# Colmar-zlicheng/Color-NeuS

Hardware: AMD Instinct MI355X
Metric: rays/sec (fwd+bwd) at 128 samples/ray (higher is better)
Workload: dtype f32; 1 GPU; Color_NeuS_dtu.yml renderer block (SDF 8x256 + colour 4x256 + relight 4x256), synthetic 800x800 view, 4096 rays/step/GPU x (64+64) samples, trained-like weights; samples_per_ray=128, parallelism=ray-sharded dp1, step=fwd+fused-loss+bwd+fused-clip-adam

## Files before the change

color-neus_amd/csrc/cnr_backend.h:

```cpp
#pragma once
#include "cnr_common.h"
#include "cnr_views.h"

namespace cnr {

constexpr int kMaxRaySamples = 256;
constexpr int kMaxOutside = 128;

struct Segment { int dst, src, len; };

struct PrepWeight {
  const float* g = nullptr;
  const float* v = nullptr;
  const float* b = nullptr;
  int n = 0, k_ref = 0;
  int nseg = 0; Segment seg[4];
  float* W = nullptr; int ldw = 0; int npad = 0;
  float* Wt = nullptr; int ldwt = 0; int kpad = 0;
  float* bias = nullptr;
  int row_rot = 0;
};

struct FinishWeight {
  const float* partial = nullptr; int nchunk = 0; int npad = 0; int ldk = 0;
// ... 24 lines not shown
};

struct UpSample {
  const float* o; const float* d; long R;
  const float* z; int ldz; const float* sdf; int lds; int n;
  int m;
  float inv_s;
  float* new_z;
  const float* w_in = nullptr;
  const float* u_in = nullptr;
};

struct MergeZ {
  long R; float* z; int ldz; const float* sdf_in; int lds_in; float* sdf_out; int lds_out; int n;
  const float* new_z; const float* new_sdf; int m;
};

struct SamplerStep {
  int do_merge; MergeZ g;
  UpSample u;
  int do_embed; float* E; float scale; int multires;
};
void be_sampler_step(const SamplerStep& p, cnr_stream s);

struct FineSetup {
  const float* o; const float* d; const float* z; long R; int M; float sample_dist;
  float scale; int multires; int multires_view;
  float* E;
  float* AUX;
};

struct GradFinish {
  long P; const float* E; const float* ce0; const float* ces; float scale; int multires;
  float* grad_out;
  float* AUX;
  int neg_g_as_view; int multires_view;
  float* featx; int ldfx; int F;
};

struct CompositeFwd {
  const float* o; const float* d; const float* z; long R; int M; float sample_dist;
  const float* sdf; const float* g; const float* color; int ldcolor; const float* gcolor; int ldg;
  const float* variance; float cos_anneal; const float* background_rgb;
  float* color_fine; float* s_val; float* cdf_fine; float* weight_sum; float* weight_max; float* weights;
  float* inside_sphere; float* depth; float* global_color;
  float* eik_partial;
  float* sdf_s; float* color_s; float* gcolor_s;
  const float* delta = nullptr; float* delta_ray_sum = nullptr;
};

struct PruneCount { const float* weights; long R; int M; float eps; int* counts; };
struct PruneScan { const int* counts; long R; int* offsets ; };
struct PruneGather {
  const float* weights; long R; int M; float eps; const int* offsets;
  int* idx;
  const float* featx; int ldfx; float* featx_c;
  const float* aux; float* aux_c;
  float* zero_gcol = nullptr; float* zero_relit = nullptr; float* zero_delta = nullptr;
};
struct PruneScatter {
  long P; const int* count; const int* idx;
  const float* gcol_c; const float* relit_c; const float* delta_c;
  float* gcol; float* relit; float* delta;
};

struct ReduceEik { const float* partial; long R; float* sums ; float* sums_out ; float* gradient_error; };

struct CompositeBwd {
  const float* o; const float* d; const float* z; long R; int M; float sample_dist;
  const float* sdf; const float* g; const float* color; int ldcolor; const float* gcolor; int ldg;
  const float* variance; float cos_anneal; const float* background_rgb; const float* eik_sums; float sdf_scale;
  int inv_sigmoid; int has_relight;
  const float* d_color_fine; const float* d_s_val; const float* d_cdf; const float* d_weight_sum; const float* d_weight_max;
  const float* d_gradients; const float* d_weights; const float* d_gradient_error; const float* d_depth;
  const float* d_global_color; const float* d_delta_relight; const float* d_delta_relight_ray ;
  const float* d_sdf_s; const float* d_color_s; const float* d_gcolor_s;
  float* ztop; int ldztop; int ztop_col;
  float* gbar;
  int ldtop = kTop;
  float* dtop;
  float* gc_a;
  float* dinvs_partial;
  float* d_rays_d;
  float* d_z;
};

struct ColTopBwd {
  long P; const float* gc_a ; const float* gc_b ; const float* gcolor; int squeeze; float* out;
  int ldtop = kTop;
};

struct GbarFinish {
  long P; const float* gbar_alpha; const float* daux_c; const float* daux_r; const float* E; float scale; int multires;
  float* gbar_total ; float* cbar ;
};

struct VarianceFinish { const float* partial; long R; const float* variance; float* d_variance; };

struct RaysGradFinish {
  long R; int M; const float* d; const float* z; float sample_dist;
  const float* pbar;
  const float* daux_dir_c; const float* daux_dir_r; int lddir; int multires_view;
  const float* d_rays_d_alpha;
  float* d_o; float* d_d;
  const float* dz_parts;
  float* d_near; float* d_far;
};

struct PbarFinish {
  long P; const float* daux_c; const float* daux_r; const float* ebar0; const float* ebars; const float* E;
  const float* ce0; const float* ces; const float* gbar_total ;
  float scale; int multires; float* pbar;
};

constexpr int kQueryCtxTag = 0x53515900;
struct QueryIn {
  long n, P; const float* pts; float* out; int* tag; int tag_value;
};
struct QuerySeed {
  long n, P; int F, ldztop; float inv_scale;
  const float* d_sdf; const float* d_feat; const float* d_grad;
  float* ztop; float* gbar;
  const int* tag; int want_grad;
};
struct QueryOut {
  long n; int F, ldf, ldg;
  const float* sdf_in; const float* feat_in; const float* g_in;
  float* sdf; float* feat; float* g;
};
void be_query_in(const QueryIn& p, cnr_stream s);
void be_query_seed(const QuerySeed& p, cnr_stream s);
void be_query_out(const QueryOut& p, cnr_stream s);

struct PackJob {
  const unsigned short* planes; long plane_stride; int rows; int ld; unsigned short* Wf;
};
void be_pack_frags_many(const PackJob* jobs, int count, cnr_stream s);
struct FusedLayer {
  const unsigned short* Wf;
  const float* wsc;
  const float* bias;
  int K;
  int N;
};
struct SdfValueChain {
  const float* E; long P;
  int nl;
  FusedLayer lay[kMaxLayers];
  int skip_mask; int emb;
  const float* wtop; const float* btop; float top_scale;
  float* sdf_out;
};
bool be_sdf_value_chain(const SdfValueChain& c, cnr_stream s);
struct SdfSaveChain {
  SdfValueChain v;
  float* Z[kMaxLayers] = {};
  int ldz = 0;
  float* rs[kMaxLayers + 1] = {};
  FusedLayer top;
  float* feat = nullptr; int ld_feat = 0;
};
bool be_sdf_save_chain(const SdfSaveChain& c, cnr_stream s);

constexpr int kChainSteps = 12;
struct ChainFwdStep {
  const unsigned short* Wf = nullptr;
  const float* wsc = nullptr;
  const float* bias = nullptr;
  int nkb_w = 0;
  int nkb_main = 0;
  int nkb_x = 0;
  const float* in = nullptr; int ld_in = 0;
  int x_src = 0;
  float* save = nullptr; int ld_save = 0;
  float* rs_in = nullptr;
  int head = 0;
};
struct ChainFwdHead { const float* W = nullptr; int ldw = 0; const float* bias = nullptr; int n = 0; };
struct ReluChainFwd {
  long P = 0; int nsteps = 0; ChainFwdStep st[kChainSteps];
  ChainFwdHead col_head; int col_squeeze = 1;
  float* gcol = nullptr;
  float* rgb_tail = nullptr; int ld_tail = 0;
  ChainFwdHead rel_head; int inv_sigmoid = 1;
  float* delta = nullptr;
  float* relit = nullptr;
  int dbg = 0;
  const int* P_dev = nullptr; const int* row_idx = nullptr;
};
bool be_relu_chain_fwd(const ReluChainFwd& c, cnr_stream s);
bool be_relu_chain_fwd_enabled();

void be_layer_gemm(const LayerGemm& g, cnr_stream s);
struct NarrowBwd {
  const float* X = nullptr; int ldx = 0;
  const float* Xb = nullptr; int ldxb = 0;
  const float* Y = nullptr; int ldy = 0; int ky = 0;
  long P = 0;
  const unsigned short* Wp = nullptr; long wp_stride = 0; int ldw = 0; int w_rows = 0; const float* wscale = nullptr;
  float* dx = nullptr; int lddx = 0; int ndx = 0;
  float* partial = nullptr; int ldk = 0; float* colsum = nullptr;
};
bool be_narrow_bwd_ok(const NarrowBwd& p);
int be_narrow_bwd_slots(long P);
void be_narrow_bwd(const NarrowBwd& p, cnr_stream s);
bool be_sweep0_ok(const LayerGemm& g);
int be_sweep0_slots(long P);
void be_sweep0_dw(const LayerGemm& g, float* partial, int ldk, cnr_stream s);
void be_dw_gemm(const DwGemm& g, cnr_stream s);
struct HeadBwd {
  const float* dtop; int ldt;
  const float* aux; int ldaux;
  const float* W; int ldw;
  int n; int K; long P;
  float* dout; int ldo;
  float* partial; float* colsum; int npad, ldk, nslots;
};
void be_head_bwd(const HeadBwd& p, cnr_stream s);
struct HeadFwd {
  const float* h; int ldh; long P; const int* P_dev;
  const float* W; int ldw; int n;
  Epi E;
};
void be_head_fwd(const HeadFwd& p, cnr_stream s);
struct StripBwd {
  const float* dout; int ldo; long P;
  int nt;
  const float* Wt; int ldwt;
  float* tail; int ldt; float tail_scale;
  const float* y; int ldy;
  float* partial; int npad, ldk, nslots;
};
void be_strip_bwd(const StripBwd& p, cnr_stream s);
bool be_fdw_enabled();
bool be_fdw_xrow();
void be_layer_dw_gemm(const LayerGemm& g, const DwGemm& d, const DwFuse& f, cnr_stream s);
void be_prep_weight(const PrepWeight& p, cnr_stream s);
void be_split_planes(const float* src, int rows, int ld, unsigned short* planes, float* inv_scale, cnr_stream s);
struct SplitJob { const float* src; int rows; int ld; unsigned short* planes; float* inv_scale; };
void be_prep_weights(const PrepWeight* p, int count, cnr_stream s);
void be_finish_weights(const FinishWeight* f, int count, cnr_stream s);
void be_split_planes_many(const SplitJob* jobs, int count, cnr_stream s);
void be_finish_weight(const FinishWeight& p, cnr_stream s);
void be_embed_z(const EmbedZ& p, cnr_stream s);
void be_embed_pts(const EmbedPts& p, cnr_stream s);
void be_upsample(const UpSample& p, cnr_stream s);
void be_merge(const MergeZ& p, cnr_stream s);
void be_fine_setup(const FineSetup& p, cnr_stream s);
void be_grad_finish(const GradFinish& p, cnr_stream s);
void be_composite_fwd(const CompositeFwd& p, cnr_stream s);
void be_reduce_eik(const ReduceEik& p, cnr_stream s);
void be_prune_count(const PruneCount& p, cnr_stream s);
void be_prune_scan(const PruneScan& p, cnr_stream s);
void be_prune_gather(const PruneGather& p, cnr_stream s);
void be_prune_scatter(const PruneScatter& p, cnr_stream s);
void be_composite_bwd(const CompositeBwd& p, cnr_stream s);
void be_coltop_bwd(const ColTopBwd& p, cnr_stream s);
void be_gbar_finish(const GbarFinish& p, cnr_stream s);
void be_variance_finish(const VarianceFinish& p, cnr_stream s);
void be_pbar_finish(const PbarFinish& p, cnr_stream s);
void be_rays_grad_finish(const RaysGradFinish& p, cnr_stream s);
void be_memset_zero(void* p, size_t bytes, cnr_stream s);

struct LossArgs {
  const float* color; const float* wsum; const float* drel; const float* gt; const float* mask;
  long R; int M; int rgb_l1; int include_mask;
  int drel_per_ray = 0;
};
constexpr int kLossBlocks = 256;
void be_loss_sums(const LossArgs& a, float* partial , float* sums , cnr_stream s);
void be_loss_grads(const LossArgs& a, const float* coef, float* d_color, float* d_wsum, float* d_drel, cnr_stream s);
struct LossScalars {
  float lf, le, lm, lr;
  float Rg, den_rgb, den_rel;
  float c_rgb, c_bce, c_rel;
  int use_mask, use_relight;
};
void be_loss_combine(const LossScalars& c, const float* sums, const float* gerr, float* out6, cnr_stream s);
void be_loss_coef(const LossScalars& c, const float* g_loss, const float* mean_rel, float* coef4, cnr_stream s);
void be_loss_forward(const LossArgs& a, float* partial, unsigned* ticket, const LossScalars& c, const float* gerr, float* sums, float* out6, cnr_stream s);
void be_loss_backward(const LossArgs& a, const LossScalars& c, const float* g_loss, const float* mean_rel, const float* eik_factor , float* coef4,
                      float* d_color, float* d_wsum, float* d_drel_ray , cnr_stream s);
void be_loss_shard_stats(const LossArgs& a, float* partial, unsigned* ticket, const float* eik_sums , float* stats8, cnr_stream s);
void be_loss_shard_combine(const LossScalars& c, const float* stats8, float* out8, cnr_stream s);
constexpr int kAdamBatch = 64;
constexpr int kAdamChunk = 4096;
struct AdamTensor { float* w; const float* g; long off; long n; int chunk0; };
struct AdamArgs {
  int count; AdamTensor t[kAdamBatch];
  int nchunks; float* partial;
  float* m; float* v;
  float lr, beta1, beta2, eps, max_norm;
  float bc1, bc2_sqrt;
  const float* hyper;
};
CNR_HD float adam_clip_coef(float norm2, float max_norm) {
  if (!(max_norm > 0.0f)) return 1.0f;
  const float c = max_norm / (sqrtf(norm2) + 1e-6f);
  return c < 1.0f ? c : 1.0f;
}
CNR_HD void adam_update1(const AdamArgs& a, float* w, float g, float* m, float* v) {
  const float m1 = *m + (g - *m) * (1.0f - a.beta1);
  const float v1 = *v * a.beta2 + (1.0f - a.beta2) * g * g;
  *m = m1; *v = v1;
  const float lr = a.hyper ? a.hyper[0] : a.lr, bc1 = a.hyper ? a.hyper[1] : a.bc1, bc2_sqrt = a.hyper ? a.hyper[2] : a.bc2_sqrt;
  const float denom = sqrtf(v1) / bc2_sqrt + a.eps;
// ... 270 lines not shown
```

color-neus_amd/csrc/cnr_bodies.h:

```cpp
#pragma once
#include "cnr_backend.h"
#include "cnr_raymath.h"

namespace cnr {

CNR_HD void body_embed_z_rows(const EmbedZ& p, long idx, float* out, float*) {
  long r = idx / p.m;
  int j = (int)(idx - r * p.m);
  float zz;
  if (p.make_z) {
    float nr = p.near_[r], fr = p.far_[r];
    zz = nr + (fr - nr) * linspace_at(0.0f, 1.0f, p.m, j);
    if (p.t_rand) zz = zz + (p.t_rand[r] - 0.5f) * 2.0f / (float)p.m;
    p.z[r * p.ldz + j] = zz;
  } else {
    zz = p.z[r * p.ldz + j];
  }
  float x[3];
  for (int c = 0; c < 3; ++c) x[c] = (p.o[r * 3 + c] + p.d[r * 3 + c] * zz) * p.scale;
  for (int c = 0; c < kEmb; ++c) out[c] = 0.0f;
  pe_row(x, p.multires, out);
}
CNR_HD void body_embed_z(const EmbedZ& p, long idx) { body_embed_z_rows(p, idx, p.E + idx * kEmb, nullptr); }

CNR_HD void body_embed_pts_rows(const EmbedPts& p, long i, float* e, float* a) {
  float pp[3];
  if (p.pts) {
    pp[0] = p.pts[i * 3]; pp[1] = p.pts[i * 3 + 1]; pp[2] = p.pts[i * 3 + 2];
  } else {
    long idx = p.start + i;
    long r2 = (long)p.res * p.res;
    int ix = (int)(idx / r2), iy = (int)((idx / p.res) % p.res), iz = (int)(idx % p.res);
    pp[0] = linspace_at(p.bmin[0], p.bmax[0], p.res, ix);
    pp[1] = linspace_at(p.bmin[1], p.bmax[1], p.res, iy);
    pp[2] = linspace_at(p.bmin[2], p.bmax[2], p.res, iz);
  }
  float x[3] = {pp[0] * p.scale, pp[1] * p.scale, pp[2] * p.scale};
  for (int c = 0; c < kEmb; ++c) e[c] = 0.0f;
  pe_row(x, p.multires, e);
  if (p.AUX) {
    for (int c = 0; c < kAux; ++c) a[c] = 0.0f;
    a[0] = pp[0]; a[1] = pp[1]; a[2] = pp[2];
  }
}
CNR_HD void body_embed_pts(const EmbedPts& p, long i) { body_embed_pts_rows(p, i, p.E + i * kEmb, p.AUX ? p.AUX + i * kAux : nullptr); }

CNR_HD void body_fine_setup_rows(const FineSetup& p, long pt, float* e, float* a) {
  long r = pt / p.M;
  int j = (int)(pt - r * p.M);
  float z0 = p.z[r * p.M + j];
  float dist = (j + 1 < p.M) ? p.z[r * p.M + j + 1] - z0 : p.sample_dist;
  float mid = z0 + dist * 0.5f;
  float pp[3], x[3], dd[3];
  for (int c = 0; c < 3; ++c) {
    dd[c] = p.d[r * 3 + c];
    pp[c] = p.o[r * 3 + c] + dd[c] * mid;
    x[c] = pp[c] * p.scale;
  }
  for (int c = 0; c < kEmb; ++c) e[c] = 0.0f;
  pe_row(x, p.multires, e);
  for (int c = 0; c < kAux; ++c) a[c] = 0.0f;
  a[0] = pp[0]; a[1] = pp[1]; a[2] = pp[2];
  if (p.multires_view > 0) pe_row(dd, p.multires_view, a + 6);
  else { a[6] = dd[0]; a[7] = dd[1]; a[8] = dd[2]; }
}
CNR_HD void body_fine_setup(const FineSetup& p, long pt) { body_fine_setup_rows(p, pt, p.E + pt * kEmb, p.AUX + pt * kAux); }

CNR_HD void body_grad_finish(const GradFinish& p, long pt) {
  const float* e = p.E + pt * kEmb;
  const float* c0 = p.ce0 + pt * kEmb;
  const float* cs = p.ces ? p.ces + pt * kEmb : nullptr;
  for (int c = 0; c < 3; ++c) {
    float acc = c0[c] + (cs ? cs[c] : 0.0f);
    float f = 1.0f;
    for (int k = 0; k < p.multires; ++k) {
      float csin = c0[3 + 6 * k + c] + (cs ? cs[3 + 6 * k + c] : 0.0f);
      float ccos = c0[6 + 6 * k + c] + (cs ? cs[6 + 6 * k + c] : 0.0f);
      acc = acc + f * (e[6 + 6 * k + c] * csin - e[3 + 6 * k + c] * ccos);
      f *= 2.0f;
    }
    float g = acc * p.scale;
    p.grad_out[pt * 3 + c] = g;
    p.AUX[pt * kAux + 3 + c] = g;
  }
  if (p.neg_g_as_view) {
    float v[3] = {-p.AUX[pt * kAux + 3], -p.AUX[pt * kAux + 4], -p.AUX[pt * kAux + 5]};
    float row[kAux];
    for (int c = 0; c < kAux; ++c) row[c] = 0.0f;
    if (p.multires_view > 0) pe_row(v, p.multires_view, row);
    else { row[0] = v[0]; row[1] = v[1]; row[2] = v[2]; }
    int npe = p.multires_view > 0 ? 3 + 6 * p.multires_view : 3;
    for (int c = 0; c < npe; ++c) p.AUX[pt * kAux + 6 + c] = row[c];
  }
  if (p.featx) {
    float* fx = p.featx + pt * p.ldfx + p.F;
    const float* a = p.AUX + pt * kAux;
    const int w = p.ldfx - p.F;
    for (int c = 0; c < w; ++c) fx[c] = c < kAux ? a[c] : 0.0f;
  }
}

CNR_HD void body_coltop_bwd(const ColTopBwd& p, long pt) {
  for (int c = 0; c < 3; ++c) {
    float gc = p.gc_a[pt * p.ldtop + c] + (p.gc_b ? p.gc_b[pt * 4 + c] : 0.0f);
    float y = p.gcolor[pt * 4 + c];
    p.out[pt * p.ldtop + c] = p.squeeze ? gc * y * (1.0f - y) : gc;
  }
  for (int c = 3; c < p.ldtop; ++c) p.out[pt * p.ldtop + c] = 0.0f;
}

CNR_HD void body_gbar_finish(const GbarFinish& p, long pt) {
  const float* e = p.E + pt * kEmb;
  float* cb = p.cbar + pt * kEmb;
  for (int c = 0; c < kEmb; ++c) cb[c] = 0.0f;
  for (int c = 0; c < 3; ++c) {
    float gb = p.gbar_alpha[pt * 4 + c];
    if (p.daux_c) gb += p.daux_c[pt * kAux + 3 + c];
    if (p.daux_r) gb += p.daux_r[pt * kAux + 3 + c];
    p.gbar_total[pt * 4 + c] = gb;
    float t = gb * p.scale;
    cb[c] = t;
    float f = 1.0f;
    for (int k = 0; k < p.multires; ++k) {
      cb[3 + 6 * k + c] = f * e[6 + 6 * k + c] * t;
      cb[6 + 6 * k + c] = -f * e[3 + 6 * k + c] * t;
      f *= 2.0f;
    }
  }
  p.gbar_total[pt * 4 + 3] = 0.0f;
}

CNR_HD void body_pbar_finish(const PbarFinish& p, long pt) {
  const float* e = p.E + pt * kEmb;
  for (int c = 0; c < 3; ++c) {
    float eb = p.ebar0[pt * kEmb + c] + (p.ebars ? p.ebars[pt * kEmb + c] : 0.0f);
    float x0bar = eb;
    float second = 0.0f;
    float f = 1.0f;
    for (int k = 0; k < p.multires; ++k) {
      float s = e[3 + 6 * k + c], co = e[6 + 6 * k + c];
      float ebs = p.ebar0[pt * kEmb + 3 + 6 * k + c] + (p.ebars ? p.ebars[pt * kEmb + 3 + 6 * k + c] : 0.0f);
      float ebc = p.ebar0[pt * kEmb + 6 + 6 * k + c] + (p.ebars ? p.ebars[pt * kEmb + 6 + 6 * k + c] : 0.0f);
      x0bar += f * (co * ebs - s * ebc);
      if (p.gbar_total) {
        float ces = p.ce0[pt * kEmb + 3 + 6 * k + c] + (p.ces ? p.ces[pt * kEmb + 3 + 6 * k + c] : 0.0f);
        float cec = p.ce0[pt * kEmb + 6 + 6 * k + c] + (p.ces ? p.ces[pt * kEmb + 6 + 6 * k + c] : 0.0f);
        second += f * f * (-s * ces - co * cec);
      }
      f *= 2.0f;
    }
    if (p.gbar_total) x0bar += p.gbar_total[pt * 4 + c] * p.scale * second;
    float pb = x0bar * p.scale;
    if (p.daux_c) pb += p.daux_c[pt * kAux + c];
    if (p.daux_r) pb += p.daux_r[pt * kAux + c];
    p.pbar[pt * 4 + c] = pb;
  }
  p.pbar[pt * 4 + 3] = 0.0f;
}

CNR_HD void body_query_in(const QueryIn& p, long i) {
  p.out[i] = i < p.n * 3 ? p.pts[i] : 0.0f;
  if (i == 0) *p.tag = p.tag_value;
}
CNR_HD bool query_ctx_mismatch(const QuerySeed& p) {
  const int t = *p.tag;
  return p.want_grad ? t != kQueryCtxTag + 1 : (t != kQueryCtxTag && t != kQueryCtxTag + 1);
}

CNR_HD void body_query_seed(const QuerySeed& p, long i) {
  const long q4 = p.ldztop / 4, nz = p.P * q4;
  const float poison = query_ctx_mismatch(p) ? __builtin_nanf("") : 0.0f;
  if (i < nz) {
    const long row = i / q4;
    const int c0 = (int)(i - row * q4) * 4;
    float v[4];
    for (int j = 0; j < 4; ++j) {
      const int c = c0 + j;
      float t = 0.0f;
      if (row < p.n) {
        if (c < p.F) t = p.d_feat ? p.d_feat[row * p.F + c] : 0.0f;
        else if (c == p.F) t = p.d_sdf ? p.d_sdf[row] * p.inv_scale : 0.0f;
      }
      v[j] = t + poison;
    }
    f4 o; o.x = v[0]; o.y = v[1]; o.z = v[2]; o.w = v[3];
    *reinterpret_cast<f4*>(p.ztop + row * p.ldztop + c0) = o;
  } else {
    const long row = i - nz;
    const bool live = row < p.n && p.d_grad;
    f4 o;
    o.x = (live ? p.d_grad[row * 3 + 0] : 0.0f) + poison; o.y = (live ? p.d_grad[row * 3 + 1] : 0.0f) + poison;
    o.z = (live ? p.d_grad[row * 3 + 2] : 0.0f) + poison; o.w = 0.0f;
    *reinterpret_cast<f4*>(p.gbar + row * 4) = o;
  }
}

CNR_HD void body_query_out(const QueryOut& p, long i) {
  if (p.sdf) {
    if (i < p.n) { p.sdf[i] = p.sdf_in[i]; return; }
    i -= p.n;
  }
  if (p.feat) {
    const long nf = p.n * p.F;
    if (i < nf) { const long r = i / p.F; p.feat[i] = p.feat_in[r * p.ldf + (i - r * p.F)]; return; }
    i -= nf;
  }
  const long r = i / 3;
  p.g[i] = p.g_in[r * p.ldg + (i - r * 3)];
}
CNR_HD long query_out_count(const QueryOut& p) { return (p.sdf ? p.n : 0) + (p.feat ? p.n * p.F : 0) + (p.g ? p.n * 3 : 0); }

struct PixKey { unsigned k0, k1, step; };
CNR_HD PixKey pix_key(long seed, long step) {
  const unsigned long long s = (unsigned long long)seed;
  return PixKey{(unsigned)(s & 0xffffffffull), (unsigned)(s >> 32), (unsigned)((unsigned long long)step & 0xffffffffull)};
}
CNR_HD void pix_philox(unsigned c0, unsigned c1, unsigned c2, unsigned c3, unsigned k0, unsigned k1, unsigned out[4]) {
// ... 636 lines not shown
```

color-neus_amd/csrc/cnr_chain.hip:

```cpp
#include <hip/hip_runtime.h>

#include <cstdlib>
#include <type_traits>

#include "cnr_backend.h"
#include "cnr_hip_util.h"
#include "cnr_gemm_int.h"
#include "cnr_chain_util.h"

namespace cnr {

constexpr int kPackBatch = 64;
struct PackBatch { int count; int blk_start[kPackBatch + 1]; PackJob j[kPackBatch]; };
static_assert(sizeof(PackBatch) <= 4096, "kernel argument block");

__global__ __launch_bounds__(64) void pack_frags_kernel(const PackBatch b) {
  int i = 0;
  while (i + 1 < b.count && (int)blockIdx.x >= b.blk_start[i + 1]) ++i;
  const PackJob& j = b.j[i];
  const int blk = (int)blockIdx.x - b.blk_start[i];
  const int nkb = j.ld / 16;
  const int plane = blk & 1, kb = (blk >> 1) % nkb, cb = (blk >> 1) / nkb;
  const int lane = threadIdx.x, m = lane & 31;
  const int n = cb * 32 + 16 * ((m >> 2) & 1) + 4 * (m >> 3) + (m & 3);
  typedef unsigned short u16x8 __attribute__((ext_vector_type(8)));
  u16x8 v = {0, 0, 0, 0, 0, 0, 0, 0};
  if (n < j.rows) v = *reinterpret_cast<const u16x8*>(j.planes + (long)plane * j.plane_stride + (long)n * j.ld + kb * 16 + (lane >> 5) * 8);
  *reinterpret_cast<u16x8*>(j.Wf + ((long)blk * 64 + lane) * 8) = v;
}

void be_pack_frags_many(const PackJob* jobs, int count, cnr_stream s) {
  for (int i0 = 0; i0 < count; i0 += kPackBatch) {
    PackBatch b;
    b.count = count - i0 < kPackBatch ? count - i0 : kPackBatch;
    int blks = 0;
    for (int i = 0; i < b.count; ++i) { b.blk_start[i] = blks; b.j[i] = jobs[i0 + i]; blks += 8 * (jobs[i0 + i].ld / 16) * 2; }
    b.blk_start[b.count] = blks;
    TimingScope ts_("pack_frags", 2, 0, blks, 0, 0, 0, s);
    hipLaunchKernelGGL(pack_frags_kernel, dim3(blks), dim3(64), 0, s, b);
  }
  CNR_LAUNCH_CHECK("pack_frags");
}

template <int RT, int CB>
__global__ __launch_bounds__(512 / CB, 2 / (3 - CB) + 0) void sdf_value_chain_kernel(const SdfValueChain c) {
  constexpr int WAVES = 8 / CB, THREADS = 64 * WAVES;
  constexpr int T = 32 * RT;
  constexpr int APLANE = T * CH_ALD;
  extern __shared__ __attribute__((aligned(16))) unsigned char smem[];
  float* rs = reinterpret_cast<float*>(smem + 2 * APLANE);
  float* pm = rs + T;
  float* cwb = pm + T * 8;
  float* wtop = cwb + 1024;
  const int tid0 = threadIdx.x, wave = __builtin_amdgcn_readfirstlane(tid0 >> 6);
  const long ntiles = (c.P + T - 1) / T;
#define VC_LANE_INDICES                                                                      \
  int tid = tid0;                                                                            \
  asm volatile("" : "+v"(tid));                                                              \
  const int lane = tid & 63, half = lane >> 5, pt = lane & 31;                               \
  const int cbase = wave * CB * 32 + 16 * half;

  f16x8 wr1[4][CB], wr2[4][CB];
  auto wlane_of = [&](const FusedLayer& L, int lane_) __attribute__((always_inline)) { return L.Wf + (long)wave * CB * (L.K >> 4) * 1024 + lane_ * 8; };
  auto wprime = [&](const FusedLayer& L, int lane_) __attribute__((always_inline)) { chain_wprime<CB>(wr1, wr2, wlane_of(L, lane_), L.K >> 4, 0, L.K >> 4); };
  auto cw_fetch = [&](const FusedLayer& L, int tid_) __attribute__((always_inline)) {
    f4 v = {0.f, 0.f, 0.f, 0.f};
    if (tid_ < 64) v = *reinterpret_cast<const f4*>(L.wsc + tid_ * 4);
    else if (tid_ < 128) v = *reinterpret_cast<const f4*>(L.bias + (tid_ - 64) * 4);
    return v;
  };

  wprime(c.lay[0], tid0 & 63);
  for (int i = tid0; i < 256; i += THREADS) wtop[i] = c.wtop[i];
  for (long tile = blockIdx.x; tile < ntiles; tile += gridDim.x) {
    constexpr int NPASS = T * 16 / THREADS;
    {
    int tid = tid0;
    asm volatile("" : "+v"(tid));
    if (tid < 128) *reinterpret_cast<f4*>(cwb + tid * 4) = cw_fetch(c.lay[0], tid);
    f4 erows[NPASS];
#pragma unroll
    for (int pass = 0; pass < NPASS; ++pass) {
      const int row_l = pass * (THREADS / 16) + (tid >> 4), sc4 = (tid & 15) * 4;
      long grow = tile * T + row_l; if (grow >= c.P) grow = c.P - 1;
      erows[pass] = *reinterpret_cast<const f4*>(c.E + grow * kEmb + (sc4 < kEmb ? sc4 : 0));
    }
#pragma unroll
    for (int pass = 0; pass < NPASS; ++pass) {
      const int row_l = pass * (THREADS / 16) + (tid >> 4), sc4 = (tid & 15) * 4;
      const f4 z4 = {0.f, 0.f, 0.f, 0.f};
      const f4 v = sc4 < kEmb ? erows[pass] : z4;
      float mx = ws_absmax4(v);
      mx = cnr_max16(mx);
      const float sc = chain_row_scale(mx);
      if (sc4 < kEmb) {
        f16x4 h1, h2;
        float x;
        x = v.x * sc; h1[0] = (_Float16)x; h2[0] = (_Float16)(x - (float)h1[0]);
        x = v.y * sc; h1[1] = (_Float16)x; h2[1] = (_Float16)(x - (float)h1[1]);
        x = v.z * sc; h1[2] = (_Float16)x; h2[2] = (_Float16)(x - (float)h1[2]);
        x = v.w * sc; h1[3] = (_Float16)x; h2[3] = (_Float16)(x - (float)h1[3]);
        unsigned char* dst = smem + row_l * CH_ALD + sc4 * 2;
        *reinterpret_cast<f16x4*>(dst) = h1;
        *reinterpret_cast<f16x4*>(dst + APLANE) = h2;
      }
      if ((tid & 15) == 0) rs[row_l] = cnr_pow2_rcp(sc);
    }
    }
    lds_barrier();

    for (int l = 0; l < c.nl; ++l) {
      VC_LANE_INDICES
      const FusedLayer& L = c.lay[l];
      const int nkb = L.K >> 4;
      const bool last = l + 1 == c.nl;
      const unsigned short* wlane = wlane_of(L, lane);
      const f4 cw_next = cw_fetch(c.lay[last ? l : l + 1], tid);
      f32x16 acc[CB][RT];
#pragma unroll
      for (int j = 0; j < CB; ++j)
#pragma unroll
        for (int rt = 0; rt < RT; ++rt)
#pragma unroll
          for (int r = 0; r < 16; ++r) acc[j][rt][r] = 0.0f;
      const unsigned char* Ab = smem + pt * CH_ALD + half * 16;
      if (nkb == 16) chain_mfma_blocks<RT, CB, 16>(acc, wr1, wr2, Ab, APLANE, wlane, 16, 0);
      else chain_mfma_blocks<RT, CB, 3>(acc, wr1, wr2, Ab, APLANE, wlane, 3, 0);
      wprime(last ? c.lay[0] : c.lay[l + 1], lane);

      const float* cw = cwb + (l & 1) * 512;
      const bool next_skip = !last && ((c.skip_mask >> (l + 1)) & 1);
      const float oscale = next_skip ? kInvSqrt2 : 1.0f;
      const bool ragged = L.N < 256;
      float red[RT], dotj[CB][RT];
#pragma unroll
      for (int rt = 0; rt < RT; ++rt) {
        red[rt] = 0.0f;
#pragma unroll
        for (int j = 0; j < CB; ++j) dotj[j][rt] = 0.0f;
      }
#pragma unroll
      for (int j = 0; j < CB; ++j) {
        const int c0 = cbase + 32 * j;
        f4 wsc4[4], b4[4];
#pragma unroll
        for (int q = 0; q < 4; ++q) {
          wsc4[q] = *reinterpret_cast<const f4*>(cw + c0 + 4 * q);
          b4[q] = *reinterpret_cast<const f4*>(cw + 256 + c0 + 4 * q);
        }
#pragma unroll
        for (int rt = 0; rt < RT; ++rt) {
          const int row_l = rt * 32 + pt;
          const f2 rsc = pk_splat(rs[row_l]);
#pragma unroll
          for (int q = 0; q < 8; ++q) {
            const f2 w = {wsc4[q >> 1][(2 * q) & 3], wsc4[q >> 1][(2 * q + 1) & 3]};
            const f2 b = {b4[q >> 1][(2 * q) & 3], b4[q >> 1][(2 * q + 1) & 3]};
            f2 a = {acc[j][rt][2 * q], acc[j][rt][2 * q + 1]};
            a = pk_fma(a, rsc * w, b);
            a = softplus100_pk(a);
            if (next_skip) a = a * pk_splat(kInvSqrt2);
            acc[j][rt][2 * q] = a.x; acc[j][rt][2 * q + 1] = a.y;
          }
          if (ragged && c0 + 16 > L.N) {
            long grow = tile * T + row_l; if (grow >= c.P) grow = c.P - 1;
            const float* erow = c.E + grow * kEmb;
            float ev[16];
#pragma unroll
            for (int r = 0; r < 16; ++r) { const int ei = c0 + r - L.N; ev[r] = erow[ei < 0 ? 0 : (ei < kEmb ? ei : kEmb - 1)]; }
#pragma unroll
            for (int r = 0; r < 16; ++r) {
              const int ei = c0 + r - L.N;
              const float tail = (next_skip && ei < c.emb) ? ev[r] * oscale : 0.0f;
              acc[j][rt][r] = ei < 0 ? acc[j][rt][r] : tail;
            }
          }
          float mx = 0.0f, dot = 0.0f;
          if (last) {
#pragma unroll
            for (int q = 0; q < 4; ++q) {
              const f4 wt = *reinterpret_cast<const f4*>(wtop + c0 + 4 * q);
              dot = fmaf(acc[j][rt][4 * q], wt.x, dot); dot = fmaf(acc[j][rt][4 * q + 1], wt.y, dot);
              dot = fmaf(acc[j][rt][4 * q + 2], wt.z, dot); dot = fmaf(acc[j][rt][4 * q + 3], wt.w, dot);
            }
          } else {
#pragma unroll
            for (int r = 0; r < 16; r += 2) mx = fmaxf(fmaxf(fabsf(acc[j][rt][r]), fabsf(acc[j][rt][r + 1])), mx);
          }
          if (last) dotj[j][rt] = dot; else red[rt] = fmaxf(red[rt], mx);
        }
      }
#pragma unroll
      for (int rt = 0; rt < RT; ++rt) {
        if (last) {
#pragma unroll
          for (int j = 0; j < CB; ++j) {
            const float both = cnr_pair32_sum(dotj[j][rt]);
            if (half == 0) pm[(rt * 32 + pt) * 8 + wave * CB + j] = both;
          }
        } else {
          const float both = cnr_pair32_max(red[rt]);
          if (half == 0) pm[(rt * 32 + pt) * 8 + wave] = both;
        }
      }
      lds_barrier();
      if (!last) {
        if (tid < 128) *reinterpret_cast<f4*>(cwb + ((l + 1) & 1) * 512 + tid * 4) = cw_next;
#pragma unroll
        for (int rt = 0; rt < RT; ++rt) {
          const int row_l = rt * 32 + pt;
          float mx = pm[row_l * 8];
#pragma unroll
          for (int w = 1; w < WAVES; ++w) mx = fmaxf(mx, pm[row_l * 8 + w]);
          const float sc = chain_row_scale(mx);
#pragma unroll
          for (int j = 0; j < CB; ++j) chain_put16(acc[j][rt], sc, smem + row_l * CH_ALD + (cbase + 32 * j) * 2, APLANE);
          if (wave == 0 && half == 0) rs[row_l] = cnr_pow2_rcp(sc);
        }
      } else {
        for (int row = tid; row < T; row += THREADS) {
          float sum = pm[row * 8];
#pragma unroll
          for (int w = 1; w < 8; ++w) sum += pm[row * 8 + w];
          const long grow = tile * T + row;
          if (grow < c.P) c.sdf_out[grow] = (sum + c.btop[0]) * c.top_scale;
        }
      }
      lds_barrier();
    }
  }
}

#undef VC_LANE_INDICES

template <int RT, int CB>
static void launch_sdf_value_chain(const SdfValueChain& c, cnr_stream s) {
  constexpr int T = 32 * RT, THREADS = 512 / CB;
  const size_t lds = (size_t)2 * T * CH_ALD + (size_t)T * 9 * sizeof(float) + (size_t)(1024 + 256) * sizeof(float);
  static DeviceOnce attr_once;
  if (attr_once.first())
    (void)hipFuncSetAttribute(reinterpret_cast<const void*>(&sdf_value_chain_kernel<RT, CB>), hipFuncAttributeMaxDynamicSharedMemorySize, 160 * 1024);
  const long ntiles = (c.P + T - 1) / T;
  const int wgs_env = debug_flags().chain_wgs;
  const long wgs = wgs_env > 0 ? wgs_env : (lds * 2 <= 160 * 1024 ? 512 : 256);
  const unsigned grid = (unsigned)(ntiles < wgs ? ntiles : wgs);
  double macs = 0.0;
  for (int l = 0; l < c.nl; ++l) macs += (double)c.lay[l].K * 256.0;
  TimingScope ts_("chain_sdf_value", 3, RT * 10 + CB, c.P, (int)(macs / 256.0), 256, 1, s, (double)c.P * (kEmb + 1) * 4.0);
  hipLaunchKernelGGL((sdf_value_chain_kernel<RT, CB>), dim3(grid), dim3(THREADS), lds, s, c);
}

bool be_sdf_value_chain(const SdfValueChain& c, cnr_stream s) {
  const bool off = debug_flags().no_fused;
  if (off || c.P <= 0) return false;
  for (int l = 0; l < c.nl; ++l)
    if ((c.lay[l].K != 256 && c.lay[l].K != 48) || c.lay[l].N > 256 || c.lay[l].N < 1) return false;
  const int force = debug_flags().chain_shape;
  const int shape = force ? force : (c.P >= 256L * 128 ? 41 : (c.P >= 256L * 64 ? 22 : 12));
  if (shape == 41) launch_sdf_value_chain<4, 1>(c, s);
  else if (shape == 22) launch_sdf_value_chain<2, 2>(c, s);
  else launch_sdf_value_chain<1, 2>(c, s);
  CNR_LAUNCH_CHECK("chain_sdf_value");
  return true;
}

}
```

color-neus_amd/csrc/cnr_debug.h:

```cpp
#pragma once

namespace cnr {

struct DebugFlags {
  bool no_fused = false, no_chain_fwd = false, no_chain_sdf = false, no_fdw = false, fdw_split = false, no_top_fuse = false,
       no_head_bwd = false, no_head_fwd = false, no_strip_bwd = false, no_sampler_fuse = false, no_sweep0 = false, no_narrow_bwd = false,
       no_narrow_dx = false, disable_ws = false, ws_generic = false, ws_nostream = false, dw_fp32 = false, dw_bf16 = false, roctx = false;
  int ws_serp = 1;
#ifdef CNR_TUNING
  int ws_kinds = 0xffff, ws_minw = 96, ws_wgs = 256, ws_mintpw = 1, chain_wgs = 0, chain_shape = 0, chain_fwd_rt = 0, fdw_deep = 0, fdw_norev = 0,
      fdw_revmode = 0, fdw_dbg = 0, chain_fwd_dbg = 0;
  long chain_sdf_maxp = 1L << 62;
#else
  static constexpr int ws_kinds = 0xffff, ws_minw = 96, ws_wgs = 256, ws_mintpw = 1, chain_wgs = 0, chain_shape = 0, chain_fwd_rt = 0, fdw_deep = 0,
                       fdw_norev = 0, fdw_revmode = 0, fdw_dbg = 0, chain_fwd_dbg = 0;
  static constexpr long chain_sdf_maxp = 1L << 62;
#endif
};

const DebugFlags& debug_flags();

#ifdef CNR_TUNING
#define CNR_ABLATION(x) (x)
#else
#define CNR_ABLATION(x) 0
#endif

}
```

color-neus_amd/csrc/cnr_kernels.hip:

```cpp
#include <hip/hip_runtime.h>
#include <dlfcn.h>

#include <cstdio>
#include <vector>

#include "cnr_backend.h"
#include "cnr_loss.h"
#include "cnr_bodies.h"
#include "cnr_hip_util.h"

namespace cnr {

typedef float f32x16 __attribute__((ext_vector_type(16)));

hipError_t g_first_error = hipSuccess;
const char* g_first_error_where = "";

const char* be_name() { return "hip-gfx950"; }

struct TimingRec { KernelTiming t; hipEvent_t e0, e1; };
static bool g_timing_on = false;
static std::vector<TimingRec> g_timing;
static std::vector<hipEvent_t> g_event_pool;
static hipEvent_t get_event() {
  if (!g_event_pool.empty()) { hipEvent_t e = g_event_pool.back(); g_event_pool.pop_back(); return e; }
  hipEvent_t e;
  (void)hipEventCreate(&e);
  return e;
}
void timing_begin(const char* name, int kind, int nt, long P, int N, int K, int pairs, hipStream_t s, double bytes) {
  if (!g_timing_on) return;
  TimingRec r;
  snprintf(r.t.name, sizeof r.t.name, "%s", name);
  r.t.kind = kind; r.t.nt = nt; r.t.P = P; r.t.N = N; r.t.K = K; r.t.pairs = pairs; r.t.ms = 0.f; r.t.bytes = bytes;
  r.e0 = get_event(); r.e1 = get_event();
  (void)hipEventRecord(r.e0, s);
  g_timing.push_back(r);
}
void timing_end(hipStream_t s) {
  if (!g_timing_on || g_timing.empty()) return;
  (void)hipEventRecord(g_timing.back().e1, s);
}
void be_timing_enable(int on) { g_timing_on = on != 0; }
int be_timing_collect(KernelTiming* out, int max_records) {
  int n = 0;
  for (auto& r : g_timing) {
    (void)hipEventSynchronize(r.e1);
    float ms = 0.f;
    (void)hipEventElapsedTime(&ms, r.e0, r.e1);
    r.t.ms = ms;
    if (out && n < max_records) out[n] = r.t;
    ++n;
    g_event_pool.push_back(r.e0);
    g_event_pool.push_back(r.e1);
  }
  g_timing.clear();
  return n;
}

namespace {
struct Roctx {
  int (*push)(const char*) = nullptr; int (*pop)() = nullptr;
  Roctx() {
    if (!debug_flags().roctx) return;
    for (const char* lib : {"librocprofiler-sdk-roctx.so", "libroctx64.so"}) {
      void* h = dlopen(lib, RTLD_LAZY | RTLD_GLOBAL);
      if (!h) continue;
      push = reinterpret_cast<int (*)(const char*)>(dlsym(h, "roctxRangePushA"));
      pop = reinterpret_cast<int (*)()>(dlsym(h, "roctxRangePop"));
      if (push && pop) return;
      push = nullptr; pop = nullptr;
    }
  }
};
Roctx& roctx() { static Roctx r; return r; }
}
void be_range_push(const char* name) { if (roctx().push) (void)roctx().push(name); }
void be_range_pop() { if (roctx().pop) (void)roctx().pop(); }

int be_check_last_error(char* msg, size_t n) {
  if (g_first_error == hipSuccess) return 0;
  snprintf(msg, n, "HIP error in %s: %s", g_first_error_where, hipGetErrorString(g_first_error));
  g_first_error = hipSuccess;
  return -1;
}

void be_memset_zero(void* p, size_t bytes, cnr_stream s) {
  hipError_t e = hipMemsetAsync(p, 0, bytes, s);
  if (e != hipSuccess && g_first_error == hipSuccess) { g_first_error = e; g_first_error_where = "memset"; }
}

__global__ void zero_cols_kernel(float* p, int ld, int c0, int c1, long rows) {
  const int w = c1 - c0;
  const long i = (long)blockIdx.x * blockDim.x + threadIdx.x;
  if (i < rows * w) p[(i / w) * ld + c0 + (int)(i % w)] = 0.0f;
}
void be_zero_cols(float* p, int ld, int c0, int c1, long rows, cnr_stream s) {
  if (c1 <= c0 || rows <= 0) return;
  const long n = rows * (c1 - c0);
  hipLaunchKernelGGL(zero_cols_kernel, dim3((unsigned)((n + 255) / 256)), dim3(256), 0, s, p, ld, c0, c1, rows);
  CNR_LAUNCH_CHECK("zero_cols");
}

__global__ __launch_bounds__(256) void copy_cols_kernel(float* dst, int ld_dst, const float* src, int ld_src, int ncols, long rows) {
  const long n = rows * ncols;
  for (long i = (long)blockIdx.x * 256 + threadIdx.x; i < n; i += (long)gridDim.x * 256) {
    const long r = i / ncols;
    const int c = (int)(i - r * ncols);
    dst[r * ld_dst + c] = src[r * ld_src + c];
  }
}
void be_copy_cols(float* dst, int ld_dst, const float* src, int ld_src, int ncols, long rows, cnr_stream s) {
  if (ncols <= 0 || rows <= 0) return;
  long blocks = (rows * ncols + 255) / 256;
  if (blocks > 65536) blocks = 65536;
  hipLaunchKernelGGL(copy_cols_kernel, dim3((unsigned)blocks), dim3(256), 0, s, dst, ld_dst, src, ld_src, ncols, rows);
  CNR_LAUNCH_CHECK("copy_cols");
}

__global__ __launch_bounds__(512) void head_bwd_kernel(const HeadBwd p, long pts_per_slot) {
  __shared__ float red[8][4][256];
  const int cg = threadIdx.x & 63, rl = threadIdx.x >> 6, k = cg * 4;
  const long p0 = (long)blockIdx.x * pts_per_slot;
  long p1 = p0 + pts_per_slot;
  if (p1 > p.P) p1 = p.P;
  const bool live = k < p.K;
  f4 w[4], acc[4];
  float cs[4] = {0.f, 0.f, 0.f, 0.f};
  const f4 z4 = {0.f, 0.f, 0.f, 0.f};
#pragma unroll
  for (int j = 0; j < 4; ++j) { acc[j] = z4; w[j] = (live && j < p.n) ? *reinterpret_cast<const f4*>(p.W + (long)j * p.ldw + k) : z4; }
  f4 an[8], dn[8];
  const int kl = live ? k : 0;
  auto fetch = [&](long pt) __attribute__((always_inline)) {
#pragma unroll
    for (int u = 0; u < 8; ++u) {
      long q = pt + 8 * u < p1 ? pt + 8 * u : p1 - 1;
      if (q < 0) q = 0;
      an[u] = *reinterpret_cast<const f4*>(p.aux + q * p.ldaux + kl);
      dn[u] = *reinterpret_cast<const f4*>(p.dtop + q * p.ldt);
    }
  };
  fetch(p0 + rl);
  for (long pt = p0 + rl; pt < p1; pt += 64) {
    f4 a[8], d[8];
#pragma unroll
    for (int u = 0; u < 8; ++u) { a[u] = live ? an[u] : z4; d[u] = dn[u]; }
    fetch(pt + 64);
#pragma unroll
    for (int u = 0; u < 8; ++u) {
      if (pt + 8 * u < p1) {
        const float dj[4] = {d[u].x, d[u].y, d[u].z, d[u].w};
        f4 v = z4;
#pragma unroll
        for (int j = 0; j < 4; ++j) {
          v.x = fmaf(w[j].x, dj[j], v.x); v.y = fmaf(w[j].y, dj[j], v.y); v.z = fmaf(w[j].z, dj[j], v.z); v.w = fmaf(w[j].w, dj[j], v.w);
          acc[j].x = fmaf(dj[j], a[u].x, acc[j].x); acc[j].y = fmaf(dj[j], a[u].y, acc[j].y);
          acc[j].z = fmaf(dj[j], a[u].z, acc[j].z); acc[j].w = fmaf(dj[j], a[u].w, acc[j].w);
          cs[j] += dj[j];
        }
        f4 o;
        o.x = a[u].x > 0.0f ? v.x : 0.0f; o.y = a[u].y > 0.0f ? v.y : 0.0f; o.z = a[u].z > 0.0f ? v.z : 0.0f; o.w = a[u].w > 0.0f ? v.w : 0.0f;
// ... 189 lines not shown
  }
CNR_POINTWISE_KERNELS(CNR_PW_KERNEL)

constexpr int kRowsPerBlock = 128, kRowLd = 49;
static_assert(kEmb == 48 && kAux == 48, "row staging assumes 48-float rows");
template <class PARAM, void (*ROWS)(const PARAM&, long, float*, float*)>
__global__ __launch_bounds__(kRowsPerBlock) void staged_rows_kernel(const PARAM p, long n, float* E, float* AUX) {
  __shared__ float sE[kRowsPerBlock * kRowLd];
  __shared__ float sA[kRowsPerBlock * kRowLd];
  const int tid = threadIdx.x;
  for (long base = (long)blockIdx.x * kRowsPerBlock; base < n; base += (long)gridDim.x * kRowsPerBlock) {
    if (base + tid < n) ROWS(p, base + tid, sE + tid * kRowLd, sA + tid * kRowLd);
    __syncthreads();
    const int cnt = (int)((n - base) < kRowsPerBlock ? (n - base) : kRowsPerBlock) * 48;
    for (int e = tid; e < cnt; e += kRowsPerBlock) {
      const int r = e / 48, c = e - r * 48;
      E[base * 48 + e] = sE[r * kRowLd + c];
      if (AUX) AUX[base * 48 + e] = sA[r * kRowLd + c];
    }
    __syncthreads();
  }
}
template <class PARAM, void (*ROWS)(const PARAM&, long, float*, float*)>
static void staged_rows_launch(const char* name, const PARAM& p, long n, float* E, float* AUX, cnr_stream s) {
  if (n <= 0) return;
  long blocks = (n + kRowsPerBlock - 1) / kRowsPerBlock;
  if (blocks > 16384) blocks = 16384;
  TimingScope ts_(name, 2, 0, n, 0, 0, 0, s);
  hipLaunchKernelGGL((staged_rows_kernel<PARAM, ROWS>), dim3((unsigned)blocks), dim3(kRowsPerBlock), 0, s, p, n, E, AUX);
}
void be_embed_z(const EmbedZ& p, cnr_stream s) { staged_rows_launch<EmbedZ, body_embed_z_rows>("embed_z", p, p.R * p.m, p.E, nullptr, s); CNR_LAUNCH_CHECK("embed_z"); }
void be_embed_pts(const EmbedPts& p, cnr_stream s) { staged_rows_launch<EmbedPts, body_embed_pts_rows>("embed_pts", p, p.n, p.E, p.AUX, s); CNR_LAUNCH_CHECK("embed_pts"); }
void be_fine_setup(const FineSetup& p, cnr_stream s) { staged_rows_launch<FineSetup, body_fine_setup_rows>("fine_setup", p, p.R * p.M, p.E, p.AUX, s); CNR_LAUNCH_CHECK("fine_setup"); }

__global__ __launch_bounds__(256) void grad_finish_kernel(const GradFinish p) {
  const int lane16 = threadIdx.x & 15;
  const long pt0 = ((long)blockIdx.x * 256 + threadIdx.x) >> 4;
  const long stride = (long)gridDim.x * 16;
  for (long pt = pt0; pt < p.P; pt += stride) {
    const int c0 = lane16 * 3;
    float e[3], ce[3];
#pragma unroll
    for (int c = 0; c < 3; ++c) {
      e[c] = p.E[pt * kEmb + c0 + c];
      ce[c] = p.ce0[pt * kEmb + c0 + c] + (p.ces ? p.ces[pt * kEmb + c0 + c] : 0.0f);
    }
    const int k = lane16 > 0 ? (lane16 - 1) >> 1 : 0;
    const bool is_sin = lane16 >= 1 && (lane16 & 1) == 1 && lane16 <= 2 * p.multires;
    const bool is_cos = lane16 >= 2 && (lane16 & 1) == 0 && lane16 <= 2 * p.multires;
    const float f = (float)(1 << k);
    float part[3];
#pragma unroll
    for (int c = 0; c < 3; ++c) {
      const float e_next = __shfl_down(e[c], 1, 16);
      const float e_prev = __shfl_up(e[c], 1, 16);
      float t = 0.0f;
      if (lane16 == 0) t = ce[c];
      else if (is_sin) t = f * (e_next * ce[c]);
      else if (is_cos) t = -(f * (e_prev * ce[c]));
      part[c] = t;
    }
#pragma unroll
    for (int d = 8; d >= 1; d >>= 1)
#pragma unroll
      for (int c = 0; c < 3; ++c) part[c] += __shfl_xor(part[c], d, 16);
    float g[3];
#pragma unroll
    for (int c = 0; c < 3; ++c) g[c] = part[c] * p.scale;
    if (lane16 == 0) {
#pragma unroll
      for (int c = 0; c < 3; ++c) { p.grad_out[pt * 3 + c] = g[c]; p.AUX[pt * kAux + 3 + c] = g[c]; }
    }
    float aux[3];
#pragma unroll
    for (int c = 0; c < 3; ++c) aux[c] = lane16 == 1 ? g[c] : p.AUX[pt * kAux + c0 + c];
    if (p.neg_g_as_view) {
      const int et = lane16 - 2;
      if (et >= 0) {
        float v[3] = {-g[0], -g[1], -g[2]};
        const int npe_tr = p.multires_view > 0 ? 1 + 2 * p.multires_view : 1;
#pragma unroll
        for (int c = 0; c < 3; ++c) {
          float val = 0.0f;
          if (et == 0) val = v[c];
          else if (et < npe_tr) { const float ff = (float)(1 << ((et - 1) >> 1)); val = (et & 1) ? sinf(v[c] * ff) : cosf(v[c] * ff); }
          if (et < npe_tr) { aux[c] = val; p.AUX[pt * kAux + c0 + c] = val; }
        }
      }
    }
    if (p.featx) {
      const int w = p.ldfx - p.F;
#pragma unroll
      for (int c = 0; c < 3; ++c)
        if (c0 + c < w) p.featx[pt * p.ldfx + p.F + c0 + c] = aux[c];
      for (int c = kAux + lane16; c < w; c += 16) p.featx[pt * p.ldfx + p.F + c] = 0.0f;
    }
  }
}
void be_grad_finish(const GradFinish& p, cnr_stream s) {
  if (p.P <= 0) return;
  long blocks = (p.P * 16 + 255) / 256;
  if (blocks > 16384) blocks = 16384;
  TimingScope ts_("grad_finish", 2, 0, p.P, 0, 0, 0, s);
  hipLaunchKernelGGL(grad_finish_kernel, dim3((unsigned)blocks), dim3(256), 0, s, p);
  CNR_LAUNCH_CHECK("grad_finish");
}

__global__ __launch_bounds__(256) void gbar_finish_kernel(const GbarFinish p) {
  const int lane16 = threadIdx.x & 15;
  const long pt0 = ((long)blockIdx.x * 256 + threadIdx.x) >> 4;
  const long stride = (long)gridDim.x * 16;
  for (long pt = pt0; pt < p.P; pt += stride) {
    const int c0 = lane16 * 3;
    float e[3], gb[3];
#pragma unroll
    for (int c = 0; c < 3; ++c) {
      e[c] = p.E[pt * kEmb + c0 + c];
      float v = p.gbar_alpha[pt * 4 + c];
      if (p.daux_c) v += p.daux_c[pt * kAux + 3 + c];
      if (p.daux_r) v += p.daux_r[pt * kAux + 3 + c];
      gb[c] = v;
    }
    const int k = lane16 > 0 ? (lane16 - 1) >> 1 : 0;
    const bool is_sin = lane16 >= 1 && (lane16 & 1) == 1 && lane16 <= 2 * p.multires;
    const bool is_cos = lane16 >= 2 && (lane16 & 1) == 0 && lane16 <= 2 * p.multires;
    const float f = (float)(1 << k);
#pragma unroll
    for (int c = 0; c < 3; ++c) {
      const float e_next = __shfl_down(e[c], 1, 16);
      const float e_prev = __shfl_up(e[c], 1, 16);
      const float t = gb[c] * p.scale;
      float out = 0.0f;
      if (lane16 == 0) out = t;
      else if (is_sin) out = f * e_next * t;
      else if (is_cos) out = -f * e_prev * t;
      p.cbar[pt * kEmb + c0 + c] = out;
    }
    if (lane16 == 0) {
#pragma unroll
      for (int c = 0; c < 3; ++c) p.gbar_total[pt * 4 + c] = gb[c];
      p.gbar_total[pt * 4 + 3] = 0.0f;
    }
  }
}
void be_gbar_finish(const GbarFinish& p, cnr_stream s) {
  if (p.P <= 0) return;
  long blocks = (p.P * 16 + 255) / 256;
  if (blocks > 16384) blocks = 16384;
  TimingScope ts_("gbar_finish", 2, 0, p.P, 0, 0, 0, s);
  hipLaunchKernelGGL(gbar_finish_kernel, dim3((unsigned)blocks), dim3(256), 0, s, p);
  CNR_LAUNCH_CHECK("gbar_finish");
}

__device__ __forceinline__ float wave_sum(float x) {
#pragma unroll
  for (int d = 32; d >= 1; d >>= 1) x += __shfl_xor(x, d);
  return x;
}
__device__ __forceinline__ float wave_max(float x) {
#pragma unroll
  for (int d = 32; d >= 1; d >>= 1) x = fmaxf(x, __shfl_xor(x, d));
  return x;
}
__device__ __forceinline__ int wave_min_int(int x) {
#pragma unroll
  for (int d = 32; d >= 1; d >>= 1) { int y = __shfl_xor(x, d); x = y < x ? y : x; }
  return x;
}
__device__ __forceinline__ float block_sum_256(float x, float* sh4 ) {
  x = wave_sum(x);
  __syncthreads();
  if ((threadIdx.x & 63) == 0) sh4[threadIdx.x >> 6] = x;
  __syncthreads();
  return (sh4[0] + sh4[1]) + (sh4[2] + sh4[3]);
}

__device__ __forceinline__ double block_sum_256d(double x, double* sh4) {
#pragma unroll
  for (int d = 32; d >= 1; d >>= 1) x += __shfl_xor(x, d);
  __syncthreads();
  if ((threadIdx.x & 63) == 0) sh4[threadIdx.x >> 6] = x;
  __syncthreads();
  return (sh4[0] + sh4[1]) + (sh4[2] + sh4[3]);
}

__device__ __forceinline__ void prep_weight_row(const PrepWeight& p, const int n, double* redd) {
  const int tid = threadIdx.x;
  const bool real = n < p.n;
  const int nr = real ? (n + p.row_rot) % p.n : 0;
  float scale = 1.0f;
  if (p.g != nullptr) {
    double ss = 0.0;
    if (real)
      for (int c = tid; c < p.k_ref; c += 256) { double x = p.v[(long)nr * p.k_ref + c]; ss += x * x; }
    ss = block_sum_256d(ss, redd);
    if (real) scale = p.g[nr] / (float)sqrt(ss);
  }
  for (int j = tid; j < p.kpad; j += 256) {
    float val = 0.0f;
    if (real && j < p.ldw) {
      int src = -1;
      for (int q = 0; q < p.nseg; ++q)
        if (j >= p.seg[q].dst && j < p.seg[q].dst + p.seg[q].len) src = p.seg[q].src + (j - p.seg[q].dst);
      if (src >= 0) val = p.v[(long)nr * p.k_ref + src] * scale;
    }
    if (j < p.ldw) p.W[(long)n * p.ldw + j] = val;
    if (n < p.ldwt) p.Wt[(long)j * p.ldwt + n] = val;
  }
  if (tid == 0) p.bias[n] = real && p.b ? p.b[nr] : 0.0f;
}
__global__ __launch_bounds__(256) void prep_weight_kernel(const PrepWeight p) {
  __shared__ double redd[4];
  prep_weight_row(p, blockIdx.x, redd);
}
constexpr int kPrepBatch = 24;
struct PrepBatch { int count; int row_start[kPrepBatch + 1]; PrepWeight p[kPrepBatch]; };
static_assert(sizeof(PrepBatch) <= 4096, "kernel argument block");
__global__ __launch_bounds__(256) void prep_weight_batch_kernel(const PrepBatch b) {
  __shared__ double redd[4];
  int i = 0;
  while (i + 1 < b.count && (int)blockIdx.x >= b.row_start[i + 1]) ++i;
  prep_weight_row(b.p[i], (int)blockIdx.x - b.row_start[i], redd);
}

__device__ __forceinline__ void split_planes_row(const float* src, int ld, unsigned short* planes, long plane_stride, float* inv_scale, const int r) {
  const float* row = src + (long)r * ld;
  float mx = 0.0f;
  for (int k = threadIdx.x; k < ld; k += 64) mx = fmaxf(mx, fabsf(row[k]));
#pragma unroll
  for (int d = 32; d >= 1; d >>= 1) mx = fmaxf(mx, __shfl_xor(mx, d));
  float sc = 1.0f;
  if (mx > 0.0f && mx < 3.0e38f) { int e; (void)frexpf(mx, &e); if (e < -100) e = -100; sc = ldexpf(1.0f, 14 - e); }
  for (int k = threadIdx.x; k < ld; k += 64) {
    const float x = row[k] * sc;
    const _Float16 h1 = (_Float16)x;
    const _Float16 h2 = (_Float16)(x - (float)h1);
    planes[(long)r * ld + k] = __builtin_bit_cast(unsigned short, h1);
    planes[plane_stride + (long)r * ld + k] = __builtin_bit_cast(unsigned short, h2);
  }
  if (threadIdx.x == 0) inv_scale[r] = 1.0f / sc;
}
__global__ __launch_bounds__(64) void split_planes_kernel(const float* src, int ld, unsigned short* planes, long plane_stride, float* inv_scale) {
  split_planes_row(src, ld, planes, plane_stride, inv_scale, blockIdx.x);
}
constexpr int kSplitBatch = 2 * kPrepBatch;
struct SplitBatch { int count; int row_start[kSplitBatch + 1]; SplitJob j[kSplitBatch]; };
static_assert(sizeof(SplitBatch) <= 4096, "kernel argument block");
__global__ __launch_bounds__(64) void split_planes_batch_kernel(const SplitBatch b) {
  int i = 0;
  while (i + 1 < b.count && (int)blockIdx.x >= b.row_start[i + 1]) ++i;
  const SplitJob& j = b.j[i];
  split_planes_row(j.src, j.ld, j.planes, (long)j.rows * j.ld, j.inv_scale, (int)blockIdx.x - b.row_start[i]);
}
void be_split_planes_many(const SplitJob* jobs, int count, cnr_stream s) {
  for (int i0 = 0; i0 < count; i0 += kSplitBatch) {
    SplitBatch b;
    b.count = count - i0 < kSplitBatch ? count - i0 : kSplitBatch;
    int rows = 0;
    for (int i = 0; i < b.count; ++i) { b.row_start[i] = rows; b.j[i] = jobs[i0 + i]; rows += jobs[i0 + i].rows; }
    b.row_start[b.count] = rows;
    TimingScope ts_("split_planes", 2, 0, rows, 0, 0, 0, s);
    hipLaunchKernelGGL(split_planes_batch_kernel, dim3(rows), dim3(64), 0, s, b);
  }
  CNR_LAUNCH_CHECK("split_planes");
}
void be_prep_weights(const PrepWeight* p, int count, cnr_stream s) {
  for (int i0 = 0; i0 < count; i0 += kPrepBatch) {
    PrepBatch b;
    b.count = count - i0 < kPrepBatch ? count - i0 : kPrepBatch;
    int rows = 0;
    for (int i = 0; i < b.count; ++i) { b.row_start[i] = rows; b.p[i] = p[i0 + i]; rows += p[i0 + i].npad; }
    b.row_start[b.count] = rows;
    TimingScope ts_("prep_weight", 2, 0, rows, 0, 0, 0, s);
    hipLaunchKernelGGL(prep_weight_batch_kernel, dim3(rows), dim3(256), 0, s, b);
  }
  CNR_LAUNCH_CHECK("prep_weight");
}
void be_split_planes(const float* src, int rows, int ld, unsigned short* planes, float* inv_scale, cnr_stream s) {
  TimingScope ts_("split_planes", 2, 0, rows, 0, 0, 0, s);
  hipLaunchKernelGGL(split_planes_kernel, dim3(rows), dim3(64), 0, s, src, ld, planes, (long)rows * ld, inv_scale);
  CNR_LAUNCH_CHECK("split_planes");
}

void be_prep_weight(const PrepWeight& p, cnr_stream s) {
  TimingScope ts_("prep_weight", 2, 0, p.npad, 0, 0, 0, s);
  hipLaunchKernelGGL(prep_weight_kernel, dim3(p.npad), dim3(256), 0, s, p);
  CNR_LAUNCH_CHECK("prep_weight");
}

__device__ __forceinline__ void finish_weight_row(const FinishWeight& p, const int n, float* red, double* redd, float* dwi) {
  const int tid = threadIdx.x;
  const int nr = (n + p.row_rot) % p.n;
  for (int j = tid; j < p.ldk; j += 256) {
    const float* src = p.partial + (long)n * p.ldk + j;
    const long cs = (long)p.npad * p.ldk;
    float s = 0.0f;
    int c = 0;
    const int nch = j >= p.col_hi ? p.nchunk_hi : p.nchunk;
    for (; c + 8 <= nch; c += 8) {
      float v[8];
#pragma unroll
      for (int q = 0; q < 8; ++q) v[q] = src[(long)(c + q) * cs];
#pragma unroll
      for (int q = 0; q < 8; ++q) s += v[q];
    }
    for (; c < nch; ++c) s += src[(long)c * cs];
    dwi[j] = s;
  }
  __syncthreads();
  float dref[2] = {0.f, 0.f};
  int cref[2] = {-1, -1};
// ... 95 lines not shown
  for (int j = 0; j < 3; ++j) { const float s = block_sum_256(v[j], red); if (tid == 0) sums[j] = s; }
  if (tid == 0) sums[3] = 0.f;
}
void be_loss_sums(const LossArgs& a, float* partial, float* sums, cnr_stream s) {
  TimingScope ts_("loss_sums", 2, 0, a.R, 0, 0, 0, s);
  hipLaunchKernelGGL(loss_partial_kernel, dim3(kLossBlocks), dim3(256), 0, s, a, partial);
  hipLaunchKernelGGL(loss_fold_kernel, dim3(1), dim3(256), 0, s, partial, kLossBlocks, sums);
  CNR_LAUNCH_CHECK("loss_sums");
}
__global__ __launch_bounds__(256) void loss_forward_kernel(const LossArgs a, float* partial, unsigned* ticket, const LossScalars c, const float* gerr, float* sums,
                                                           float* out6, const int shard, const float* eik_sums) {
  __shared__ float red[4];
  __shared__ int is_last;
  const int tid = threadIdx.x, nb = gridDim.x, b = blockIdx.x;
  float s_rgb = 0.f, s_bce = 0.f, s_rel = 0.f;
  const long n_rgb = a.R * 3;
  for (long i = (long)b * 256 + tid; i < n_rgb; i += (long)nb * 256) s_rgb += loss_rgb_term(a.color[i], a.gt[i], a.rgb_l1);
  if (a.mask)
    for (long r = (long)b * 256 + tid; r < a.R; r += (long)nb * 256) s_bce += loss_bce_term(a.wsum[r], a.mask[r]);
  if (a.drel) {
    const long per_ray = a.drel_per_ray ? 1 : (long)a.M * 3, n_rel = a.R * per_ray;
    for (long i = (long)b * 256 + tid; i < n_rel; i += (long)nb * 256) {
      const float m = (a.include_mask && a.mask) ? a.mask[i / per_ray] : 1.0f;
      s_rel += a.drel[i] * m;
    }
  }
  s_rgb = block_sum_256(s_rgb, red);
  s_bce = block_sum_256(s_bce, red);
  s_rel = block_sum_256(s_rel, red);
  if (tid == 0) {
    partial[b * 4 + 0] = s_rgb; partial[b * 4 + 1] = s_bce; partial[b * 4 + 2] = s_rel; partial[b * 4 + 3] = 0.f;
    __threadfence();
    const unsigned t = atomicAdd(ticket, 1u);
    is_last = t == (unsigned)nb - 1u;
  }
  __syncthreads();
  if (!is_last) return;
  __threadfence();
  float v[3] = {0.f, 0.f, 0.f};
  for (int k = tid; k < nb; k += 256) {
    v[0] += __hip_atomic_load(partial + k * 4, __ATOMIC_RELAXED, __HIP_MEMORY_SCOPE_AGENT);
    v[1] += __hip_atomic_load(partial + k * 4 + 1, __ATOMIC_RELAXED, __HIP_MEMORY_SCOPE_AGENT);
    v[2] += __hip_atomic_load(partial + k * 4 + 2, __ATOMIC_RELAXED, __HIP_MEMORY_SCOPE_AGENT);
  }
  __shared__ float tot[4];
  for (int j = 0; j < 3; ++j) { const float sj = block_sum_256(v[j], red); if (tid == 0) tot[j] = sj; }
  if (tid == 0) {
    tot[3] = 0.f;
    if (shard) {
      const float num = eik_sums[0], den = eik_sums[1];
      sums[0] = tot[0]; sums[1] = tot[1]; sums[2] = tot[2]; sums[3] = num; sums[4] = den; sums[5] = den; sums[6] = 0.f; sums[7] = 0.f;
    } else {
      sums[0] = tot[0]; sums[1] = tot[1]; sums[2] = tot[2]; sums[3] = 0.f;
      loss_combine(c, tot, gerr, out6);
    }
    *ticket = 0;
  }
}
void be_loss_forward(const LossArgs& a, float* partial, unsigned* ticket, const LossScalars& c, const float* gerr, float* sums, float* out6, cnr_stream s) {
  TimingScope ts_("loss_forward", 2, 0, a.R, 0, 0, 0, s);
  hipLaunchKernelGGL(loss_forward_kernel, dim3(kLossBlocks), dim3(256), 0, s, a, partial, ticket, c, gerr, sums, out6, 0, (const float*)nullptr);
  CNR_LAUNCH_CHECK("loss_forward");
}
void be_loss_shard_stats(const LossArgs& a, float* partial, unsigned* ticket, const float* eik_sums, float* stats8, cnr_stream s) {
  TimingScope ts_("loss_shard_stats", 2, 0, a.R, 0, 0, 0, s);
  hipLaunchKernelGGL(loss_forward_kernel, dim3(kLossBlocks), dim3(256), 0, s, a, partial, ticket, LossScalars{}, (const float*)nullptr, stats8, (float*)nullptr, 1, eik_sums);
  CNR_LAUNCH_CHECK("loss_shard_stats");
}
__global__ void loss_shard_combine_kernel(const LossScalars c, const float* stats, float* out8) { if (threadIdx.x == 0 && blockIdx.x == 0) loss_shard_combine(c, stats, out8); }
void be_loss_shard_combine(const LossScalars& c, const float* stats8, float* out8, cnr_stream s) {
  TimingScope ts_("loss_shard_combine", 2, 0, 1, 0, 0, 0, s);
  hipLaunchKernelGGL(loss_shard_combine_kernel, dim3(1), dim3(64), 0, s, c, stats8, out8);
  CNR_LAUNCH_CHECK("loss_shard_combine");
}
__global__ __launch_bounds__(256) void loss_backward_kernel(const LossArgs a, const LossScalars c, const float* g_loss, const float* mean_rel, const float* eik_factor,
                                                            float* coef_out, float* d_color, float* d_wsum, float* d_drel_ray) {
  float coef[4];
  loss_coef(c, g_loss, c.use_relight ? mean_rel : g_loss, eik_factor, coef);
  if (blockIdx.x == 0 && threadIdx.x == 0) { coef_out[0] = coef[0]; coef_out[1] = coef[1]; coef_out[2] = coef[2]; coef_out[3] = coef[3]; }
  const long n_rgb = a.R * 3;
  const long stride = (long)gridDim.x * 256;
  for (long i = (long)blockIdx.x * 256 + threadIdx.x; i < n_rgb; i += stride) d_color[i] = coef[0] * loss_rgb_grad(a.color[i], a.gt[i], a.rgb_l1);
  if (d_wsum)
    for (long r = (long)blockIdx.x * 256 + threadIdx.x; r < a.R; r += stride) d_wsum[r] = a.mask ? coef[1] * loss_bce_grad(a.wsum[r], a.mask[r]) : 0.0f;
  if (d_drel_ray)
    for (long r = (long)blockIdx.x * 256 + threadIdx.x; r < a.R; r += stride) d_drel_ray[r] = (a.include_mask && a.mask) ? coef[2] * a.mask[r] : coef[2];
}
void be_loss_backward(const LossArgs& a, const LossScalars& c, const float* g_loss, const float* mean_rel, const float* eik_factor, float* coef4, float* d_color,
                      float* d_wsum, float* d_drel_ray, cnr_stream s) {
  TimingScope ts_("loss_backward", 2, 0, a.R, 0, 0, 0, s);
  long blocks = (a.R * 3 + 255) / 256;
  if (blocks > 1024) blocks = 1024;
  if (blocks < 1) blocks = 1;
  hipLaunchKernelGGL(loss_backward_kernel, dim3((unsigned)blocks), dim3(256), 0, s, a, c, g_loss, mean_rel, eik_factor, coef4, d_color, d_wsum, d_drel_ray);
  CNR_LAUNCH_CHECK("loss_backward");
}
__global__ __launch_bounds__(256) void loss_grads_kernel(const LossArgs a, const float* coef, float* d_color, float* d_wsum, float* d_drel) {
  const float c_rgb = coef[0], c_bce = coef[1], c_rel = coef[2];
  const long n_rgb = a.R * 3, per_ray = (long)a.M * 3, n_rel = a.drel || d_drel ? a.R * per_ray : 0;
  const long stride = (long)gridDim.x * 256;
  for (long i = (long)blockIdx.x * 256 + threadIdx.x; i < n_rgb; i += stride) d_color[i] = c_rgb * loss_rgb_grad(a.color[i], a.gt[i], a.rgb_l1);
  if (d_wsum)
    for (long r = (long)blockIdx.x * 256 + threadIdx.x; r < a.R; r += stride) d_wsum[r] = a.mask ? c_bce * loss_bce_grad(a.wsum[r], a.mask[r]) : 0.0f;
  if (d_drel)
    for (long i = (long)blockIdx.x * 256 + threadIdx.x; i < n_rel; i += stride) d_drel[i] = c_rel * ((a.include_mask && a.mask) ? a.mask[i / per_ray] : 1.0f);
}
__global__ void loss_combine_kernel(const LossScalars c, const float* sums, const float* gerr, float* out) { if (threadIdx.x == 0 && blockIdx.x == 0) loss_combine(c, sums, gerr, out); }
__global__ void loss_coef_kernel(const LossScalars c, const float* g_loss, const float* mean_rel, float* coef) { if (threadIdx.x == 0 && blockIdx.x == 0) loss_coef(c, g_loss, mean_rel, nullptr, coef); }
void be_loss_combine(const LossScalars& c, const float* sums, const float* gerr, float* out6, cnr_stream s) {
  hipLaunchKernelGGL(loss_combine_kernel, dim3(1), dim3(64), 0, s, c, sums, gerr, out6);
  CNR_LAUNCH_CHECK("loss_combine");
}
void be_loss_coef(const LossScalars& c, const float* g_loss, const float* mean_rel, float* coef4, cnr_stream s) {
  hipLaunchKernelGGL(loss_coef_kernel, dim3(1), dim3(64), 0, s, c, g_loss, mean_rel, coef4);
  CNR_LAUNCH_CHECK("loss_coef");
}
void be_loss_grads(const LossArgs& a, const float* coef, float* d_color, float* d_wsum, float* d_drel, cnr_stream s) {
  TimingScope ts_("loss_grads", 2, 0, a.R, 0, 0, 0, s);
  hipLaunchKernelGGL(loss_grads_kernel, dim3(1024), dim3(256), 0, s, a, coef, d_color, d_wsum, d_drel);
  CNR_LAUNCH_CHECK("loss_grads");
}

__global__ __launch_bounds__(256) void reduce_eik_kernel(const ReduceEik p) {
  __shared__ float red[4];
  float a = 0.0f, b = 0.0f;
  for (long r = threadIdx.x; r < p.R; r += 256) { a += p.partial[r * 2]; b += p.partial[r * 2 + 1]; }
  a = block_sum_256(a, red);
  b = block_sum_256(b, red);
  if (threadIdx.x == 0) {
    p.sums[0] = a; p.sums[1] = b;
    if (p.sums_out) { p.sums_out[0] = a; p.sums_out[1] = b; }
    *p.gradient_error = a / (b + 1e-5f);
  }
}
void be_reduce_eik(const ReduceEik& p, cnr_stream s) {
  TimingScope ts_("reduce_eik", 2, 0, p.R, 0, 0, 0, s);
  hipLaunchKernelGGL(reduce_eik_kernel, dim3(1), dim3(256), 0, s, p);
  CNR_LAUNCH_CHECK("reduce_eik");
}

__global__ __launch_bounds__(256) void variance_finish_kernel(const VarianceFinish p) {
  __shared__ float red[4];
  float a = 0.0f;
  for (long r = threadIdx.x; r < p.R; r += 256) a += p.partial[r];
  a = block_sum_256(a, red);
  if (threadIdx.x == 0) *p.d_variance = inv_s_backward(p.variance[0], a);
}
void be_variance_finish(const VarianceFinish& p, cnr_stream s) {
  TimingScope ts_("variance_finish", 2, 0, p.R, 0, 0, 0, s);
  hipLaunchKernelGGL(variance_finish_kernel, dim3(1), dim3(256), 0, s, p);
  CNR_LAUNCH_CHECK("variance_finish");
}

__device__ __forceinline__ float wave_scan_incl_add(float x, int lane) {
#pragma unroll
  for (int d = 1; d < 64; d <<= 1) { float y = __shfl_up(x, d); if (lane >= d) x = y + x; }
  return x;
}
__device__ __forceinline__ float wave_scan_incl_mul(float x, int lane) {
#pragma unroll
  for (int d = 1; d < 64; d <<= 1) { float y = __shfl_up(x, d); if (lane >= d) x = y * x; }
  return x;
}
__device__ __forceinline__ float wave_excl_cumprod(float f, int lane, float& carry) {
  const float incl = wave_scan_incl_mul(f, lane);
  float excl = __shfl_up(incl, 1);
  if (lane == 0) excl = 1.0f;
  const float T = carry * excl;
  carry = carry * __shfl(incl, 63);
  return T;
}
__device__ __forceinline__ float wave_scan_incl_add_rev(float x, int lane) {
#pragma unroll
  for (int d = 1; d < 64; d <<= 1) { float y = __shfl_down(x, d); if (lane + d < 64) x = x + y; }
  return x;
}

__device__ __forceinline__ void ray_section_slopes(const float* zs, const float* ss, int nsec, float* cs, int lane) {
  for (int i = lane; i < nsec; i += 64) cs[i] = upsample_slope(ss[i], ss[i + 1], zs[i], zs[i + 1]);
}
__device__ __forceinline__ void ray_section_alphas(const float* zs, const float* ss, const float* cs, const float* rs, int nsec, float inv_s, float* as, int lane) {
  for (int i = lane; i < nsec; i += 64) {
    const float c = upsample_cos(i > 0 ? cs[i - 1] : 0.0f, cs[i], rs[i], rs[i + 1]);
    as[i] = upsample_alpha(ss[i], ss[i + 1], zs[i], zs[i + 1], c, inv_s);
  }
}
__device__ __forceinline__ float ray_pdf_weights(float* as, int nsec, bool given_w, int lane) {
  float carry = 1.0f, part = 0.0f;
  for (int base = 0; base < nsec; base += 64) {
    const int i = base + lane;
    const bool ok = i < nsec;
    const float a = ok ? as[i] : 0.0f;
    const float T = wave_excl_cumprod(ok ? 1.0f - a + 1e-7f : 1.0f, lane, carry);
    const float w = (given_w ? a : a * T) + 1e-5f;
    if (ok) { as[i] = w; part += w; }
  }
  return wave_sum(part);
}
__device__ __forceinline__ void ray_cdf(const float* as, float total, int nsec, float* cs, int lane) {
  float csum = 0.0f;
  for (int base = 0; base < nsec; base += 64) {
    const int i = base + lane;
    const bool ok = i < nsec;
    const float pdf = ok ? as[i] / total : 0.0f;
    const float incl = wave_scan_incl_add(pdf, lane);
    if (ok) cs[i + 1] = csum + incl;
    csum = csum + __shfl(incl, 63);
  }
  if (lane == 0) cs[0] = 0.0f;
}

__global__ __launch_bounds__(256) void upsample_kernel(const UpSample p) {
  __shared__ float sh[4][5][kMaxRaySamples];
  const int lane = threadIdx.x & 63, wave = threadIdx.x >> 6;
  long ray = (long)blockIdx.x * 4 + wave;
  const bool active = ray < p.R;
  if (!active) ray = p.R - 1;
  float* zs = sh[wave][0]; float* ss = sh[wave][1]; float* cs = sh[wave][2]; float* rs = sh[wave][3]; float* as = sh[wave][4];
  const int n = p.n, nsec = p.n - 1;
  const bool given_w = p.w_in != nullptr;
  if (given_w) {
    for (int i = lane; i < n; i += 64) zs[i] = p.z[ray * p.ldz + i];
    for (int i = lane; i < nsec; i += 64) as[i] = p.w_in[ray * nsec + i];
  } else {
    float o[3], d[3];
    for (int c = 0; c < 3; ++c) { o[c] = p.o[ray * 3 + c]; d[c] = p.d[ray * 3 + c]; }
    for (int i = lane; i < n; i += 64) {
      float z = p.z[ray * p.ldz + i];
      zs[i] = z;
      ss[i] = p.sdf[ray * p.lds + i];
      rs[i] = ray_radius(o, d, z);
    }
  }
  __syncthreads();
  if (!given_w) ray_section_slopes(zs, ss, nsec, cs, lane);
  __syncthreads();
  if (!given_w) ray_section_alphas(zs, ss, cs, rs, nsec, p.inv_s, as, lane);
  __syncthreads();
  const float total = ray_pdf_weights(as, nsec, given_w, lane);
  __syncthreads();
  ray_cdf(as, total, nsec, cs, lane);
  __syncthreads();
  if (lane < p.m && active) {
    const float u = p.u_in ? p.u_in[ray * p.m + lane] : linspace_at(0.5f / (float)p.m, 1.0f - 0.5f / (float)p.m, p.m, lane);
    p.new_z[ray * p.m + lane] = invert_cdf(cs, zs, n, u);
  }
}
void be_upsample(const UpSample& p, cnr_stream s) {
  TimingScope ts_("upsample", 2, 0, p.R, 0, 0, 0, s, (double)p.R * (4.0 * p.n + 4.0 * (p.w_in ? p.n - 1 : p.n) + (p.w_in ? 0.0 : 24.0) + 4.0 * p.m));
  hipLaunchKernelGGL(upsample_kernel, dim3((unsigned)((p.R + 3) / 4)), dim3(256), 0, s, p);
  CNR_LAUNCH_CHECK("upsample");
}

__global__ __launch_bounds__(256) void merge_kernel(const MergeZ p) {
  __shared__ float sh[4][2][kMaxRaySamples];
  __shared__ float shn[4][2][64];
  const int lane = threadIdx.x & 63, wave = threadIdx.x >> 6;
  long ray = (long)blockIdx.x * 4 + wave;
  const bool active = ray < p.R;
  if (!active) ray = p.R - 1;
  float* zs = sh[wave][0]; float* ss = sh[wave][1]; float* nz = shn[wave][0]; float* ns = shn[wave][1];
  const bool with_sdf = p.new_sdf != nullptr;
  for (int i = lane; i < p.n; i += 64) { zs[i] = p.z[ray * p.ldz + i]; ss[i] = with_sdf ? p.sdf_in[ray * p.lds_in + i] : 0.0f; }
  for (int j = lane; j < p.m; j += 64) { nz[j] = p.new_z[ray * p.m + j]; ns[j] = with_sdf ? p.new_sdf[ray * p.m + j] : 0.0f; }
  __syncthreads();
  if (active)
    merge_samples(zs, ss, p.n, nz, ns, p.m, lane, 64, [&](int at, float z, float s) {
      p.z[ray * p.ldz + at] = z;
      if (with_sdf) p.sdf_out[ray * p.lds_out + at] = s;
    });
}
__global__ __launch_bounds__(256) void sampler_step_kernel(const SamplerStep p) {
  __shared__ float sh[4][7][kMaxRaySamples];
  __shared__ float shn[4][2][64];
  const int lane = threadIdx.x & 63, wave = threadIdx.x >> 6;
  long ray = (long)blockIdx.x * 4 + wave;
  const bool active = ray < p.u.R;
  if (!active) ray = p.u.R - 1;
  float* zs = sh[wave][0]; float* ss = sh[wave][1]; float* cs = sh[wave][2]; float* rs = sh[wave][3]; float* as = sh[wave][4];
  float* zo = sh[wave][5]; float* so = sh[wave][6]; float* nz = shn[wave][0]; float* ns = shn[wave][1];
  const UpSample& u = p.u;
  const int n = u.n, nsec = u.n - 1;
  float o[3], d[3];
  for (int c = 0; c < 3; ++c) { o[c] = u.o[ray * 3 + c]; d[c] = u.d[ray * 3 + c]; }
  if (p.do_merge) {
    const MergeZ& g = p.g;
    for (int i = lane; i < g.n; i += 64) { zo[i] = g.z[ray * g.ldz + i]; so[i] = g.sdf_in[ray * g.lds_in + i]; }
    for (int j = lane; j < g.m; j += 64) { nz[j] = g.new_z[ray * g.m + j]; ns[j] = g.new_sdf[ray * g.m + j]; }
    __syncthreads();
    merge_samples(zo, so, g.n, nz, ns, g.m, lane, 64, [&](int at, float z, float s) { zs[at] = z; ss[at] = s; });
    __syncthreads();
    if (active)
      for (int i = lane; i < n; i += 64) { g.z[ray * g.ldz + i] = zs[i]; g.sdf_out[ray * g.lds_out + i] = ss[i]; }
  } else {
    for (int i = lane; i < n; i += 64) { zs[i] = u.z[ray * u.ldz + i]; ss[i] = u.sdf[ray * u.lds + i]; }
    __syncthreads();
  }
  for (int i = lane; i < n; i += 64) rs[i] = ray_radius(o, d, zs[i]);
  __syncthreads();
  ray_section_slopes(zs, ss, nsec, cs, lane);
  __syncthreads();
  ray_section_alphas(zs, ss, cs, rs, nsec, u.inv_s, as, lane);
  __syncthreads();
  const float total = ray_pdf_weights(as, nsec, false, lane);
  __syncthreads();
  ray_cdf(as, total, nsec, cs, lane);
  __syncthreads();
  if (lane < u.m) {
    const float znew = invert_cdf(cs, zs, n, linspace_at(0.5f / (float)u.m, 1.0f - 0.5f / (float)u.m, u.m, lane));
    nz[lane] = znew;
    if (active) u.new_z[ray * u.m + lane] = znew;
  }
  if (p.do_embed) {
    __syncthreads();
    if (active) {
      const int ntr = kEmb / 3;
      for (int idx = lane; idx < u.m * ntr; idx += 64) {
        const int j = idx / ntr, t = idx - j * ntr;
        const float z = nz[j];
        float v[3];
        const int k = t > 0 ? (t - 1) >> 1 : 0;
        const float f = (float)(1 << k);
#pragma unroll
        for (int c = 0; c < 3; ++c) {
          const float x = (o[c] + d[c] * z) * p.scale;
          float sn, cn;
          sincosf(x * f, &sn, &cn);
          v[c] = t == 0 ? x : (t <= 2 * p.multires ? ((t & 1) ? sn : cn) : 0.0f);
        }
        float* e = p.E + (ray * u.m + j) * kEmb + 3 * t;
        e[0] = v[0]; e[1] = v[1]; e[2] = v[2];
      }
    }
  }
}
void be_sampler_step(const SamplerStep& p, cnr_stream s) {
  TimingScope ts_("sampler_step", 2, 0, p.u.R, 0, 0, 0, s, (double)p.u.R * (8.0 * p.u.n + 24.0 + 4.0 * p.u.m + (p.do_embed ? 4.0 * kEmb * p.u.m : 0.0)));
  hipLaunchKernelGGL(sampler_step_kernel, dim3((unsigned)((p.u.R + 3) / 4)), dim3(256), 0, s, p);
  CNR_LAUNCH_CHECK("sampler_step");
}

void be_merge(const MergeZ& p, cnr_stream s) {
  TimingScope ts_("merge", 2, 0, p.R, 0, 0, 0, s, (double)p.R * (p.new_sdf ? 2.0 : 1.0) * (4.0 * p.n + 4.0 * p.m + 4.0 * (p.n + p.m)));
  hipLaunchKernelGGL(merge_kernel, dim3((unsigned)((p.R + 3) / 4)), dim3(256), 0, s, p);
  CNR_LAUNCH_CHECK("merge");
}

constexpr int kRayChunks = kMaxRaySamples / 64;

__global__ __launch_bounds__(256) void composite_fwd_kernel(const CompositeFwd p) {
  __shared__ float shz[4][kMaxRaySamples];
  const int lane = threadIdx.x & 63, wave = threadIdx.x >> 6;
  long ray = (long)blockIdx.x * 4 + wave;
  const bool active = ray < p.R;
  if (!active) ray = p.R - 1;
  float* zs = shz[wave];
  const int M = p.M;
  for (int i = lane; i < M; i += 64) zs[i] = p.z[ray * M + i];
  __syncthreads();
  float o[3], d[3];
  for (int c = 0; c < 3; ++c) { o[c] = p.o[ray * 3 + c]; d[c] = p.d[ray * 3 + c]; }
  const float inv_s = inv_s_of(p.variance[0]);

  float carry = 1.0f;
  float wsum = 0.f, wmax = -1.f, dep = 0.f, col[3] = {0.f, 0.f, 0.f}, gcl[3] = {0.f, 0.f, 0.f}, e0 = 0.f, e1 = 0.f, drs = 0.f;
#pragma unroll
  for (int c = 0; c < kRayChunks; ++c) {
    if (c * 64 < M) {
      const int j = c * 64 + lane;
      const long pt = ray * M + j;
      if (p.delta && j < M) drs += (p.delta[pt * 3] + p.delta[pt * 3 + 1]) + p.delta[pt * 3 + 2];
      RaySample q = ray_sample(zs, j, M, p.sample_dist, o, d, p.sdf, p.g, pt, inv_s, p.cos_anneal);
      const float T = wave_excl_cumprod(q.ok ? 1.0f - q.a.alpha + 1e-7f : 1.0f, lane, carry);
      const float w = q.ok ? q.a.alpha * T : 0.0f;
      if (q.ok) {
        wsum += w; wmax = fmaxf(wmax, w); dep += w * q.z;
        if (p.color) for (int k = 0; k < 3; ++k) col[k] += w * p.color[pt * p.ldcolor + k];
        if (p.gcolor) for (int k = 0; k < 3; ++k) gcl[k] += w * p.gcolor[pt * p.ldg + k];
        e0 += q.relax * (q.gn - 1.0f) * (q.gn - 1.0f);
        e1 += q.relax;
        if (active) {
          p.weights[pt] = w;
          p.cdf_fine[pt] = q.a.pc;
          p.inside_sphere[pt] = q.inside;
          if (p.sdf_s) p.sdf_s[pt] = p.sdf[pt];
          if (p.color_s && p.color) for (int k = 0; k < 3; ++k) p.color_s[pt * 3 + k] = p.color[pt * p.ldcolor + k];
          if (p.gcolor_s && p.gcolor) for (int k = 0; k < 3; ++k) p.gcolor_s[pt * 3 + k] = p.gcolor[pt * p.ldg + k];
        }
      }
    }
  }
  wsum = wave_sum(wsum); wmax = wave_max(wmax); dep = wave_sum(dep);
  for (int k = 0; k < 3; ++k) { col[k] = wave_sum(col[k]); gcl[k] = wave_sum(gcl[k]); }
  e0 = wave_sum(e0); e1 = wave_sum(e1);
  if (p.delta_ray_sum) { drs = wave_sum(drs); if (lane == 0 && active) p.delta_ray_sum[ray] = drs; }
  if (lane == 0 && active) {
    for (int k = 0; k < 3; ++k) {
      float cc = col[k];
      if (p.background_rgb) cc = cc + p.background_rgb[k] * (1.0f - wsum);
      p.color_fine[ray * 3 + k] = cc;
      if (p.global_color) p.global_color[ray * 3 + k] = gcl[k];
    }
    p.weight_sum[ray] = wsum; p.weight_max[ray] = wmax; p.depth[ray] = dep;
    p.s_val[ray] = 1.0f / inv_s;
    p.eik_partial[ray * 2] = e0; p.eik_partial[ray * 2 + 1] = e1;
  }
}
void be_composite_fwd(const CompositeFwd& p, cnr_stream s) {
  TimingScope ts_("composite_fwd", 2, 0, p.R, 0, 0, 0, s,
                  (double)p.R * ((4.0 + 4.0 + 12.0 + 12.0 + (p.gcolor ? 12.0 : 0.0)) * p.M + 24.0 + 12.0 * p.M + 52.0));
  hipLaunchKernelGGL(composite_fwd_kernel, dim3((unsigned)((p.R + 3) / 4)), dim3(256), 0, s, p);
  CNR_LAUNCH_CHECK("composite_fwd");
}

__global__ __launch_bounds__(256) void composite_bwd_kernel(const CompositeBwd p) {
  __shared__ float shz[4][kMaxRaySamples];
  const int lane = threadIdx.x & 63, wave = threadIdx.x >> 6;
  long ray = (long)blockIdx.x * 4 + wave;
  const bool active = ray < p.R;
  if (!active) ray = p.R - 1;
  float* zs = shz[wave];
  const int M = p.M;
  for (int i = lane; i < M; i += 64) zs[i] = p.z[ray * M + i];
  __syncthreads();
  float o[3], d[3];
  for (int c = 0; c < 3; ++c) { o[c] = p.o[ray * 3 + c]; d[c] = p.d[ray * 3 + c]; }
  const float inv_s = inv_s_of(p.variance[0]);

  RaySample q[kRayChunks];
  float T[kRayChunks], w[kRayChunks];
  float carry = 1.0f, wsum = 0.0f, wmax = -1.0f;
#pragma unroll
  for (int c = 0; c < kRayChunks; ++c) {
    T[c] = 0.f; w[c] = 0.f;
    if (c * 64 < M) {
      const int j = c * 64 + lane;
      q[c] = ray_sample(zs, j, M, p.sample_dist, o, d, p.sdf, p.g, ray * M + j, inv_s, p.cos_anneal);
      T[c] = wave_excl_cumprod(q[c].ok ? 1.0f - q[c].a.alpha + 1e-7f : 1.0f, lane, carry);
      w[c] = q[c].ok ? q[c].a.alpha * T[c] : 0.0f;
      wsum += w[c];
      if (q[c].ok) wmax = fmaxf(wmax, w[c]);
    }
  }
  wsum = wave_sum(wsum);
  wmax = wave_max(wmax);
  int amax = 1 << 30;
#pragma unroll
  for (int c = 0; c < kRayChunks; ++c)
    if (c * 64 < M && q[c].ok && w[c] == wmax && c * 64 + lane < amax) amax = c * 64 + lane;
  amax = wave_min_int(amax);

  const RayUpstream up = ray_upstream(p, ray);

  float wbar[kRayChunks], S[kRayChunks];
  float rcarry = 0.0f;
#pragma unroll
  for (int c = kRayChunks - 1; c >= 0; --c) {
    wbar[c] = 0.f; S[c] = 0.f;
    if (c * 64 < M) {
      const int j = c * 64 + lane;
      const long pt = ray * M + j;
      wbar[c] = q[c].ok ? sample_wbar(p, up, pt, q[c].z, j == amax) : 0.0f;
      const float x = wbar[c] * w[c];
      const float incl = wave_scan_incl_add_rev(x, lane);
      S[c] = rcarry + (incl - x);
      rcarry = rcarry + __shfl(incl, 0);
    }
  }

  float dinvs = 0.0f, drd[3] = {0.f, 0.f, 0.f};
#pragma unroll
  for (int c = 0; c < kRayChunks; ++c) {
    if (c * 64 < M) {
      const int j = c * 64 + lane;
      const long pt = ray * M + j;
      if (q[c].ok) dinvs += sample_backward(p, up, q[c], d, pt, inv_s, T[c], w[c], wbar[c], S[c], active, drd);
    }
  }
  dinvs = wave_sum(dinvs);
  for (int k = 0; k < 3; ++k) drd[k] = wave_sum(drd[k]);
  if (lane == 0 && active) {
    if (p.d_s_val) dinvs += -p.d_s_val[ray] / (inv_s * inv_s);
    p.dinvs_partial[ray] = dinvs;
    if (p.d_rays_d) for (int k = 0; k < 3; ++k) p.d_rays_d[ray * 3 + k] = drd[k];
  }
}
void be_composite_bwd(const CompositeBwd& p, cnr_stream s) {
// ... 391 lines not shown
```

color-neus_amd/csrc/cnr_kernels_emu.cpp:

```cpp
#include <algorithm>
#include <cstdlib>
#include <cstdio>
#include <vector>

#include "cnr_backend.h"
#include "cnr_mc_table.h"
#include "cnr_loss.h"
#include "cnr_bodies.h"

namespace cnr {

const char* be_name() { return "cpu-emu"; }
void be_split_planes(const float*, int, int, unsigned short*, float*, cnr_stream) {}
void be_split_planes_many(const SplitJob*, int, cnr_stream) {}
void be_prep_weights(const PrepWeight* p, int count, cnr_stream s) { for (int i = 0; i < count; ++i) be_prep_weight(p[i], s); }
void be_finish_weights(const FinishWeight* f, int count, cnr_stream s) { for (int i = 0; i < count; ++i) be_finish_weight(f[i], s); }
void be_timing_enable(int) {}
int be_timing_collect(KernelTiming*, int) { return 0; }
int be_check_last_error(char*, size_t) { return 0; }
void be_range_push(const char*) {}
void be_range_pop() {}
void be_memset_zero(void* p, size_t bytes, cnr_stream) { memset(p, 0, bytes); }
void be_loss_sums(const LossArgs& a, float* partial, float* sums, cnr_stream) {
  (void)partial;
// ... 332 lines not shown
    const float qx = p.query[i * 3], qy = p.query[i * 3 + 1], qz = p.query[i * 3 + 2];
    float best = INFINITY;
    int besti = -1;
    for (long j = 0; j < p.m; ++j)
      nn_update(nn_dist2(qx, qy, qz, p.target[j * 3], p.target[j * 3 + 1], p.target[j * 3 + 2]), (int)j, best, besti);
    if (besti < 0)
      for (long j = 0; j < p.m; ++j)
        nn_update_inf(nn_dist2(qx, qy, qz, p.target[j * 3], p.target[j * 3 + 1], p.target[j * 3 + 2]), (int)j, best, besti);
    p.keys[i] = nn_key(best, besti);
    nn_unpack(p.keys[i], &p.dist2[i], &p.idx[i]);
  }
}

void be_image_stats(const ImageStats& p, cnr_stream) {
  const int cs = p.cs;
  const long rowlen = (long)p.W * cs, nrows = p.planes * p.H;
  std::vector<double> part((size_t)nrows * 2);
#pragma omp parallel for schedule(static)
  for (long pr = 0; pr < nrows; ++pr) {
    const long plane = pr / p.H;
    const int r = (int)(pr - plane * p.H);
    const float* px = p.x + plane * p.H * rowlen;
    const float* py = p.y + plane * p.H * rowlen;
    double sum_d = 0.0, sum_s = 0.0;
    for (long g = 0; g < rowlen; ++g) {
      const int pix = (int)(g / cs), ch = (int)(g - (long)pix * cs);
      const long gl = (long)img_reflect(pix - 1, p.W) * cs + ch, gr = (long)img_reflect(pix + 1, p.W) * cs + ch;
      float h[5][3];
      for (int k = 0; k < 3; ++k) {
        const long row = (long)img_reflect(r - 1 + k, p.H) * rowlen;
        const float xl = px[row + gl], xc = px[row + g], xr = px[row + gr];
        const float yl = py[row + gl], yc = py[row + g], yr = py[row + gr];
        h[0][k] = img_tap3(xl, xc, xr);
        h[1][k] = img_tap3(yl, yc, yr);
        h[2][k] = img_tap3(xl * xl, xc * xc, xr * xr);
        h[3][k] = img_tap3(yl * yl, yc * yc, yr * yr);
        h[4][k] = img_tap3(xl * yl, xc * yc, xr * yr);
      }
      float m[5];
      for (int q = 0; q < 5; ++q) m[q] = img_tap3(h[q][0], h[q][1], h[q][2]);
      const float s = img_ssim(m[0], m[1], m[2], m[3], m[4]);
      const long at = (long)r * rowlen + g;
      if (p.map) p.map[plane * p.H * rowlen + at] = s;
      sum_d += (double)img_sqerr(px[at], py[at]);
      sum_s += (double)s;
    }
    part[2 * pr] = sum_d;
    part[2 * pr + 1] = sum_s;
  }
  double a = 0.0, b = 0.0;
  for (long pr = 0; pr < nrows; ++pr) { a += part[2 * pr]; b += part[2 * pr + 1]; }
  p.sums[0] = a;
  p.sums[1] = b;
}

void be_image_panel(const ImagePanel& p, cnr_stream) {
  p.keys[0] = p.keys[1] = 0xffffffffu;
  for (long i = 0; i < (long)p.H * p.W; ++i) {
    const float d = p.depth[i];
    if (d == d) {
      const unsigned k = img_depth_key(d);
      p.keys[0] = std::min(p.keys[0], k);
      p.keys[1] = std::min(p.keys[1], ~k);
    }
  }
  float vmin, vmax;
  img_depth_range(p.keys, &vmin, &vmax);
  p.range[0] = vmin;
  p.range[1] = vmax;
  const int rowb = p.nsec * 3 * p.W;
#pragma omp parallel for schedule(static)
  for (int row = 0; row < p.H; ++row)
    for (int col = 0; col < rowb; ++col) p.panel[(long)row * rowb + col] = img_panel_byte(p, row, col, vmin, vmax);
}

void be_gen_rays_bwd(const GenRaysBwd& q, cnr_stream) {
  for (int cam = 0; cam < q.f.n_cams; ++cam) {
    double acc[14] = {0};
    for (long i = 0; i < q.f.n; ++i) {
      int c; float out[14];
      body_gen_rays_bwd1(q, i, &c, out);
      if (c == cam) for (int k = 0; k < 14; ++k) acc[k] += out[k];
    }
    for (int k = 0; k < 12; ++k) q.d_c2w[cam * 16 + k] = (float)acc[k];
    for (int k = 12; k < 16; ++k) q.d_c2w[cam * 16 + k] = 0.0f;
    q.d_focal_partial[cam * 2] = (float)acc[12]; q.d_focal_partial[cam * 2 + 1] = (float)acc[13];
  }
  for (int j = 0; j < 2; ++j) {
    float s = 0.0f;
    for (int c = 0; c < q.f.n_cams; ++c) s += q.d_focal_partial[c * 2 + j];
    q.d_focal[j] = s;
  }
}

void be_pixel_table(const PixelTable& t, cnr_stream) {
#pragma omp parallel for schedule(static)
  for (int n = 0; n < t.n_images; ++n) {
    const float* m = t.masks + (long)n * t.hw;
    int* row = t.order + (long)n * t.hw;
    int f = 0, g = 0;
    for (long i = 0; i < t.hw; ++i) f += pix_class(m[i]) == 1;
    for (long i = 0, a = 0; i < t.hw; ++i) {
      const int c = pix_class(m[i]);
      if (c == 1) row[a++] = (int)i;
      else if (c == 2) row[f + g++] = (int)i;
    }
    t.fg_count[n] = f; t.bg_count[n] = g;
  }
}

void be_choose_pixels(const PixelDraw& p, cnr_stream) {
  const PixKey k = pix_key(p.state[0], p.state[1]);
  std::vector<unsigned> pf(p.B), pb(p.B);
  std::vector<int> cams(p.B);
  unsigned F = 0, G = 0;
  for (int b = 0; b < p.B; ++b) {
    unsigned f, g;
    cams[b] = pix_slot_image(p, k, b);
    pix_slot_counts(p, cams[b], &f, &g);
    pf[b] = F += f; pb[b] = G += g;
    if (p.cams_out) p.cams_out[b] = cams[b];
  }
  const unsigned want = (unsigned)pix_want_fg(p), kfg = want < F ? want : F;
  const unsigned long long m = (unsigned long long)p.n - kfg;
  if (p.counts_out) { p.counts_out[0] = p.order ? (int)kfg : 0; p.counts_out[1] = p.order ? (int)(m < G ? m : G) : 0; }
#pragma omp parallel for schedule(static)
  for (long j = 0; j < p.n; ++j) {
    if (p.order) pix_draw_masked(p, k, j, pf.data(), pb.data(), cams.data(), kfg);
    else p.idx[j] = pix_draw_replace(p, k, j);
    if (p.t_rand) p.t_rand[j] = pix_jitter(k, j);
  }
  p.state[1] = (long)((unsigned long long)p.state[1] + 1ull);
}

void be_clip_adam(const AdamArgs& a, cnr_stream) {
  for (int k = 0; k < a.count; ++k) {
    const AdamTensor& t = a.t[k];
    float coef = 1.0f;
    if (a.max_norm > 0.0f) {
      float tot = 0.0f;
      for (long c0 = 0; c0 < t.n; c0 += kAdamChunk) {
        float ss = 0.0f;
        for (long i = c0; i < t.n && i < c0 + kAdamChunk; ++i) ss += t.g[i] * t.g[i];
        tot += ss;
      }
      coef = adam_clip_coef(tot, a.max_norm);
    }
    for (long i = 0; i < t.n; ++i) adam_update1(a, t.w + i, t.g[i] * coef, a.m + t.off + i, a.v + t.off + i);
  }
}

void be_pack_frags_many(const PackJob*, int, cnr_stream) {}
bool be_sdf_value_chain(const SdfValueChain&, cnr_stream) { return false; }
bool be_relu_chain_fwd(const ReluChainFwd&, cnr_stream) { return false; }
bool be_relu_chain_fwd_enabled() { return false; }
bool be_sdf_save_chain(const SdfSaveChain&, cnr_stream) { return false; }
bool be_sweep0_ok(const LayerGemm&) { return false; }
int be_sweep0_slots(long) { return 0; }
void be_sweep0_dw(const LayerGemm&, float*, int, cnr_stream) {}
bool be_narrow_bwd_ok(const NarrowBwd&) { return false; }
int be_narrow_bwd_slots(long) { return 0; }
void be_narrow_bwd(const NarrowBwd&, cnr_stream) {}

void be_upsample(const UpSample& p, cnr_stream) {
#pragma omp parallel for
  for (long ray = 0; ray < p.R; ++ray) {
    const int n = p.n, nsec = n - 1;
    const float* z = p.z + ray * p.ldz;
    const float* s = p.w_in ? nullptr : p.sdf + ray * p.lds;
    std::vector<float> rad(n), cs(n), w(n), cdf(n);
    float T = 1.0f, total = 0.0f;
    if (p.w_in) {
      for (int i = 0; i < nsec; ++i) { w[i] = p.w_in[ray * nsec + i] + 1e-5f; total += w[i]; }
    } else {
    for (int i = 0; i < n; ++i) rad[i] = ray_radius(p.o + ray * 3, p.d + ray * 3, z[i]);
    for (int i = 0; i < nsec; ++i) cs[i] = upsample_slope(s[i], s[i + 1], z[i], z[i + 1]);
    for (int i = 0; i < nsec; ++i) {
      float c = upsample_cos(i > 0 ? cs[i - 1] : 0.0f, cs[i], rad[i], rad[i + 1]);
      float a = upsample_alpha(s[i], s[i + 1], z[i], z[i + 1], c, p.inv_s);
      w[i] = a * T + 1e-5f;
      T = T * (1.0f - a + 1e-7f);
      total += w[i];
    }
    }
    cdf[0] = 0.0f;
    float run = 0.0f;
    for (int i = 0; i < nsec; ++i) { run += w[i] / total; cdf[i + 1] = run; }
    for (int k = 0; k < p.m; ++k) {
      float u = p.u_in ? p.u_in[ray * p.m + k] : linspace_at(0.5f / (float)p.m, 1.0f - 0.5f / (float)p.m, p.m, k);
      p.new_z[ray * p.m + k] = invert_cdf(cdf.data(), z, n, u);
    }
  }
}

void be_merge(const MergeZ& p, cnr_stream) {
#pragma omp parallel for
  for (long ray = 0; ray < p.R; ++ray) {
    std::vector<float> z(p.z + ray * p.ldz, p.z + ray * p.ldz + p.n), s(p.n, 0.0f);
    if (p.new_sdf) s.assign(p.sdf_in + ray * p.lds_in, p.sdf_in + ray * p.lds_in + p.n);
    const float* nz = p.new_z + ray * p.m;
    const float* ns = p.new_sdf ? p.new_sdf + ray * p.m : nz;
    merge_samples(z.data(), s.data(), p.n, nz, ns, p.m, 0, 1, [&](int at, float zv, float sv) {
      p.z[ray * p.ldz + at] = zv;
      if (p.new_sdf) p.sdf_out[ray * p.lds_out + at] = sv;
    });
  }
}

void be_composite_fwd(const CompositeFwd& p, cnr_stream) {
  const float inv_s = inv_s_of(p.variance[0]);
#pragma omp parallel for
  for (long ray = 0; ray < p.R; ++ray) {
    const int M = p.M;
    const float* z = p.z + ray * M;
    float T = 1.0f, wsum = 0.f, wmax = -1.f, dep = 0.f, col[3] = {0, 0, 0}, gcl[3] = {0, 0, 0}, e0 = 0.f, e1 = 0.f;
    for (int j = 0; j < M; ++j) {
      long pt = ray * M + j;
      RaySample q = ray_sample(z, j, M, p.sample_dist, p.o + ray * 3, p.d + ray * 3, p.sdf, p.g, pt, inv_s, p.cos_anneal);
      float w = q.a.alpha * T;
      T = T * (1.0f - q.a.alpha + 1e-7f);
      wsum += w; wmax = std::max(wmax, w); dep += w * q.z;
      if (p.color) for (int k = 0; k < 3; ++k) col[k] += w * p.color[pt * p.ldcolor + k];
      if (p.gcolor) for (int k = 0; k < 3; ++k) gcl[k] += w * p.gcolor[pt * p.ldg + k];
      e0 += q.relax * (q.gn - 1.0f) * (q.gn - 1.0f); e1 += q.relax;
      p.weights[pt] = w; p.cdf_fine[pt] = q.a.pc; p.inside_sphere[pt] = q.inside;
      if (p.sdf_s) p.sdf_s[pt] = p.sdf[pt];
      if (p.color_s && p.color) for (int k = 0; k < 3; ++k) p.color_s[pt * 3 + k] = p.color[pt * p.ldcolor + k];
      if (p.gcolor_s && p.gcolor) for (int k = 0; k < 3; ++k) p.gcolor_s[pt * 3 + k] = p.gcolor[pt * p.ldg + k];
    }
    for (int k = 0; k < 3; ++k) {
      float cc = col[k];
      if (p.background_rgb) cc = cc + p.background_rgb[k] * (1.0f - wsum);
      p.color_fine[ray * 3 + k] = cc;
      if (p.global_color) p.global_color[ray * 3 + k] = gcl[k];
    }
    p.weight_sum[ray] = wsum; p.weight_max[ray] = wmax; p.depth[ray] = dep; p.s_val[ray] = 1.0f / inv_s;
    p.eik_partial[ray * 2] = e0; p.eik_partial[ray * 2 + 1] = e1;
    if (p.delta && p.delta_ray_sum) {
      float drs = 0.f;
      for (long i = ray * M * 3; i < (ray + 1) * M * 3; ++i) drs += p.delta[i];
      p.delta_ray_sum[ray] = drs;
    }
  }
}

void be_composite_bwd(const CompositeBwd& p, cnr_stream) {
  const float inv_s = inv_s_of(p.variance[0]);
#pragma omp parallel for
  for (long ray = 0; ray < p.R; ++ray) {
    const int M = p.M;
    const float* z = p.z + ray * M;
    const float* d = p.d + ray * 3;
    std::vector<RaySample> q(M);
    std::vector<float> T(M), w(M), wbar(M), S(M);
    float t = 1.0f, wmax = -1.0f;
    int amax = 0;
    for (int j = 0; j < M; ++j) {
      q[j] = ray_sample(z, j, M, p.sample_dist, p.o + ray * 3, d, p.sdf, p.g, ray * M + j, inv_s, p.cos_anneal);
      T[j] = t; w[j] = q[j].a.alpha * t; t = t * (1.0f - q[j].a.alpha + 1e-7f);
      if (w[j] > wmax) { wmax = w[j]; amax = j; }
    }
    const RayUpstream up = ray_upstream(p, ray);
    for (int j = 0; j < M; ++j) wbar[j] = sample_wbar(p, up, ray * M + j, q[j].z, j == amax);
    float run = 0.0f;
    for (int j = M - 1; j >= 0; --j) { S[j] = run; run += wbar[j] * w[j]; }
    float dinvs = 0.0f, drd[3] = {0, 0, 0};
    for (int j = 0; j < M; ++j) dinvs += sample_backward(p, up, q[j], d, ray * M + j, inv_s, T[j], w[j], wbar[j], S[j], true, drd);
    if (p.d_s_val) dinvs += -p.d_s_val[ray] / (inv_s * inv_s);
    p.dinvs_partial[ray] = dinvs;
    if (p.d_rays_d) for (int k = 0; k < 3; ++k) p.d_rays_d[ray * 3 + k] = drd[k];
  }
}

void be_rays_grad_finish(const RaysGradFinish& p, cnr_stream) {
  const int npe = p.multires_view > 0 ? 3 + 6 * p.multires_view : 3;
  for (long ray = 0; ray < p.R; ++ray) {
    float so[3] = {0, 0, 0}, sd[3] = {0, 0, 0}, spe[27];
    for (int q = 0; q < 27; ++q) spe[q] = 0.0f;
    const float* dr = p.d + ray * 3;
    float snear = 0.0f, sfar = 0.0f;
    std::vector<float> dmid(p.M);
    for (int j = 0; j < p.M; ++j) {
      long pt = ray * p.M + j;
      float z0 = p.z[pt];
      float dist = j + 1 < p.M ? p.z[pt + 1] - z0 : p.sample_dist;
      float mid = z0 + dist * 0.5f;
      dmid[j] = 0.0f;
      for (int k = 0; k < 3; ++k) { float pb = p.pbar[pt * 4 + k]; so[k] += pb; sd[k] += pb * mid; dmid[j] += pb * dr[k]; }
      for (int q = 0; q < npe; ++q) {
        if (p.daux_dir_c) spe[q] += p.daux_dir_c[pt * p.lddir + 6 + q];
        if (p.daux_dir_r) spe[q] += p.daux_dir_r[pt * p.lddir + 6 + q];
      }
    }
    if (p.dz_parts && p.d_near && p.d_far) {
      for (int j = 0; j < p.M; ++j) {
        long pt = ray * p.M + j;
        float dz = p.dz_parts[pt * 2] + dmid[j];
        if (j + 1 < p.M) dz -= p.dz_parts[pt * 2 + 1] + 0.5f * dmid[j];
        if (j > 0) dz += p.dz_parts[(pt - 1) * 2 + 1] + 0.5f * dmid[j - 1];
        float lin = linspace_at(0.0f, 1.0f, p.M, j);
        snear += dz * (1.0f - lin);
        sfar += dz * lin;
      }
      p.d_near[ray] = snear; p.d_far[ray] = sfar;
    }
    if (!(p.d_o && p.d_d)) continue;
// ... 53 lines not shown
```

color-neus_amd/csrc/cnr_plan.cpp:

```cpp
#include <cmath>
#include <cstdarg>
#include <cstdio>
#include <cstdlib>
#include <string>
#include <vector>

#include "../../include/colorneus_render.h"
#include "cnr_backend.h"

namespace cnr {

const DebugFlags& debug_flags() {
  static const DebugFlags flags = [] {
    DebugFlags d;
    struct B { const char* name; bool DebugFlags::*m; };
    struct I { const char* name; int DebugFlags::*m; };
    static const B bools[] = {
        {"CNR_NO_FUSED", &DebugFlags::no_fused}, {"CNR_NO_CHAIN_FWD", &DebugFlags::no_chain_fwd}, {"CNR_NO_CHAIN_SDF", &DebugFlags::no_chain_sdf},
        {"CNR_NO_FDW", &DebugFlags::no_fdw}, {"CNR_FDW_SPLIT", &DebugFlags::fdw_split},
        {"CNR_NO_TOP_FUSE", &DebugFlags::no_top_fuse}, {"CNR_NO_HEAD_BWD", &DebugFlags::no_head_bwd}, {"CNR_NO_HEAD_FWD", &DebugFlags::no_head_fwd},
        {"CNR_NO_STRIP_BWD", &DebugFlags::no_strip_bwd}, {"CNR_NO_SAMPLER_FUSE", &DebugFlags::no_sampler_fuse}, {"CNR_NO_SWEEP0", &DebugFlags::no_sweep0},
        {"CNR_NO_NARROW_BWD", &DebugFlags::no_narrow_bwd}, {"CNR_NO_NARROW_DX", &DebugFlags::no_narrow_dx}, {"CNR_DISABLE_WS", &DebugFlags::disable_ws},
        {"CNR_WS_GENERIC", &DebugFlags::ws_generic}, {"CNR_WS_NOSTREAM", &DebugFlags::ws_nostream}, {"CNR_DW_FP32", &DebugFlags::dw_fp32},
        {"CNR_DW_BF16", &DebugFlags::dw_bf16}, {"CNR_ROCTX", &DebugFlags::roctx}};
    static const I ints[] = {
        {"CNR_WS_SERP", &DebugFlags::ws_serp},
#ifdef CNR_TUNING
        {"CNR_WS_KINDS", &DebugFlags::ws_kinds}, {"CNR_WS_MINW", &DebugFlags::ws_minw}, {"CNR_WS_WGS", &DebugFlags::ws_wgs}, {"CNR_WS_MINTPW", &DebugFlags::ws_mintpw},
        {"CNR_CHAIN_WGS", &DebugFlags::chain_wgs}, {"CNR_CHAIN_SHAPE", &DebugFlags::chain_shape}, {"CNR_CHAIN_FWD_RT", &DebugFlags::chain_fwd_rt},
        {"CNR_FDW_DEEP", &DebugFlags::fdw_deep}, {"CNR_FDW_NOREV", &DebugFlags::fdw_norev}, {"CNR_FDW_REVMODE", &DebugFlags::fdw_revmode},
        {"CNR_FDW_DBG", &DebugFlags::fdw_dbg}, {"CNR_CHAIN_FWD_DBG", &DebugFlags::chain_fwd_dbg},
#endif
    };
    auto env = [](const char* name) { return getenv(name); };
    const char* v;
    for (const B& b : bools) d.*(b.m) = env(b.name) != nullptr;
    for (const I& i : ints) if ((v = env(i.name)) != nullptr) d.*(i.m) = *v ? atoi(v) : 1;
#ifdef CNR_TUNING
    if ((v = env("CNR_CHAIN_SDF_MAXP")) != nullptr) d.chain_sdf_maxp = atol(v);
#endif
    return d;
  }();
  return flags;
}

static thread_local std::string g_err;
static int fail(const char* fmt, ...) {
  char buf[512];
  va_list ap;
  va_start(ap, fmt);
  vsnprintf(buf, sizeof buf, fmt, ap);
  va_end(ap);
  g_err = buf;
  return -1;
}

struct Lin {
  int n = 0, k_ref = 0, k_int = 0;
  int nseg = 0;
  Segment seg[4];
  int ldw = 0, npad = 0, ldwt = 0, kpad = 0;
  int wpad = 0;
  bool wn = false;
  int row_rot = 0;
  int p_b = -1, p_g = -1, p_v = -1;
  float *W = nullptr, *Wt = nullptr, *bias = nullptr;
  unsigned short *Wp = nullptr, *Wtp = nullptr;
  unsigned short* Wf = nullptr;
  float *Wps = nullptr, *Wtps = nullptr;
  std::string name;
  void finish_dims() {
    ldw = round_up(k_int, 16);
    npad = round_up(n, 32);
    wpad = npad;
    ldwt = round_up(n, 16);
    kpad = round_up(k_int, 32);
  }
  size_t bytes() const { return ((size_t)wpad * ldw + (size_t)kpad * ldwt + wpad) * sizeof(float); }
};

struct ParamInfo { std::string name; int rows, cols; };

struct Model {
  cnr_config c;
  int S, I, M, K;
  int emb;
  int Hs, L;
  int F;
  int Hc, NC;
  int Hr, NR;
  int nv;
  int mv;
  int naux;
  bool has_relight;
  std::vector<Lin> sdf, col, rel;
  std::vector<ParamInfo> params;
  int p_variance = -1;
  bool skip(int l) const { return (c.sdf_skip_mask >> l) & 1; }
};

static void identity_seg(Lin& l) {
  l.k_int = l.k_ref;
  l.nseg = 1;
  l.seg[0] = {0, 0, l.k_ref};
}

static int add_linear_params(Model& m, Lin& l, const std::string& prefix, bool wn) {
  l.name = prefix;
  l.wn = wn;
  l.p_b = (int)m.params.size();
  m.params.push_back({prefix + ".bias", l.n, 1});
  if (wn) {
    l.p_g = (int)m.params.size();
    m.params.push_back({prefix + ".weight_g", l.n, 1});
    l.p_v = (int)m.params.size();
    m.params.push_back({prefix + ".weight_v", l.n, l.k_ref});
  } else {
    l.p_v = (int)m.params.size();
    m.params.push_back({prefix + ".weight", l.n, l.k_ref});
  }
  return 0;
}

static int build_model(const cnr_config* cfg, Model& m) {
  if (!cfg) return fail("null config");
  m.c = *cfg;
  const cnr_config& c = m.c;
  m.S = c.n_samples; m.I = c.n_importance; m.M = m.S + m.I; m.K = c.up_sample_steps;
  if (m.S < 2 || m.M > kMaxRaySamples) return fail("n_samples + n_importance must be in [2, %d]", kMaxRaySamples);
  if (m.I > 0 && (m.K < 1 || m.I % m.K != 0 || m.I / m.K > 64)) return fail("n_importance must be a multiple of up_sample_steps (<= 64 new samples per step)");
  if (c.sdf_multires < 1 || c.sdf_multires > 6) return fail("sdf multires must be in [1,6]");
  m.emb = 3 + 6 * c.sdf_multires;
  m.Hs = c.sdf_d_hidden; m.L = c.sdf_n_layers; m.F = c.sdf_d_out - 1;
  if (m.Hs < 48 || m.Hs > 256 || m.Hs % 16) return fail("sdf d_hidden must be a multiple of 16 in [48,256]");
  if (m.L < 1 || m.L > kMaxLayers) return fail("sdf n_layers out of range");
  if (m.F < 1 || m.F > 256 || m.F != c.col_d_feature) return fail("sdf d_out - 1 must equal colour d_feature (<= 256)");
  if (c.sdf_skip_mask & 1) return fail("skip connection at layer 0 is not supported");
  if ((c.sdf_skip_mask >> m.L) & 1) return fail("skip connection at the top layer is not supported");
  m.has_relight = c.type == 1;
  m.Hc = c.col_d_hidden; m.NC = c.col_n_layers + 1;
  if (m.Hc < 16 || m.Hc > 256 || m.Hc % 16 || c.col_n_layers < 1 || c.col_n_layers >= kMaxLayers) return fail("colour d_hidden must be a multiple of 16 in [16,256]");
  const bool col_view = c.col_mode != 1;
  if (col_view && c.col_multires_view > 4) return fail("colour multires_view must be <= 4");
  int mv_c = col_view ? c.col_multires_view : -1, mv_r = m.has_relight ? c.rel_multires_view : -1;
  if (mv_c >= 0 && mv_r >= 0 && mv_c != mv_r) return fail("colour and relight multires_view must match when both use view directions");
  m.mv = mv_c >= 0 ? mv_c : (mv_r >= 0 ? mv_r : 0);
  if (m.mv > 4) return fail("multires_view must be <= 4");
  m.nv = (mv_c >= 0 || mv_r >= 0) ? (m.mv > 0 ? 3 + 6 * m.mv : 3) : 0;
  m.naux = 6 + m.nv;
  if (m.naux > kAux) return fail("aux input too wide");

  m.sdf.resize(m.L + 1);
  int prev = m.emb;
  for (int l = 0; l <= m.L; ++l) {
    Lin& q = m.sdf[l];
    q.k_ref = (l == 0) ? m.emb : m.Hs;
    int out = (l == m.L) ? c.sdf_d_out : m.Hs;
    if (l < m.L && m.skip(l + 1)) out = m.Hs - m.emb;
    q.n = out;
    if (l > 0 && !m.skip(l) && prev != q.k_ref) return fail("inconsistent SDF dims");
    if (l > 0 && m.skip(l) && prev + m.emb != q.k_ref) return fail("inconsistent SDF skip dims");
    identity_seg(q);
    if (l == m.L) q.row_rot = 1;
    q.finish_dims();
    if (l < m.L && m.skip(l + 1) && round_up(q.n + m.emb, 32) <= 256) q.wpad = round_up(q.n + m.emb, 32);
    add_linear_params(m, q, "sdf_network.lin" + std::to_string(l), c.sdf_weight_norm != 0);
    prev = out;
  }
  m.p_variance = (int)m.params.size();
  m.params.push_back({"deviation_network.variance", 1, 1});
  m.col.resize(m.NC);
  for (int l = 0; l < m.NC; ++l) {
    Lin& q = m.col[l];
    q.n = (l == m.NC - 1) ? 3 : m.Hc;
// ... 257 lines not shown
  place_row_scales(x.rsX1, m.L, 1, m.L, P, a);
  place_row_scales(x.rsC, m.NC, 0, m.NC - 1, P, a);
  place_row_scales(x.rsR, m.NR, 0, m.NR - 1, P, a);
  place_slack(a);
}

struct Bwd {
  float *ZTOP, *gbar_a, *dtop, *gc_a, *gc_b, *dctop, *dinvs, *drd_alpha, *dAUXc, *dAUXr, *gbar_t, *cbar, *ebar0, *ebars, *pbar, *dzparts;
  std::vector<float*> D, DC, VB, Z2;
  std::vector<float*> rsX0, rsY1;
  float* rsD;
  float* partial;
  size_t partial_floats, partial_off;
  std::vector<FinishWeight> pending;
  int nchunk; long chunk_pts;
  int fslots;
  int cap_slots;
  int cu_slots;
  int ldtop;
};

static int fdw_slots(long P) {
  long s = round_up((int)((P / 32 + 3) / 4), 8);
  if (s < 8) s = 8;
  if (s > kFdwSlots) s = kFdwSlots;
  return (int)s;
}

static int region_slots(const Lin& q, const Bwd& b) {
  const int narrow = (b.nchunk > b.cu_slots ? b.nchunk : b.cu_slots) + b.cu_slots;
  return (q.k_int <= 48 && b.cap_slots < narrow) ? narrow : b.cap_slots;
}

static bool head_bwd_static_ok(const Lin& q, int ldaux) {
  const bool off = debug_flags().no_head_bwd;
  return !off && q.n <= 4 && q.k_int == 256 && q.ldw == 256 && (ldaux & 3) == 0;
}

static int dw_chunks(long P) {
  const long nch = P / 128;
  return nch < 1 ? 1 : nch > 256 ? 256 : (int)nch;
}

static void bwd_slots(long P, Bwd& b) {
  b.nchunk = dw_chunks(P);
  b.chunk_pts = round_up((int)((P + b.nchunk - 1) / b.nchunk), 16);
  b.fslots = fdw_slots(P);
  b.cap_slots = b.fslots + (b.nchunk > b.fslots ? b.nchunk : b.fslots);
  const long ntiles = (P + 31) / 32, tpw = (ntiles + 255) / 256;
  b.cu_slots = ntiles > 0 ? (int)((ntiles + tpw - 1) / tpw) : 0;
}

static void place_sdf_seeds(long P, bool grad_path, const Ctx& x, Arena& a, Bwd& b) {
  b.ZTOP = a.f((size_t)P * x.ldztop);
  b.gbar_a = grad_path ? a.f((size_t)P * 4) : nullptr;
}
static void place_sdf_cotangents(long P, bool grad_path, Arena& a, Bwd& b) {
  b.gbar_t = grad_path ? a.f((size_t)P * 4) : nullptr;
  b.cbar = grad_path ? a.f((size_t)P * kEmb) : nullptr;
  b.ebar0 = a.f((size_t)P * kEmb);
  b.ebars = a.f((size_t)P * kEmb);
  b.pbar = a.f((size_t)P * 4);
}
static void place_sdf_sweeps(const Model& m, long P, bool grad_path, Arena& a, Bwd& b) {
  b.VB.assign(m.L, nullptr); b.Z2.resize(m.L);
  for (int l = 0; l < m.L; ++l) { if (grad_path) b.VB[l] = a.f((size_t)P * m.Hs); b.Z2[l] = a.f((size_t)P * m.Hs); }
}
static void place_dw_pool(std::initializer_list<const std::vector<Lin>*> stacks, long P, Arena& a, Bwd& b) {
  bwd_slots(P, b);
  size_t tot = 0;
  for (auto* st : stacks)
    for (auto& q : *st) { const int cap = region_slots(q, b); tot += round_up_sz((size_t)cap * q.npad * q.ldw, 64) + round_up_sz((size_t)cap * q.npad, 64); }
  b.partial_floats = tot;
  b.partial = a.f(tot);
  b.partial_off = 0;
  b.pending.clear();
}
static void place_sdf_bwd_row_scales(const Model& m, long P, bool grad_path, Arena& a, Bwd& b) {
  place_row_scales(b.rsX0, m.L + 1, 1, m.L + 1, P, a);
  place_row_scales(b.rsY1, m.L + 1, 1, grad_path ? m.L : 1, P, a);
}

static void layout_bwd(const Model& m, long R, const Ctx& x, Arena& a, Bwd& b) {
  const long P = R * m.M;
  place_sdf_seeds(P, true, x, a, b);
  const bool packed = m.NC >= 2 && head_bwd_static_ok(m.col[m.NC - 1], m.Hc) && (m.Hc & 3) == 0 &&
                      (!m.has_relight || (m.NR >= 2 && head_bwd_static_ok(m.rel[m.NR], hr_ld(m, x, m.NR - 1)) && (m.Hr & 3) == 0));
  b.ldtop = packed ? 4 : kTop;
  b.dtop = a.f((size_t)P * b.ldtop);
  b.gc_a = a.f((size_t)P * b.ldtop);
  b.gc_b = a.f((size_t)P * 4);
  b.dctop = a.f((size_t)P * b.ldtop);
  b.dinvs = a.f(R);
  b.drd_alpha = a.f((size_t)R * 3);
  b.dAUXc = a.f((size_t)P * kAux);
  b.dAUXr = a.f((size_t)P * kAux);
  place_sdf_cotangents(P, true, a, b);
  b.dzparts = m.I == 0 ? a.f((size_t)P * 2) : nullptr;
  place_sdf_sweeps(m, P, true, a, b);
  b.D.resize(m.NR);
  b.DC.resize(m.NC > 0 ? m.NC - 1 : 0);
  const int nshare = m.NR + (int)b.DC.size();
  const bool share = (m.NR == 0 || m.Hr == m.Hs) && m.Hc == m.Hs && nshare <= 2 * m.L;
  auto shared = [&](int k) { return (k & 1) ? b.Z2[k >> 1] : b.VB[k >> 1]; };
  for (int i = 0; i < m.NR; ++i) b.D[i] = share ? shared(i) : a.f((size_t)P * m.Hr);
  for (int l = 0; l + 1 < m.NC; ++l) b.DC[l] = share ? shared(m.NR + l) : a.f((size_t)P * m.Hc);
  place_dw_pool({&m.sdf, &m.col, &m.rel}, P, a, b);
  place_sdf_bwd_row_scales(m, P, true, a, b);
  b.rsD = a.f(P);
  place_slack(a);
}

static void prep_all(Model& m, const float* const* params, cnr_stream s, bool sdf_only = false) {
  std::vector<PrepWeight> pw;
  std::vector<SplitJob> sj;
  auto prep = [&](Lin& q) {
    PrepWeight p;
    p.g = q.p_g >= 0 ? params[q.p_g] : nullptr;
    p.v = params[q.p_v];
    p.b = params[q.p_b];
    p.n = q.n; p.k_ref = q.k_ref;
    p.nseg = q.nseg;
    for (int i = 0; i < q.nseg; ++i) p.seg[i] = q.seg[i];
    p.W = q.W; p.ldw = q.ldw; p.npad = q.wpad;
    p.Wt = q.Wt; p.ldwt = q.ldwt; p.kpad = q.kpad;
    p.bias = q.bias; p.row_rot = q.row_rot;
    pw.push_back(p);
    sj.push_back(SplitJob{q.W, q.wpad, q.ldw, q.Wp, q.Wps});
    sj.push_back(SplitJob{q.Wt, q.kpad, q.ldwt, q.Wtp, q.Wtps});
  };
  for (auto& q : m.sdf) prep(q);
  if (!sdf_only) for (auto& q : m.col) prep(q);
  if (!sdf_only) for (auto& q : m.rel) prep(q);
  be_prep_weights(pw.data(), (int)pw.size(), s);
  be_split_planes_many(sj.data(), (int)sj.size(), s);
  std::vector<PackJob> pj;
  for (auto& q : m.sdf) if (q.Wf) pj.push_back(PackJob{q.Wp, (long)q.wpad * q.ldw, q.wpad, q.ldw, q.Wf});
  if (!sdf_only) for (auto& q : m.col) if (q.Wf && q.n == 256) pj.push_back(PackJob{q.Wp, (long)q.wpad * q.ldw, q.wpad, q.ldw, q.Wf});
  if (!sdf_only) for (auto& q : m.rel) if (q.Wf && q.n == 256) pj.push_back(PackJob{q.Wp, (long)q.wpad * q.ldw, q.wpad, q.ldw, q.Wf});
  be_pack_frags_many(pj.data(), (int)pj.size(), s);
}

static View sdf_input_view(const Model& m, int l, const float* E, const float* const* Z) {
  View v;
  if (l == 0) {
    v.kind = VK_DIRECT; v.a = E; v.lda = kEmb;
  } else {
    v.kind = VK_SOFTPLUS; v.a = Z[l - 1]; v.lda = m.Hs;
    if (m.skip(l)) { v.math_split = m.sdf[l - 1].n; v.scale = kInvSqrt2; }
  }
  return v;
}

static bool sdf_value_chain_fused(const Model& m, long n, const float* E, float* sdf_out, float top_scale, cnr_stream s) {
  if (m.Hs != 256 || m.L < 1) return false;
  if (m.skip(m.L) || m.sdf[m.L - 1].n != 256 || m.sdf[m.L].ldw < 256) return false;
  SdfValueChain c;
  c.E = E; c.P = n; c.nl = m.L; c.skip_mask = m.c.sdf_skip_mask; c.emb = m.emb;
  for (int l = 0; l < m.L; ++l) {
    const Lin& q = m.sdf[l];
    if (!q.Wf) return false;
    c.lay[l] = FusedLayer{q.Wf, q.Wps, q.bias, q.ldw, q.n};
  }
  const Lin& t = m.sdf[m.L];
  c.wtop = t.W + (long)m.F * t.ldw; c.btop = t.bias + m.F; c.top_scale = top_scale; c.sdf_out = sdf_out;
  return be_sdf_value_chain(c, s);
}

static bool sdf_save_chain_fused(const Model& m, long n, const float* E, float* const* Z, float* sdf_out, float* feat_out, int ld_feat,
                                 float top_scale, float* const* rs, cnr_stream s) {
  if (m.Hs != 256 || m.L < 1 || m.F != 256 || m.L + 1 > kMaxLayers) return false;
  if (m.skip(m.L) || m.sdf[m.L - 1].n != 256 || m.sdf[m.L].ldw != 256 || !m.sdf[m.L].Wf) return false;
  const long maxp = debug_flags().chain_sdf_maxp;
  if (n > maxp) return false;
  SdfSaveChain c;
  c.v.E = E; c.v.P = n; c.v.nl = m.L; c.v.skip_mask = m.c.sdf_skip_mask; c.v.emb = m.emb;
  for (int l = 0; l < m.L; ++l) {
    const Lin& q = m.sdf[l];
    if (!q.Wf || !Z[l]) return false;
    c.v.lay[l] = FusedLayer{q.Wf, q.Wps, q.bias, q.ldw, q.n};
    c.Z[l] = Z[l];
  }
  c.ldz = m.Hs;
  for (int l = 1; l <= m.L; ++l) c.rs[l] = rs ? rs[l] : nullptr;
  const Lin& t = m.sdf[m.L];
  c.top = FusedLayer{t.Wf, t.Wps, t.bias, t.ldw, m.F};
  c.feat = feat_out; c.ld_feat = ld_feat;
  c.v.wtop = t.W + (long)m.F * t.ldw; c.v.btop = t.bias + m.F; c.v.top_scale = top_scale; c.v.sdf_out = sdf_out;
  return be_sdf_save_chain(c, s);
}

static void sdf_chain(const Model& m, long n, const float* E, float* const* Z, float* sdf_out, float* feat_out, int ld_feat,
                      float top_scale, cnr_stream s, float* const* rs = nullptr ) {
  if (!feat_out && !rs && sdf_value_chain_fused(m, n, E, sdf_out, top_scale, s)) return;
  if (feat_out && sdf_save_chain_fused(m, n, E, Z, sdf_out, feat_out, ld_feat, top_scale, rs, s)) return;
  for (int l = 0; l <= m.L; ++l) {
    const Lin& q = m.sdf[l];
    LayerGemm g = fwd_gemm(q, n);
    g.A = sdf_input_view(m, l, E, Z);
    if (rs && (l < m.L || feat_out)) g.rs_out = rs[l];
    if (l < m.L) {
      g.E.kind = EK_STORE; g.E.n_out = q.n; g.E.bias = q.bias; g.E.o1 = Z[l]; g.E.ld1 = m.Hs;
      if (m.skip(l + 1)) { g.E.tail_src = E; g.E.ld_tail = kEmb; g.E.tail_n = m.emb; }
    } else if (feat_out) {
      g.N = m.F;
      g.E.kind = EK_SDF_TOP; g.E.n_out = m.F; g.E.bias = q.bias; g.E.scale = top_scale; g.E.split = m.F;
      g.E.o1 = feat_out; g.E.ld1 = ld_feat; g.E.o2 = sdf_out;
      g.dot_w = q.W + (long)m.F * q.ldw; g.dot_bias = q.bias + m.F; g.dot_scale = top_scale; g.dot_out = sdf_out;
    } else {
      g.W = q.W + (long)m.F * q.ldw; g.N = 1; g.Wp = nullptr;
      g.E.kind = EK_STORE; g.E.n_out = 1; g.E.bias = q.bias + m.F; g.E.scale = top_scale; g.E.o1 = sdf_out; g.E.ld1 = 1;
    }
    be_layer_gemm(g, s);
  }
}

static void run_sampler(const Model& m, const cnr_render_inputs* in, float* z, Ctx& x, cnr_stream s) {
  const long R = in->n_rays;
  const float scale = m.c.sdf_scale;
  EmbedZ e;
  e.o = in->rays_o; e.d = in->rays_d; e.R = R; e.m = m.S; e.z = z; e.ldz = m.M; e.make_z = 1;
  e.near_ = in->near_; e.far_ = in->far_; e.t_rand = in->t_rand; e.scale = scale; e.multires = m.c.sdf_multires; e.E = x.sE;
  be_embed_z(e, s);
  if (m.I <= 0) return;
  float* Zp[kMaxLayers];
  for (int l = 0; l < m.L; ++l) Zp[l] = (l & 1) ? x.sZb : x.sZa;
  sdf_chain(m, R * m.S, x.sE, Zp, x.s_sdf0, nullptr, 0, 1.0f / scale, s);
  const int mnew = m.I / m.K;
  int n = m.S;
  const bool unfused = debug_flags().no_sampler_fuse;
  MergeZ prev;
  for (int i = 0; i < m.K; ++i) {
    const bool last = i + 1 == m.K;
    UpSample u;
    u.o = in->rays_o; u.d = in->rays_d; u.R = R; u.z = z; u.ldz = m.M;
    u.sdf = i == 0 ? x.s_sdf0 : x.s_sdf; u.lds = i == 0 ? m.S : m.M; u.n = n; u.m = mnew;
    u.inv_s = 64.0f * (float)(1 << i); u.new_z = x.s_newz;
    EmbedZ e2 = e;
    e2.m = mnew; e2.z = x.s_newz; e2.ldz = mnew; e2.make_z = 0;
    if (!unfused && mnew <= 64) {
      SamplerStep st;
      st.do_merge = i > 0; st.g = prev; st.u = u; st.do_embed = !last; st.E = x.sE; st.scale = scale; st.multires = m.c.sdf_multires;
      be_sampler_step(st, s);
    } else {
      if (i > 0) be_merge(prev, s);
      be_upsample(u, s);
      if (!last) be_embed_z(e2, s);
    }
    if (!last) sdf_chain(m, R * mnew, x.sE, Zp, x.s_newsdf, nullptr, 0, 1.0f / scale, s);
    MergeZ g;
    g.R = R; g.z = z; g.ldz = m.M; g.sdf_in = i == 0 ? x.s_sdf0 : x.s_sdf; g.lds_in = i == 0 ? m.S : m.M;
    g.sdf_out = x.s_sdf; g.lds_out = m.M; g.n = n; g.new_z = x.s_newz; g.new_sdf = last ? nullptr : x.s_newsdf; g.m = mnew;
    if (last) be_merge(g, s);
    prev = g;
    n += mnew;
  }
}

static int skip_off(const Model& m) {
  for (int l = 1; l < m.L; ++l) if (m.skip(l)) return m.sdf[l - 1].n & 3;
  return 0;
}

static void sdf_grad_chain(const Model& m, long P, const float* E, const float* const* Z, float* const* V, float* CE0, float* CES,
                           cnr_stream s, float* const* rs = nullptr ) {
  const float inv_scale = 1.0f / m.c.sdf_scale;
  bool ces_written = false;
  for (int l = m.L - 1; l >= 0; --l) {
    const Lin& q = m.sdf[l];
    if (l >= 1 && m.skip(l) && V[l - 1] && round_up(m.sdf[l - 1].n, 16) > m.sdf[l - 1].n)
      be_zero_cols(V[l - 1], m.Hs, m.sdf[l - 1].n, round_up(m.sdf[l - 1].n, 16), P, s);
    LayerGemm g = bwd_gemm(q, P);
    g.A.a = Z[l]; g.A.lda = m.Hs;
    if (l == m.L - 1) { g.A.kind = VK_SIGMUL_ROW; g.A.b = m.sdf[m.L].W + (long)m.F * m.sdf[m.L].ldw; g.A.scale = inv_scale; }
    else { g.A.kind = VK_SIGMUL; g.A.b = V[l]; g.A.ldb = m.Hs; }
    if (rs) g.rs_out = rs[l];
    if (l == 0) {
      g.E.kind = EK_STORE; g.E.n_out = m.emb; g.E.o1 = CE0; g.E.ld1 = kEmb;
      NarrowBwd nb;
      nb.X = Z[0]; nb.ldx = m.Hs; nb.Xb = g.A.b; nb.ldxb = g.A.ldb; nb.P = P;
      narrow_bwd_weights(nb, q);
      nb.dx = CE0; nb.lddx = kEmb; nb.ndx = m.emb;
      if (g.A.kind == VK_SIGMUL && g.A.scale == 1.0f && g.rs_out == nullptr && q.n == 256 && m.Hs == 256 && be_narrow_bwd_ok(nb)) { be_narrow_bwd(nb, s); continue; }
    } else if (m.skip(l)) {
      g.E.kind = EK_SPLIT; g.E.n_out = q.k_int; g.E.scale = kInvSqrt2; g.E.split = m.sdf[l - 1].n;
      g.E.o1 = V[l - 1]; g.E.ld1 = m.Hs; g.E.o2 = CES; g.E.ld2 = kEmb; g.E.o2_off = skip_off(m);
      g.E.o2_acc = ces_written; ces_written = true;
    } else {
      g.E.kind = EK_STORE; g.E.n_out = q.k_int; g.E.o1 = V[l - 1]; g.E.ld1 = m.Hs;
    }
    be_layer_gemm(g, s);
  }
}

static int top_skip(const Model& m) {
  for (int l = m.L - 1; l >= 1; --l) if (m.skip(l)) return l;
  return -1;
}
static bool has_skip(const Model& m) {
  for (int l = 1; l < m.L; ++l) if (m.skip(l)) return true;
  return false;
}

static void embed_points(const Model& m, const float* pts, long n, float* E, float* AUX, cnr_stream s, const float* bmin = nullptr,
                         const float* bmax = nullptr, int res = 0, long start = 0) {
  EmbedPts ep;
  ep.pts = pts; ep.n = n; ep.res = res; ep.start = start;
  for (int c = 0; c < 3; ++c) { ep.bmin[c] = bmin ? bmin[c] : 0.f; ep.bmax[c] = bmax ? bmax[c] : 0.f; }
  ep.scale = m.c.sdf_scale; ep.multires = m.c.sdf_multires; ep.E = E; ep.AUX = AUX;
  be_embed_pts(ep, s);
}

struct PointOpts {
  bool grad = true;
  float* grad_out = nullptr;
  bool aux_to_featx = true;
  int neg_g_as_view = 0;
  int multires_view = 0;
};
static void point_pipeline(const Model& m, long P, const Ctx& x, const PointOpts& o, cnr_stream s) {
  const float scale = m.c.sdf_scale;
  { RangeScope r_("sdf value chain"); sdf_chain(m, P, x.E, x.Z.data(), x.sdf, x.featx, x.ldfx, 1.0f / scale, s, x.rsY.data()); }
  if (!o.grad) return;
  { RangeScope r_("sdf gradient chain"); sdf_grad_chain(m, P, x.E, x.Z.data(), x.V.data(), x.CE0, x.CES, s, x.rsX1.data()); }
  GradFinish gf;
  gf.featx = o.aux_to_featx ? x.featx : nullptr; gf.ldfx = o.aux_to_featx ? x.ldfx : 0; gf.F = m.F;
  gf.P = P; gf.E = x.E; gf.ce0 = x.CE0; gf.ces = has_skip(m) ? x.CES + skip_off(m) : nullptr; gf.scale = scale; gf.multires = m.c.sdf_multires;
  gf.grad_out = o.grad_out; gf.AUX = x.AUX; gf.neg_g_as_view = o.neg_g_as_view; gf.multires_view = o.multires_view;
  be_grad_finish(gf, s);
}

static View color_input_view(const Model& m, int l, const Ctx& x) {
  View v;
  v.kind = VK_DIRECT;
  if (l == 0) { v.a = x.featx; v.lda = x.ldfx; }
  else { v.a = x.HC[l - 1]; v.lda = m.Hc; }
  return v;
}

static bool head_fwd(const Lin& q, const LayerGemm& g, cnr_stream s) {
  const bool off = debug_flags().no_head_fwd;
  if (off || q.n > 4 || q.k_int != 256 || g.A.kind != VK_DIRECT || g.A.scale != 1.0f || (g.A.lda & 3) != 0 || (q.ldw & 3) != 0 || g.E.tail_src != nullptr) return false;
  HeadFwd h;
  h.h = g.A.a; h.ldh = g.A.lda; h.P = g.P; h.P_dev = g.P_dev; h.W = q.W; h.ldw = q.ldw; h.n = q.n; h.E = g.E;
  be_head_fwd(h, s);
  return true;
}

static void color_chain(const Model& m, long P, const Ctx& x, cnr_stream s, const int* P_dev = nullptr) {
  for (int l = 0; l < m.NC; ++l) {
    const Lin& q = m.col[l];
    LayerGemm g = fwd_gemm(q, P);
    g.A = color_input_view(m, l, x); g.P_dev = P_dev;
    g.E.bias = q.bias; g.E.n_out = q.n;
    if (!P_dev && (size_t)l < x.rsC.size()) g.rs_out = x.rsC[l];
    if (l + 1 < m.NC) { g.E.kind = EK_RELU; g.E.o1 = x.HC[l]; g.E.ld1 = m.Hc; }
    else {
      g.E.kind = m.c.col_squeeze_out ? EK_SIGMOID : EK_LINEAR_SIG; g.E.o1 = x.gcol; g.E.ld1 = 4;
      if (m.has_relight) { g.E.o2 = x.hry; g.E.ld2 = x.ldy; g.E.o2_off = m.Hr; }
    }
    if (l + 1 == m.NC && head_fwd(q, g, s)) continue;
    be_layer_gemm(g, s);
  }
}

static View relight_input_view(const Model& m, int i , const Ctx& x) {
  View v;
  v.kind = VK_DIRECT;
  if (i < 0) { v.a = x.AUX; v.lda = kAux; }
  else { v.a = x.HR[i]; v.lda = hr_ld(m, x, i); }
  return v;
}

static void relight_chain(const Model& m, long P, const Ctx& x, float* delta_out, cnr_stream s, const int* P_dev = nullptr) {
  {
    const Lin& q = m.rel[0];
    LayerGemm g = fwd_gemm(q, P);
    g.A = relight_input_view(m, -1, x); g.P_dev = P_dev;
    g.E.kind = EK_RELU; g.E.bias = q.bias; g.E.n_out = q.n; g.E.o1 = x.HR[0]; g.E.ld1 = hr_ld(m, x, 0);
    be_layer_gemm(g, s);
  }
  for (int i = 0; i < m.NR; ++i) {
    const Lin& q = m.rel[1 + i];
    LayerGemm g = fwd_gemm(q, P);
    g.A = relight_input_view(m, i, x); g.P_dev = P_dev;
    g.E.bias = q.bias; g.E.n_out = q.n;
    if (!P_dev && (size_t)i < x.rsR.size()) g.rs_out = x.rsR[i];
    if (i + 1 < m.NR) { g.E.kind = EK_RELU; g.E.o1 = x.HR[i + 1]; g.E.ld1 = hr_ld(m, x, i + 1); }
    else {
      g.E.kind = EK_RELIGHT_TOP; g.E.o1 = delta_out; g.E.ld1 = 3; g.E.o2 = x.relit; g.E.ld2 = 4;
      g.E.aux = x.gcol; g.E.ldaux = 4; g.E.inv_sigmoid = m.c.rel_inv_sigmoid;
    }
    if (i + 1 == m.NR && head_fwd(q, g, s)) continue;
    be_layer_gemm(g, s);
  }
}

static bool relu_chains_fused(const Model& m, long P, const Ctx& x, float* delta_out, cnr_stream s, const int* P_dev = nullptr, const int* row_idx = nullptr) {
  if (!relu_fused_shapes(m)) return false;
  ReluChainFwd c;
  c.P = P; c.P_dev = P_dev; c.row_idx = row_idx;
  auto hidden_ok = [](const Lin& q, int k_lo, int k_hi) { return q.n == 256 && q.Wf && q.wpad >= 256 && q.k_int >= k_lo && q.k_int <= k_hi; };
  auto head_ok = [](const Lin& q) { return q.n >= 1 && q.n <= 3 && q.k_int == 256 && (q.ldw & 3) == 0; };
  auto fill = [](ChainFwdStep& st, const Lin& q) { st.Wf = q.Wf; st.wsc = q.Wps; st.bias = q.bias; st.nkb_w = q.ldw / 16; };
  int n = 0;
  for (int l = 0; l + 1 < m.NC; ++l) {
    const Lin& q = m.col[l];
    ChainFwdStep& st = c.st[n++];
    fill(st, q);
    if (l == 0) {
      if (!hidden_ok(q, 257, 304) || q.ldw > x.ldfx) return false;
      st.in = x.featx; st.ld_in = x.ldfx; st.nkb_main = 16; st.nkb_x = q.ldw / 16 - 16; st.x_src = 1;
    } else {
      if (!hidden_ok(q, 256, 256) || q.ldw != 256) return false;
      st.nkb_main = 16;
    }
    st.save = x.HC[l]; st.ld_save = m.Hc;
    st.rs_in = (size_t)l < x.rsC.size() ? x.rsC[l] : nullptr;
  }
  c.st[n - 1].head = 1;
  {
    const Lin& q = m.col[m.NC - 1];
    if (!head_ok(q)) return false;
    c.col_head = ChainFwdHead{q.W, q.ldw, q.bias, q.n};
    c.col_squeeze = m.c.col_squeeze_out ? 1 : 0;
    c.gcol = x.gcol;
    if (m.has_relight && x.hry) { c.rgb_tail = x.hry + m.Hr; c.ld_tail = x.ldy; }
  }
  if (m.has_relight) {
    if (m.Hr != 256 || m.NR < 2) return false;
    const int y = m.c.rel_y_in_layer - 1;
    if (y < 1 || y > m.NR - 2) return false;
    {
      const Lin& q = m.rel[0];
      if (q.n != 256 || !q.Wf || q.ldw > kAux || q.ldw < 16) return false;
      ChainFwdStep& st = c.st[n++];
      fill(st, q);
      st.in = x.AUX; st.ld_in = kAux; st.nkb_main = q.ldw / 16;
      st.save = x.HR[0]; st.ld_save = hr_ld(m, x, 0);
    }
    for (int i = 0; i + 1 < m.NR; ++i) {
      const Lin& q = m.rel[1 + i];
      ChainFwdStep& st = c.st[n++];
      fill(st, q);
      st.nkb_main = 16;
      if (i == y) {
        if (!hidden_ok(q, 257, 259) || q.ldw != 272) return false;
        st.nkb_x = 1; st.x_src = 2;
      } else if (!hidden_ok(q, 256, 256) || q.ldw != 256) return false;
      st.save = x.HR[i + 1]; st.ld_save = hr_ld(m, x, i + 1);
      st.rs_in = (size_t)i < x.rsR.size() ? x.rsR[i] : nullptr;
    }
    c.st[n - 1].head = 2;
    const Lin& q = m.rel[m.NR];
    if (!head_ok(q) || q.n != m.col[m.NC - 1].n) return false;
    c.rel_head = ChainFwdHead{q.W, q.ldw, q.bias, q.n};
    c.inv_sigmoid = m.c.rel_inv_sigmoid;
    c.delta = delta_out; c.relit = x.relit;
  }
  c.nsteps = n;
  return be_relu_chain_fwd(c, s);
}

static void prune_select(const CompositeFwd& cf, float eps, const Ctx& x, PruneGather pg, cnr_stream s) {
  CompositeFwd cw = cf;
  cw.color = nullptr; cw.gcolor = nullptr; cw.delta = nullptr; cw.delta_ray_sum = nullptr;
  be_composite_fwd(cw, s);
  PruneCount pc; pc.weights = cf.weights; pc.R = cf.R; pc.M = cf.M; pc.eps = eps; pc.counts = x.p_counts;
  be_prune_count(pc, s);
  PruneScan ps; ps.counts = x.p_counts; ps.R = cf.R; ps.offsets = x.p_offsets;
  be_prune_scan(ps, s);
  pg.weights = cf.weights; pg.R = cf.R; pg.M = cf.M; pg.eps = eps; pg.offsets = x.p_offsets; pg.idx = x.p_idx;
  pg.featx = x.featx; pg.ldfx = x.ldfx; pg.aux = x.AUX;
  be_prune_gather(pg, s);
}

static int check_backend(const char* what) {
  char msg[256];
  if (be_check_last_error(msg, sizeof msg) != 0) return fail("%s: %s", what, msg);
  return 0;
}

static int render_forward(const cnr_config* cfg, const float* const* params, const cnr_render_inputs* in,
                          const cnr_render_outputs* out, void* ctx, size_t ctx_bytes, cnr_stream s, bool infer = false) {
  Model m;
  if (build_model(cfg, m)) return -1;
  if (!params || !in || !out || !ctx) return fail("null argument");
  const long R = in->n_rays;
  if (R <= 0) return fail("n_rays must be positive");
  Ctx x;
  auto layout = [&](Arena& a) { if (infer) layout_ctx_infer(m, R, a, x); else layout_ctx(m, R, a, x); };
  if (layout_checked(infer ? "scratch buffer" : "context buffer", ctx, ctx_bytes, layout)) return -1;
  if (!out->z_vals || !out->weights || !out->color_fine || !out->cdf_fine || !out->inside_sphere ||
      !out->weight_sum || !out->weight_max || !out->depth || !out->s_val || !out->gradient_error)
    return fail("missing output buffer");
  if (m.has_relight && !out->global_color) return fail("Color_NeuS needs a global_color buffer");
  if (m.has_relight && !out->delta_relight && !out->delta_relight_ray_sum) return fail("Color_NeuS needs delta_relight or delta_relight_ray_sum");
  if (in->prune_eps > 0.0f && m.has_relight && !out->delta_relight && !x.infer_fused) return fail("prune_eps > 0 needs the delta_relight buffer");
  if (in->prune_eps > 0.0f && out->delta_relight_ray_sum) return fail("prune_eps > 0 (inference) does not go with the loss-only training outputs");
  float* const g_out = out->gradients ? out->gradients : x.gbuf;
  float* const delta_out = m.has_relight ? (out->delta_relight ? out->delta_relight : x.delta_s) : nullptr;
  const long P = R * m.M;
  const float scale = m.c.sdf_scale;

  RangeScope range_fwd("cnr_render_forward");
  { RangeScope r_("weights"); prep_all(m, params, s); }
  if (in->z_vals_override) {
    if (in->z_vals_override != out->z_vals) return fail("z_vals_override must alias outputs.z_vals (copy it there first)");
  } else {
    RangeScope r_("sampler");
    run_sampler(m, in, out->z_vals, x, s);
  }
  FineSetup fs;
  fs.o = in->rays_o; fs.d = in->rays_d; fs.z = out->z_vals; fs.R = R; fs.M = m.M; fs.sample_dist = 2.0f / (float)m.S;
  fs.scale = scale; fs.multires = m.c.sdf_multires; fs.multires_view = m.mv; fs.E = x.E; fs.AUX = x.AUX;
  be_fine_setup(fs, s);
  PointOpts po;
  po.grad_out = g_out; po.multires_view = m.mv;
  point_pipeline(m, P, x, po, s);
  CompositeFwd cf;
  cf.o = in->rays_o; cf.d = in->rays_d; cf.z = out->z_vals; cf.R = R; cf.M = m.M; cf.sample_dist = 2.0f / (float)m.S;
  cf.sdf = x.sdf; cf.g = g_out;
  cf.color = m.has_relight ? x.relit : x.gcol; cf.ldcolor = 4;
  cf.gcolor = m.has_relight ? x.gcol : nullptr; cf.ldg = 4;
  cf.variance = params[m.p_variance]; cf.cos_anneal = in->cos_anneal_ratio; cf.background_rgb = in->background_rgb;
  cf.color_fine = out->color_fine; cf.s_val = out->s_val; cf.cdf_fine = out->cdf_fine; cf.weight_sum = out->weight_sum;
  cf.weight_max = out->weight_max; cf.weights = out->weights; cf.inside_sphere = out->inside_sphere; cf.depth = out->depth;
  cf.global_color = m.has_relight ? out->global_color : nullptr; cf.eik_partial = x.eik_partial;
  cf.sdf_s = out->sdf_samples; cf.color_s = out->color_samples; cf.gcolor_s = m.has_relight ? out->global_color_samples : nullptr;
  if (m.has_relight && out->delta_relight_ray_sum) { cf.delta = delta_out; cf.delta_ray_sum = out->delta_relight_ray_sum; }

  if (in->prune_eps > 0.0f && x.infer_fused) {
    PruneGather pg;
    pg.featx_c = nullptr; pg.aux_c = nullptr;
    pg.zero_gcol = x.gcol; pg.zero_relit = m.has_relight ? x.relit : nullptr; pg.zero_delta = delta_out;
    prune_select(cf, in->prune_eps, x, pg, s);
    if (!relu_chains_fused(m, P, x, delta_out, s, x.p_offsets + R, x.p_idx)) return fail("render_forward_only: the chain-fused colour / relight launch refused its shapes");
  } else if (in->prune_eps > 0.0f) {
    be_memset_zero(x.gcol, (size_t)P * 4 * sizeof(float), s);
    be_memset_zero(x.relit, (size_t)P * 4 * sizeof(float), s);
    if (m.has_relight) be_memset_zero(out->delta_relight, (size_t)P * 3 * sizeof(float), s);
    PruneGather pg;
    pg.featx_c = x.featx_c; pg.aux_c = x.aux_c;
    prune_select(cf, in->prune_eps, x, pg, s);
    Ctx xc = x;
    xc.featx = x.featx_c; xc.AUX = x.aux_c; xc.gcol = x.gcol_c; xc.relit = x.relit_c;
    const int* kept = x.p_offsets + R;
    color_chain(m, P, xc, s, kept);
    if (m.has_relight) relight_chain(m, P, xc, x.delta_c, s, kept);
    PruneScatter sc; sc.P = P; sc.count = kept; sc.idx = x.p_idx; sc.gcol_c = x.gcol_c; sc.relit_c = m.has_relight ? x.relit_c : nullptr;
    sc.delta_c = m.has_relight ? x.delta_c : nullptr; sc.gcol = x.gcol; sc.relit = m.has_relight ? x.relit : nullptr;
    sc.delta = m.has_relight ? out->delta_relight : nullptr;
    be_prune_scatter(sc, s);
  } else {
    RangeScope r_("colour + relight chains");
    if (!relu_chains_fused(m, P, x, delta_out, s)) {
      if (x.infer_fused) return fail("render_forward_only: the chain-fused colour / relight launch refused its shapes");
      color_chain(m, P, x, s);
      if (m.has_relight) relight_chain(m, P, x, delta_out, s);
    }
  }
  RangeScope r_comp("compositor");
  be_composite_fwd(cf, s);
  ReduceEik re;
  re.partial = x.eik_partial; re.R = R; re.sums = x.eik_sums; re.sums_out = out->eik_sums; re.gradient_error = out->gradient_error;
  be_reduce_eik(re, s);
  return check_backend(infer ? "render_forward_only" : "render_forward");
}

struct DwRegion { float* part = nullptr; float* csum = nullptr; };
static DwRegion take_region(const Lin& q, Bwd& b) {
  DwRegion r;
  const int cap = region_slots(q, b);
  r.part = b.partial + b.partial_off;
  b.partial_off += round_up_sz((size_t)cap * q.npad * q.ldw, 64);
  r.csum = b.partial + b.partial_off;
  b.partial_off += round_up_sz((size_t)cap * q.npad, 64);
  return r;
}
static void finish_region(const Lin& q, const DwRegion& r, int nslots, int ncolsum, Bwd& b, const float* const* params, float* const* dparams) {
  FinishWeight f;
  f.partial = r.part; f.nchunk = nslots; f.npad = q.npad; f.ldk = q.ldw; f.colsum = ncolsum > 0 ? r.csum : nullptr; f.ncolsum = ncolsum;
  f.g = q.p_g >= 0 ? params[q.p_g] : nullptr; f.v = params[q.p_v];
  f.n = q.n; f.k_ref = q.k_ref; f.nseg = q.nseg;
  for (int i = 0; i < q.nseg; ++i) f.seg[i] = q.seg[i];
  f.dg = q.p_g >= 0 ? dparams[q.p_g] : nullptr; f.dv = dparams[q.p_v]; f.db = dparams[q.p_b]; f.row_rot = q.row_rot;
  b.pending.push_back(f);
}
static void dw_into_region(const Lin& q, DwGemm& g, const DwRegion& r, int slot0, int nchunk, long P, bool with_bias, cnr_stream s, int kmain = 0) {
  with_bias = with_bias && slot0 == 0;
  g.N = q.n; g.K = kmain > 0 ? kmain : q.k_int;
  g.nchunk = nchunk; g.chunk_pts = round_up((int)((P + nchunk - 1) / nchunk), 16);
  g.partial = r.part + (size_t)slot0 * q.npad * q.ldw; g.Npad = q.npad; g.ldk = q.ldw; g.colsum = with_bias ? r.csum : nullptr;
  const int need = (g.npairs == 2 && g.X[1].kind == VK_CONST_COL0) ? 1 : g.npairs;
  bool scaled = q.n > 32 && q.k_int > 64;
  for (int i = 0; i < need; ++i) scaled = scaled && g.sx[i] && g.sy[i];
  g.split_f16 = scaled;
  be_dw_gemm(g, s);
}
static void fused_into_region(const Lin& q, const LayerGemm& g, DwGemm& d, const float* se, int transposed, const DwRegion& r, int slot0, Bwd& b,
                              bool with_bias, cnr_stream s, int kmain = 0, const DwFuse* xrow = nullptr, int rev = 0) {
  with_bias = with_bias && slot0 == 0 && !transposed;
  DwFuse f;
  if (xrow) f = *xrow;
  const bool no_rev = debug_flags().fdw_norev != 0;
  const int rev_mode = debug_flags().fdw_revmode;
  f.rev = no_rev ? 0 : (rev_mode == 1 ? !rev : (rev_mode == 2 ? 1 : rev));
  f.se = se; f.partial = r.part + (size_t)slot0 * q.npad * q.ldw; f.Npad = q.npad; f.ldk = q.ldw; f.colsum = with_bias ? r.csum : nullptr;
  f.transposed = transposed; f.nslots = b.fslots;
  d.npairs = 1; d.P = g.P; d.N = q.n; d.K = kmain > 0 ? kmain : q.k_int; d.nchunk = b.fslots; d.chunk_pts = round_up((int)((g.P + b.fslots - 1) / b.fslots), 16);
  d.partial = f.partial; d.Npad = q.npad; d.ldk = q.ldw; d.colsum = f.colsum;
  d.split_f16 = q.n > 32 && q.k_int > 64 && d.sx[0] && d.sy[0];
  be_layer_dw_gemm(g, d, f, s);
}

static bool strip_bwd_ok(const Lin& q, const LayerGemm& g, const DwGemm& d) {
  const bool off = debug_flags().no_strip_bwd;
  const int nt = q.k_int - 256;
  return !off && q.n == 256 && nt >= 1 && nt <= 8 && q.ldw >= 256 + nt && g.A.kind == VK_DIRECT && (g.A.lda & 3) == 0 && g.A.scale == 1.0f &&
         (g.E.kind == EK_RELU_MASK || g.E.kind == EK_SPLIT) && g.E.split == 256 && g.E.bias == nullptr &&
         d.Y[0].kind == VK_DIRECT && d.Y[0].scale == 1.0f && d.npairs == 1;
}
static StripBwd take_strips(const Lin& q, LayerGemm& g, const DwGemm& d, const DwRegion& r, const Bwd& b) {
  StripBwd sb;
  sb.dout = g.A.a; sb.ldo = g.A.lda; sb.P = g.P; sb.nt = q.k_int - 256; sb.Wt = q.Wt; sb.ldwt = q.ldwt;
  sb.tail = g.E.o2 ? g.E.o2 + (g.E.kind == EK_SPLIT ? g.E.o2_off : 0) : nullptr; sb.ldt = g.E.ld2;
  sb.tail_scale = g.E.kind == EK_SPLIT ? g.E.scale : 1.0f;
  sb.y = d.Y[0].a + 256; sb.ldy = d.Y[0].lda;
  sb.partial = r.part; sb.npad = q.npad; sb.ldk = q.ldw; sb.nslots = b.nchunk;
  g.N = 256; g.E.n_out = 256; g.E.o2 = nullptr;
  return sb;
}
static void strip_columns_of_last_finish(Bwd& b) { b.pending.back().col_hi = 256; b.pending.back().nchunk_hi = b.nchunk; }

static bool head_bwd_ok(const Lin& q, const LayerGemm& g) {
  return head_bwd_static_ok(q, g.E.ldaux) && (g.E.ld1 & 3) == 0 && g.A.kind == VK_DIRECT && (g.A.lda & 3) == 0 && g.E.kind == EK_RELU_MASK &&
         g.E.split >= q.k_int && g.E.aux != nullptr && g.E.o1 != nullptr;
}
static void run_head_bwd(const Lin& q, const LayerGemm& g, Bwd& b, const float* const* params, float* const* dparams, cnr_stream s) {
  const DwRegion r = take_region(q, b);
  HeadBwd h;
  h.dtop = g.A.a; h.ldt = g.A.lda; h.aux = g.E.aux; h.ldaux = g.E.ldaux; h.W = q.W; h.ldw = q.ldw; h.n = q.n; h.K = q.k_int; h.P = g.P;
  h.dout = g.E.o1; h.ldo = g.E.ld1; h.partial = r.part; h.colsum = r.csum; h.npad = q.npad; h.ldk = q.ldw; h.nslots = b.nchunk;
  be_head_bwd(h, s);
  finish_region(q, r, b.nchunk, b.nchunk, b, params, dparams);
}

static void run_dw(const Model& m, const Lin& q, DwGemm& g, Bwd& b, const float* const* params, float* const* dparams,
                   bool with_bias, cnr_stream s) {
  const DwRegion r = take_region(q, b);
  dw_into_region(q, g, r, 0, b.nchunk, g.P, with_bias, s);
  finish_region(q, r, b.nchunk, with_bias ? b.nchunk : 0, b, params, dparams);
  (void)m;
}

static void flush_dw(Bwd& b, cnr_stream s) {
  if (!b.pending.empty()) be_finish_weights(b.pending.data(), (int)b.pending.size(), s);
  b.pending.clear();
}

static int stack_layer_bwd(const Lin& q, LayerGemm& g, DwGemm& d, const float* rs_in, int rev, bool head, Bwd& b, const float* const* params,
                           float* const* dP, cnr_stream s) {
  if (head_bwd_ok(q, g)) { run_head_bwd(q, g, b, params, dP, s); return 0; }
  if (head && b.ldtop != kTop) return fail("render_backward: packed head cotangents without the streaming head kernel");
  const DwRegion r = take_region(q, b);
  const bool strips = strip_bwd_ok(q, g, d);
  StripBwd sb;
  if (strips) sb = take_strips(q, g, d, r, b);
  const int kmain = strips ? 256 : 0;
// ... 1537 lines not shown
```

Before: 188,000 rays/s.

## Fuse hierarchical sampler step and fine setup into SDF value chain kernel tail

Adds a templated tail to the fused SDF value-chain kernel. After each tile's SDFs are computed they are kept in LDS, and the kernel runs the per-ray upsampling step (merge, alpha, PDF/CDF, invert) and optionally the final merge plus fine-sample embedding directly. This removes separate sampler_step and fine_setup launches and the global round trip of new SDF values. The cost is more LDS per workgroup, which can lower occupancy, and extra per-ray work serialized inside the chain kernel.

```diff
diff --git a/color-neus_amd/csrc/cnr_backend.h b/color-neus_amd/csrc/cnr_backend.h
--- a/color-neus_amd/csrc/cnr_backend.h
+++ b/color-neus_amd/csrc/cnr_backend.h
@@ -200,6 +200,15 @@
   float* sdf_out;
 };
 bool be_sdf_value_chain(const SdfValueChain& c, cnr_stream s);
+struct SamplerTail {
+  SamplerStep st;
+  int npr = 0;
+  int row_ld = 0;
+  int do_final = 0, do_fine = 0;
+  MergeZ fin; FineSetup fs;
+  int wave_floats = 0, top_off = 0, batch = 1;
+};
+bool be_sdf_value_chain_tail(const SdfValueChain& c, const SamplerTail& t, cnr_stream s);
 struct SdfSaveChain {
   SdfValueChain v;
   float* Z[kMaxLayers] = {};
diff --git a/color-neus_amd/csrc/cnr_bodies.h b/color-neus_amd/csrc/cnr_bodies.h
--- a/color-neus_amd/csrc/cnr_bodies.h
+++ b/color-neus_amd/csrc/cnr_bodies.h
@@ -45,11 +45,11 @@
 }
 CNR_HD void body_embed_pts(const EmbedPts& p, long i) { body_embed_pts_rows(p, i, p.E + i * kEmb, p.AUX ? p.AUX + i * kAux : nullptr); }
 
-CNR_HD void body_fine_setup_rows(const FineSetup& p, long pt, float* e, float* a) {
-  long r = pt / p.M;
-  int j = (int)(pt - r * p.M);
-  float z0 = p.z[r * p.M + j];
-  float dist = (j + 1 < p.M) ? p.z[r * p.M + j + 1] - z0 : p.sample_dist;
+CNR_HD void fine_section(const float* zrow, int j, int M, float sample_dist, float& z0, float& dist) {
+  z0 = zrow[j];
+  dist = (j + 1 < M) ? zrow[j + 1] - z0 : sample_dist;
+}
+CNR_HD void fine_setup_row(const FineSetup& p, long r, float z0, float dist, float* e, float* a) {
   float mid = z0 + dist * 0.5f;
   float pp[3], x[3], dd[3];
   for (int c = 0; c < 3; ++c) {
@@ -57,12 +57,23 @@
     pp[c] = p.o[r * 3 + c] + dd[c] * mid;
     x[c] = pp[c] * p.scale;
   }
-  for (int c = 0; c < kEmb; ++c) e[c] = 0.0f;
-  pe_row(x, p.multires, e);
-  for (int c = 0; c < kAux; ++c) a[c] = 0.0f;
-  a[0] = pp[0]; a[1] = pp[1]; a[2] = pp[2];
-  if (p.multires_view > 0) pe_row(dd, p.multires_view, a + 6);
-  else { a[6] = dd[0]; a[7] = dd[1]; a[8] = dd[2]; }
+  if (e) {
+    for (int c = 0; c < kEmb; ++c) e[c] = 0.0f;
+    pe_row(x, p.multires, e);
+  }
+  if (a) {
+    for (int c = 0; c < kAux; ++c) a[c] = 0.0f;
+    a[0] = pp[0]; a[1] = pp[1]; a[2] = pp[2];
+    if (p.multires_view > 0) pe_row(dd, p.multires_view, a + 6);
+    else { a[6] = dd[0]; a[7] = dd[1]; a[8] = dd[2]; }
+  }
+}
+CNR_HD void body_fine_setup_rows(const FineSetup& p, long pt, float* e, float* a) {
+  long r = pt / p.M;
+  int j = (int)(pt - r * p.M);
+  float z0, dist;
+  fine_section(p.z + r * p.M, j, p.M, p.sample_dist, z0, dist);
+  fine_setup_row(p, r, z0, dist, e, a);
 }
 CNR_HD void body_fine_setup(const FineSetup& p, long pt) { body_fine_setup_rows(p, pt, p.E + pt * kEmb, p.AUX + pt * kAux); }
 
diff --git a/color-neus_amd/csrc/cnr_chain.hip b/color-neus_amd/csrc/cnr_chain.hip
--- a/color-neus_amd/csrc/cnr_chain.hip
+++ b/color-neus_amd/csrc/cnr_chain.hip
@@ -7,6 +7,7 @@
 #include "cnr_hip_util.h"
 #include "cnr_gemm_int.h"
 #include "cnr_chain_util.h"
+#include "cnr_ray_steps.h"
 
 namespace cnr {
 
@@ -42,8 +43,9 @@
   CNR_LAUNCH_CHECK("pack_frags");
 }
 
-template <int RT, int CB>
-__global__ __launch_bounds__(512 / CB, 2 / (3 - CB) + 0) void sdf_value_chain_kernel(const SdfValueChain c) {
+struct NoTail {};
+template <int RT, int CB, int TAIL = 0>
+__global__ __launch_bounds__(512 / CB, 2 / (3 - CB) + 0) void sdf_value_chain_kernel(const SdfValueChain c, const typename std::conditional<TAIL != 0, SamplerTail, NoTail>::type tl) {
   constexpr int WAVES = 8 / CB, THREADS = 64 * WAVES;
   constexpr int T = 32 * RT;
   constexpr int APLANE = T * CH_ALD;
@@ -52,6 +54,9 @@
   float* pm = rs + T;
   float* cwb = pm + T * 8;
   float* wtop = cwb + 1024;
+  if constexpr (TAIL != 0) wtop = reinterpret_cast<float*>(smem + tl.top_off);
+  [[maybe_unused]] float* tsdf = wtop + 256;
+  [[maybe_unused]] int held = 0;
   const int tid0 = threadIdx.x, wave = __builtin_amdgcn_readfirstlane(tid0 >> 6);
   const long ntiles = (c.P + T - 1) / T;
 #define VC_LANE_INDICES                                                                      \
@@ -223,23 +228,67 @@
 #pragma unroll
           for (int w = 1; w < 8; ++w) sum += pm[row * 8 + w];
           const long grow = tile * T + row;
-          if (grow < c.P) c.sdf_out[grow] = (sum + c.btop[0]) * c.top_scale;
+          const float sdf = (sum + c.btop[0]) * c.top_scale;
+          if (grow < c.P) c.sdf_out[grow] = sdf;
+          if constexpr (TAIL != 0) tsdf[held * T + row] = sdf;
         }
       }
       lds_barrier();
     }
+    if constexpr (TAIL != 0) {
+      ++held;
+      if (held == tl.batch || tile + gridDim.x >= ntiles) {
+        const int lane = tid0 & 63;
+        const int npr = tl.npr, rpt = T / npr, nq = held * rpt;
+        const long R = tl.st.u.R;
+        float* wrows = reinterpret_cast<float*>(smem) + wave * tl.wave_floats;
+        const RayRows rr = ray_rows(wrows, tl.row_ld, wrows + kRayRows * tl.row_ld);
+        float* stage = wrows + kRayRows * tl.row_ld + kRayNewRows * 64;
+        auto sync = [] { asm volatile("s_waitcnt lgkmcnt(0)" ::: "memory"); };
+        for (int q0 = 0; q0 < nq; q0 += WAVES) {
+          const int q = q0 + wave < nq ? q0 + wave : nq - 1;
+          const int b = q / rpt, k = q - b * rpt;
+          long ray = (tile - (long)(held - 1 - b) * gridDim.x) * rpt + k;
+          const bool active = q0 + wave < nq && ray < R;
+          if (ray >= R) ray = R - 1;
+          sampler_step_ray(tl.st, ray, active, rr, tsdf + b * T + k * npr, tl.do_final == 0, lane, sync);
+          if (tl.do_final) sampler_final_ray(tl.fin, tl.fs, tl.do_fine != 0, ray, active, rr, stage, lane, sync);
+        }
+        held = 0;
+        lds_barrier();
+      }
+    }
   }
 }
 
 #undef VC_LANE_INDICES
 
 template <int RT, int CB>
-static void launch_sdf_value_chain(const SdfValueChain& c, cnr_stream s) {
+static size_t tail_lds(SamplerTail& t) {
+  constexpr int T = 32 * RT, WAVES = 8 / CB;
+  const size_t chain = (size_t)2 * T * CH_ALD + (size_t)T * 9 * sizeof(float) + (size_t)1024 * sizeof(float);
+  t.wave_floats = kRayRows * t.row_ld + kRayNewRows * 64 + (t.do_final && t.do_fine ? kFineStageRows * kFineRowLd : 0);
+  const size_t rows = (size_t)WAVES * t.wave_floats * sizeof(float);
+  t.top_off = (int)(((chain > rows ? chain : rows) + 15) & ~(size_t)15);
+  const int rpt = T / t.npr;
+  t.batch = rpt >= WAVES ? 1 : WAVES / rpt;
+  const size_t lds = (size_t)t.top_off + (size_t)(256 + t.batch * T) * sizeof(float);
+  return lds <= 160 * 1024 ? lds : 0;
+}
+
+template <int RT, int CB, int TAIL = 0>
+static bool launch_sdf_value_chain(const SdfValueChain& c, cnr_stream s, const SamplerTail* tail = nullptr) {
   constexpr int T = 32 * RT, THREADS = 512 / CB;
-  const size_t lds = (size_t)2 * T * CH_ALD + (size_t)T * 9 * sizeof(float) + (size_t)(1024 + 256) * sizeof(float);
+  size_t lds = (size_t)2 * T * CH_ALD + (size_t)T * 9 * sizeof(float) + (size_t)(1024 + 256) * sizeof(float);
+  typename std::conditional<TAIL != 0, SamplerTail, NoTail>::type tl;
+  if constexpr (TAIL != 0) {
+    tl = *tail;
+    lds = tail_lds<RT, CB>(tl);
+    if (lds == 0) return false;
+  }
   static DeviceOnce attr_once;
   if (attr_once.first())
-    (void)hipFuncSetAttribute(reinterpret_cast<const void*>(&sdf_value_chain_kernel<RT, CB>), hipFuncAttributeMaxDynamicSharedMemorySize, 160 * 1024);
+    (void)hipFuncSetAttribute(reinterpret_cast<const void*>(&sdf_value_chain_kernel<RT, CB, TAIL>), hipFuncAttributeMaxDynamicSharedMemorySize, 160 * 1024);
   const long ntiles = (c.P + T - 1) / T;
   const int wgs_env = debug_flags().chain_wgs;
   const long wgs = wgs_env > 0 ? wgs_env : (lds * 2 <= 160 * 1024 ? 512 : 256);
@@ -247,14 +296,39 @@
   double macs = 0.0;
   for (int l = 0; l < c.nl; ++l) macs += (double)c.lay[l].K * 256.0;
   TimingScope ts_("chain_sdf_value", 3, RT * 10 + CB, c.P, (int)(macs / 256.0), 256, 1, s, (double)c.P * (kEmb + 1) * 4.0);
-  hipLaunchKernelGGL((sdf_value_chain_kernel<RT, CB>), dim3(grid), dim3(THREADS), lds, s, c);
-}
-
-bool be_sdf_value_chain(const SdfValueChain& c, cnr_stream s) {
+  hipLaunchKernelGGL((sdf_value_chain_kernel<RT, CB, TAIL>), dim3(grid), dim3(THREADS), lds, s, c, tl);
+  return true;
+}
+
+static bool value_chain_shapes_ok(const SdfValueChain& c) {
   const bool off = debug_flags().no_fused;
   if (off || c.P <= 0) return false;
   for (int l = 0; l < c.nl; ++l)
     if ((c.lay[l].K != 256 && c.lay[l].K != 48) || c.lay[l].N > 256 || c.lay[l].N < 1) return false;
+  return true;
+}
+
+bool be_sdf_value_chain_tail(const SdfValueChain& c, const SamplerTail& t, cnr_stream s) {
+  if (!value_chain_shapes_ok(c)) return false;
+  const int npr = t.npr;
+  if (npr < 1 || npr > 128 || 128 % npr != 0 || c.P % npr != 0 || c.P / npr != t.st.u.R) return false;
+  if (t.st.u.m < 1 || t.st.u.m > 64 || t.st.u.w_in || t.st.u.u_in || t.row_ld < t.st.u.n + (t.do_final ? t.fin.m : 0)) return false;
+  if (t.st.do_merge ? (t.st.g.m != npr || t.st.g.m > 64 || t.st.g.n + t.st.g.m != t.st.u.n) : t.st.u.n != npr) return false;
+  if (t.do_final && (t.fin.n != t.st.u.n || t.fin.m != t.st.u.m || (t.do_fine && t.fs.M != t.fin.n + t.fin.m))) return false;
+  const int force = debug_flags().chain_shape;
+  int shape = force ? force : (c.P >= 256L * 128 ? 41 : (c.P >= 256L * 64 ? 22 : 12));
+  if (shape == 12 && 32 % npr != 0) shape = 22;
+  if (shape == 22 && 64 % npr != 0) shape = 41;
+  bool ok;
+  if (shape == 41) ok = launch_sdf_value_chain<4, 1, 1>(c, s, &t);
+  else if (shape == 22) ok = launch_sdf_value_chain<2, 2, 1>(c, s, &t);
+  else ok = launch_sdf_value_chain<1, 2, 1>(c, s, &t);
+  if (ok) CNR_LAUNCH_CHECK("chain_sdf_value");
+  return ok;
+}
+
+bool be_sdf_value_chain(const SdfValueChain& c, cnr_stream s) {
+  if (!value_chain_shapes_ok(c)) return false;
   const int force = debug_flags().chain_shape;
   const int shape = force ? force : (c.P >= 256L * 128 ? 41 : (c.P >= 256L * 64 ? 22 : 12));
   if (shape == 41) launch_sdf_value_chain<4, 1>(c, s);
diff --git a/color-neus_amd/csrc/cnr_debug.h b/color-neus_amd/csrc/cnr_debug.h
--- a/color-neus_amd/csrc/cnr_debug.h
+++ b/color-neus_amd/csrc/cnr_debug.h
@@ -4,7 +4,7 @@
 
 struct DebugFlags {
   bool no_fused = false, no_chain_fwd = false, no_chain_sdf = false, no_fdw = false, fdw_split = false, no_top_fuse = false,
-       no_head_bwd = false, no_head_fwd = false, no_strip_bwd = false, no_sampler_fuse = false, no_sweep0 = false, no_narrow_bwd = false,
+       no_head_bwd = false, no_head_fwd = false, no_strip_bwd = false, no_sampler_fuse = false, no_sampler_tail = false, no_sweep0 = false, no_narrow_bwd = false,
        no_narrow_dx = false, disable_ws = false, ws_generic = false, ws_nostream = false, dw_fp32 = false, dw_bf16 = false, roctx = false;
   int ws_serp = 1;
 #ifdef CNR_TUNING
diff --git a/color-neus_amd/csrc/cnr_kernels.hip b/color-neus_amd/csrc/cnr_kernels.hip
--- a/color-neus_amd/csrc/cnr_kernels.hip
+++ b/color-neus_amd/csrc/cnr_kernels.hip
@@ -8,6 +8,7 @@
 #include "cnr_loss.h"
 #include "cnr_bodies.h"
 #include "cnr_hip_util.h"
+#include "cnr_ray_steps.h"
 
 namespace cnr {
 
@@ -503,11 +504,6 @@
   CNR_LAUNCH_CHECK("gbar_finish");
 }
 
-__device__ __forceinline__ float wave_sum(float x) {
-#pragma unroll
-  for (int d = 32; d >= 1; d >>= 1) x += __shfl_xor(x, d);
-  return x;
-}
 __device__ __forceinline__ float wave_max(float x) {
 #pragma unroll
   for (int d = 32; d >= 1; d >>= 1) x = fmaxf(x, __shfl_xor(x, d));
@@ -909,62 +905,10 @@
   CNR_LAUNCH_CHECK("variance_finish");
 }
 
-__device__ __forceinline__ float wave_scan_incl_add(float x, int lane) {
-#pragma unroll
-  for (int d = 1; d < 64; d <<= 1) { float y = __shfl_up(x, d); if (lane >= d) x = y + x; }
-  return x;
-}
-__device__ __forceinline__ float wave_scan_incl_mul(float x, int lane) {
-#pragma unroll
-  for (int d = 1; d < 64; d <<= 1) { float y = __shfl_up(x, d); if (lane >= d) x = y * x; }
-  return x;
-}
-__device__ __forceinline__ float wave_excl_cumprod(float f, int lane, float& carry) {
-  const float incl = wave_scan_incl_mul(f, lane);
-  float excl = __shfl_up(incl, 1);
-  if (lane == 0) excl = 1.0f;
-  const float T = carry * excl;
-  carry = carry * __shfl(incl, 63);
-  return T;
-}
 __device__ __forceinline__ float wave_scan_incl_add_rev(float x, int lane) {
 #pragma unroll
   for (int d = 1; d < 64; d <<= 1) { float y = __shfl_down(x, d); if (lane + d < 64) x = x + y; }
   return x;
-}
-
-__device__ __forceinline__ void ray_section_slopes(const float* zs, const float* ss, int nsec, float* cs, int lane) {
-  for (int i = lane; i < nsec; i += 64) cs[i] = upsample_slope(ss[i], ss[i + 1], zs[i], zs[i + 1]);
-}
-__device__ __forceinline__ void ray_section_alphas(const float* zs, const float* ss, const float* cs, const float* rs, int nsec, float inv_s, float* as, int lane) {
-  for (int i = lane; i < nsec; i += 64) {
-    const float c = upsample_cos(i > 0 ? cs[i - 1] : 0.0f, cs[i], rs[i], rs[i + 1]);
-    as[i] = upsample_alpha(ss[i], ss[i + 1], zs[i], zs[i + 1], c, inv_s);
-  }
-}
-__device__ __forceinline__ float ray_pdf_weights(float* as, int nsec, bool given_w, int lane) {
-  float carry = 1.0f, part = 0.0f;
-  for (int base = 0; base < nsec; base += 64) {
-    const int i = base + lane;
-    const bool ok = i < nsec;
-    const float a = ok ? as[i] : 0.0f;
-    const float T = wave_excl_cumprod(ok ? 1.0f - a + 1e-7f : 1.0f, lane, carry);
-    const float w = (given_w ? a : a * T) + 1e-5f;
-    if (ok) { as[i] = w; part += w; }
-  }
-  return wave_sum(part);
-}
-__device__ __forceinline__ void ray_cdf(const float* as, float total, int nsec, float* cs, int lane) {
-  float csum = 0.0f;
-  for (int base = 0; base < nsec; base += 64) {
-    const int i = base + lane;
-    const bool ok = i < nsec;
-    const float pdf = ok ? as[i] / total : 0.0f;
-    const float incl = wave_scan_incl_add(pdf, lane);
-    if (ok) cs[i + 1] = csum + incl;
-    csum = csum + __shfl(incl, 63);
-  }
-  if (lane == 0) cs[0] = 0.0f;
 }
 
 __global__ __launch_bounds__(256) void upsample_kernel(const UpSample p) {
@@ -1028,68 +972,13 @@
     });
 }
 __global__ __launch_bounds__(256) void sampler_step_kernel(const SamplerStep p) {
-  __shared__ float sh[4][7][kMaxRaySamples];
-  __shared__ float shn[4][2][64];
+  __shared__ float sh[4][kRayRows][kMaxRaySamples];
+  __shared__ float shn[4][kRayNewRows][64];
   const int lane = threadIdx.x & 63, wave = threadIdx.x >> 6;
   long ray = (long)blockIdx.x * 4 + wave;
   const bool active = ray < p.u.R;
   if (!active) ray = p.u.R - 1;
-  float* zs = sh[wave][0]; float* ss = sh[wave][1]; float* cs = sh[wave][2]; float* rs = sh[wave][3]; float* as = sh[wave][4];
-  float* zo = sh[wave][5]; float* so = sh[wave][6]; float* nz = shn[wave][0]; float* ns = shn[wave][1];
-  const UpSample& u = p.u;
-  const int n = u.n, nsec = u.n - 1;
-  float o[3], d[3];
-  for (int c = 0; c < 3; ++c) { o[c] = u.o[ray * 3 + c]; d[c] = u.d[ray * 3 + c]; }
-  if (p.do_merge) {
-    const MergeZ& g = p.g;
-    for (int i = lane; i < g.n; i += 64) { zo[i] = g.z[ray * g.ldz + i]; so[i] = g.sdf_in[ray * g.lds_in + i]; }
-    for (int j = lane; j < g.m; j += 64) { nz[j] = g.new_z[ray * g.m + j]; ns[j] = g.new_sdf[ray * g.m + j]; }
-    __syncthreads();
-    merge_samples(zo, so, g.n, nz, ns, g.m, lane, 64, [&](int at, float z, float s) { zs[at] = z; ss[at] = s; });
-    __syncthreads();
-    if (active)
-      for (int i = lane; i < n; i += 64) { g.z[ray * g.ldz + i] = zs[i]; g.sdf_out[ray * g.lds_out + i] = ss[i]; }
-  } else {
-    for (int i = lane; i < n; i += 64) { zs[i] = u.z[ray * u.ldz + i]; ss[i] = u.sdf[ray * u.lds + i]; }
-    __syncthreads();
-  }
-  for (int i = lane; i < n; i += 64) rs[i] = ray_radius(o, d, zs[i]);
-  __syncthreads();
-  ray_section_slopes(zs, ss, nsec, cs, lane);
-  __syncthreads();
-  ray_section_alphas(zs, ss, cs, rs, nsec, u.inv_s, as, lane);
-  __syncthreads();
-  const float total = ray_pdf_weights(as, nsec, false, lane);
-  __syncthreads();
-  ray_cdf(as, total, nsec, cs, lane);
-  __syncthreads();
-  if (lane < u.m) {
-    const float znew = invert_cdf(cs, zs, n, linspace_at(0.5f / (float)u.m, 1.0f - 0.5f / (float)u.m, u.m, lane));
-    nz[lane] = znew;
-    if (active) u.new_z[ray * u.m + lane] = znew;
-  }
-  if (p.do_embed) {
-    __syncthreads();
-    if (active) {
-      const int ntr = kEmb / 3;
-      for (int idx = lane; idx < u.m * ntr; idx += 64) {
-        const int j = idx / ntr, t = idx - j * ntr;
-        const float z = nz[j];
-        float v[3];
-        const int k = t > 0 ? (t - 1) >> 1 : 0;
-        const float f = (float)(1 << k);
-#pragma unroll
-        for (int c = 0; c < 3; ++c) {
-          const float x = (o[c] + d[c] * z) * p.scale;
-          float sn, cn;
-          sincosf(x * f, &sn, &cn);
-          v[c] = t == 0 ? x : (t <= 2 * p.multires ? ((t & 1) ? sn : cn) : 0.0f);
-        }
-        float* e = p.E + (ray * u.m + j) * kEmb + 3 * t;
-        e[0] = v[0]; e[1] = v[1]; e[2] = v[2];
-      }
-    }
-  }
+  sampler_step_ray(p, ray, active, ray_rows(&sh[wave][0][0], kMaxRaySamples, &shn[wave][0][0]), nullptr, true, lane, [] { __syncthreads(); });
 }
 void be_sampler_step(const SamplerStep& p, cnr_stream s) {
   TimingScope ts_("sampler_step", 2, 0, p.u.R, 0, 0, 0, s, (double)p.u.R * (8.0 * p.u.n + 24.0 + 4.0 * p.u.m + (p.do_embed ? 4.0 * kEmb * p.u.m : 0.0)));
diff --git a/color-neus_amd/csrc/cnr_kernels_emu.cpp b/color-neus_amd/csrc/cnr_kernels_emu.cpp
--- a/color-neus_amd/csrc/cnr_kernels_emu.cpp
+++ b/color-neus_amd/csrc/cnr_kernels_emu.cpp
@@ -508,6 +508,7 @@
 
 void be_pack_frags_many(const PackJob*, int, cnr_stream) {}
 bool be_sdf_value_chain(const SdfValueChain&, cnr_stream) { return false; }
+bool be_sdf_value_chain_tail(const SdfValueChain&, const SamplerTail&, cnr_stream) { return false; }
 bool be_relu_chain_fwd(const ReluChainFwd&, cnr_stream) { return false; }
 bool be_relu_chain_fwd_enabled() { return false; }
 bool be_sdf_save_chain(const SdfSaveChain&, cnr_stream) { return false; }
diff --git a/color-neus_amd/csrc/cnr_plan.cpp b/color-neus_amd/csrc/cnr_plan.cpp
--- a/color-neus_amd/csrc/cnr_plan.cpp
+++ b/color-neus_amd/csrc/cnr_plan.cpp
@@ -19,7 +19,7 @@
         {"CNR_NO_FUSED", &DebugFlags::no_fused}, {"CNR_NO_CHAIN_FWD", &DebugFlags::no_chain_fwd}, {"CNR_NO_CHAIN_SDF", &DebugFlags::no_chain_sdf},
         {"CNR_NO_FDW", &DebugFlags::no_fdw}, {"CNR_FDW_SPLIT", &DebugFlags::fdw_split},
         {"CNR_NO_TOP_FUSE", &DebugFlags::no_top_fuse}, {"CNR_NO_HEAD_BWD", &DebugFlags::no_head_bwd}, {"CNR_NO_HEAD_FWD", &DebugFlags::no_head_fwd},
-        {"CNR_NO_STRIP_BWD", &DebugFlags::no_strip_bwd}, {"CNR_NO_SAMPLER_FUSE", &DebugFlags::no_sampler_fuse}, {"CNR_NO_SWEEP0", &DebugFlags::no_sweep0},
+        {"CNR_NO_STRIP_BWD", &DebugFlags::no_strip_bwd}, {"CNR_NO_SAMPLER_FUSE", &DebugFlags::no_sampler_fuse}, {"CNR_NO_SAMPLER_TAIL", &DebugFlags::no_sampler_tail}, {"CNR_NO_SWEEP0", &DebugFlags::no_sweep0},
         {"CNR_NO_NARROW_BWD", &DebugFlags::no_narrow_bwd}, {"CNR_NO_NARROW_DX", &DebugFlags::no_narrow_dx}, {"CNR_DISABLE_WS", &DebugFlags::disable_ws},
         {"CNR_WS_GENERIC", &DebugFlags::ws_generic}, {"CNR_WS_NOSTREAM", &DebugFlags::ws_nostream}, {"CNR_DW_FP32", &DebugFlags::dw_fp32},
         {"CNR_DW_BF16", &DebugFlags::dw_bf16}, {"CNR_ROCTX", &DebugFlags::roctx}};
@@ -583,7 +583,7 @@
   return v;
 }
 
-static bool sdf_value_chain_fused(const Model& m, long n, const float* E, float* sdf_out, float top_scale, cnr_stream s) {
+static bool sdf_value_chain_fused(const Model& m, long n, const float* E, float* sdf_out, float top_scale, cnr_stream s, const SamplerTail* tail = nullptr) {
   if (m.Hs != 256 || m.L < 1) return false;
   if (m.skip(m.L) || m.sdf[m.L - 1].n != 256 || m.sdf[m.L].ldw < 256) return false;
   SdfValueChain c;
@@ -595,7 +595,7 @@
   }
   const Lin& t = m.sdf[m.L];
   c.wtop = t.W + (long)m.F * t.ldw; c.btop = t.bias + m.F; c.top_scale = top_scale; c.sdf_out = sdf_out;
-  return be_sdf_value_chain(c, s);
+  return tail ? be_sdf_value_chain_tail(c, *tail, s) : be_sdf_value_chain(c, s);
 }
 
 static bool sdf_save_chain_fused(const Model& m, long n, const float* E, float* const* Z, float* sdf_out, float* feat_out, int ld_feat,
@@ -646,20 +646,52 @@
   }
 }
 
-static void run_sampler(const Model& m, const cnr_render_inputs* in, float* z, Ctx& x, cnr_stream s) {
+static bool run_sampler(const Model& m, const cnr_render_inputs* in, float* z, Ctx& x, cnr_stream s, const FineSetup* fine = nullptr) {
   const long R = in->n_rays;
   const float scale = m.c.sdf_scale;
   EmbedZ e;
   e.o = in->rays_o; e.d = in->rays_d; e.R = R; e.m = m.S; e.z = z; e.ldz = m.M; e.make_z = 1;
   e.near_ = in->near_; e.far_ = in->far_; e.t_rand = in->t_rand; e.scale = scale; e.multires = m.c.sdf_multires; e.E = x.sE;
   be_embed_z(e, s);
-  if (m.I <= 0) return;
+  if (m.I <= 0) return false;
   float* Zp[kMaxLayers];
   for (int l = 0; l < m.L; ++l) Zp[l] = (l & 1) ? x.sZb : x.sZa;
-  sdf_chain(m, R * m.S, x.sE, Zp, x.s_sdf0, nullptr, 0, 1.0f / scale, s);
   const int mnew = m.I / m.K;
   int n = m.S;
   const bool unfused = debug_flags().no_sampler_fuse;
+  const bool tails = !debug_flags().no_sampler_tail && !unfused && mnew >= 1 && mnew <= 64 && m.I == mnew * m.K && 128 % m.S == 0 &&
+                     128 % mnew == 0 && (long)mnew * kEmb <= (long)m.M * x.ldfx;
+  if (tails) {
+    float* En = x.featx;
+    for (int i = 0; i < m.K; ++i) {
+      const bool last = i + 1 == m.K;
+      SamplerTail t;
+      SamplerStep& st = t.st;
+      UpSample& u = st.u;
+      u.o = in->rays_o; u.d = in->rays_d; u.R = R; u.z = z; u.ldz = m.M;
+      u.sdf = i == 0 ? x.s_sdf0 : x.s_sdf; u.lds = i == 0 ? m.S : m.M; u.n = n; u.m = mnew;
+      u.inv_s = 64.0f * (float)(1 << i); u.new_z = x.s_newz;
+      MergeZ& g = st.g;
+      g.R = R; g.z = z; g.ldz = m.M; g.sdf_in = i <= 1 ? x.s_sdf0 : x.s_sdf; g.lds_in = i <= 1 ? m.S : m.M;
+      g.sdf_out = x.s_sdf; g.lds_out = m.M; g.n = n - mnew; g.new_z = x.s_newz; g.new_sdf = x.s_newsdf; g.m = mnew;
+      st.do_merge = i > 0; st.do_embed = !last; st.E = En; st.scale = scale; st.multires = m.c.sdf_multires;
+      t.npr = i == 0 ? m.S : mnew; t.row_ld = round_up(m.M, 4);
+      t.fin = g; t.fin.sdf_in = i == 0 ? x.s_sdf0 : x.s_sdf; t.fin.lds_in = i == 0 ? m.S : m.M; t.fin.n = n; t.fin.new_sdf = nullptr;
+      t.do_final = last; t.do_fine = last && fine;
+      if (fine) t.fs = *fine; else t.fs = FineSetup{};
+      const float* Ein = i == 0 ? x.sE : En;
+      float* sdf_out = i == 0 ? x.s_sdf0 : x.s_newsdf;
+      if (!sdf_value_chain_fused(m, R * t.npr, Ein, sdf_out, 1.0f / scale, s, &t)) {
+        sdf_chain(m, R * t.npr, Ein, Zp, sdf_out, nullptr, 0, 1.0f / scale, s);
+        be_sampler_step(st, s);
+        if (last) be_merge(t.fin, s);
+        if (last && fine) be_fine_setup(*fine, s);
+      }
+      n += mnew;
+    }
+    return fine != nullptr;
+  }
+  sdf_chain(m, R * m.S, x.sE, Zp, x.s_sdf0, nullptr, 0, 1.0f / scale, s);
   MergeZ prev;
   for (int i = 0; i < m.K; ++i) {
     const bool last = i + 1 == m.K;
@@ -686,6 +718,7 @@
     prev = g;
     n += mnew;
   }
+  return false;
 }
 
 static int skip_off(const Model& m) {
@@ -936,16 +969,17 @@
 
   RangeScope range_fwd("cnr_render_forward");
   { RangeScope r_("weights"); prep_all(m, params, s); }
+  FineSetup fs;
+  fs.o = in->rays_o; fs.d = in->rays_d; fs.z = out->z_vals; fs.R = R; fs.M = m.M; fs.sample_dist = 2.0f / (float)m.S;
+  fs.scale = scale; fs.multires = m.c.sdf_multires; fs.multires_view = m.mv; fs.E = x.E; fs.AUX = x.AUX;
+  bool fine_done = false;
   if (in->z_vals_override) {
     if (in->z_vals_override != out->z_vals) return fail("z_vals_override must alias outputs.z_vals (copy it there first)");
   } else {
     RangeScope r_("sampler");
-    run_sampler(m, in, out->z_vals, x, s);
-  }
-  FineSetup fs;
-  fs.o = in->rays_o; fs.d = in->rays_d; fs.z = out->z_vals; fs.R = R; fs.M = m.M; fs.sample_dist = 2.0f / (float)m.S;
-  fs.scale = scale; fs.multires = m.c.sdf_multires; fs.multires_view = m.mv; fs.E = x.E; fs.AUX = x.AUX;
-  be_fine_setup(fs, s);
+    fine_done = run_sampler(m, in, out->z_vals, x, s, &fs);
+  }
+  if (!fine_done) be_fine_setup(fs, s);
   PointOpts po;
   po.grad_out = g_out; po.multires_view = m.mv;
   point_pipeline(m, P, x, po, s);
diff --git a/color-neus_amd/csrc/cnr_ray_steps.h b/color-neus_amd/csrc/cnr_ray_steps.h
--- /dev/null
+++ b/color-neus_amd/csrc/cnr_ray_steps.h
@@ -0,0 +1,166 @@
+#pragma once
+#include <hip/hip_runtime.h>
+
+#include "cnr_backend.h"
+#include "cnr_bodies.h"
+
+namespace cnr {
+
+__device__ __forceinline__ float wave_sum(float x) {
+#pragma unroll
+  for (int d = 32; d >= 1; d >>= 1) x += __shfl_xor(x, d);
+  return x;
+}
+__device__ __forceinline__ float wave_scan_incl_add(float x, int lane) {
+#pragma unroll
+  for (int d = 1; d < 64; d <<= 1) { float y = __shfl_up(x, d); if (lane >= d) x = y + x; }
+  return x;
+}
+__device__ __forceinline__ float wave_scan_incl_mul(float x, int lane) {
+#pragma unroll
+  for (int d = 1; d < 64; d <<= 1) { float y = __shfl_up(x, d); if (lane >= d) x = y * x; }
+  return x;
+}
+__device__ __forceinline__ float wave_excl_cumprod(float f, int lane, float& carry) {
+  const float incl = wave_scan_incl_mul(f, lane);
+  float excl = __shfl_up(incl, 1);
+  if (lane == 0) excl = 1.0f;
+  const float T = carry * excl;
+  carry = carry * __shfl(incl, 63);
+  return T;
+}
+
+__device__ __forceinline__ void ray_section_slopes(const float* zs, const float* ss, int nsec, float* cs, int lane) {
+  for (int i = lane; i < nsec; i += 64) cs[i] = upsample_slope(ss[i], ss[i + 1], zs[i], zs[i + 1]);
+}
+__device__ __forceinline__ void ray_section_alphas(const float* zs, const float* ss, const float* cs, const float* rs, int nsec, float inv_s, float* as, int lane) {
+  for (int i = lane; i < nsec; i += 64) {
+    const float c = upsample_cos(i > 0 ? cs[i - 1] : 0.0f, cs[i], rs[i], rs[i + 1]);
+    as[i] = upsample_alpha(ss[i], ss[i + 1], zs[i], zs[i + 1], c, inv_s);
+  }
+}
+__device__ __forceinline__ float ray_pdf_weights(float* as, int nsec, bool given_w, int lane) {
+  float carry = 1.0f, part = 0.0f;
+  for (int base = 0; base < nsec; base += 64) {
+    const int i = base + lane;
+    const bool ok = i < nsec;
+    const float a = ok ? as[i] : 0.0f;
+    const float T = wave_excl_cumprod(ok ? 1.0f - a + 1e-7f : 1.0f, lane, carry);
+    const float w = (given_w ? a : a * T) + 1e-5f;
+    if (ok) { as[i] = w; part += w; }
+  }
+  return wave_sum(part);
+}
+__device__ __forceinline__ void ray_cdf(const float* as, float total, int nsec, float* cs, int lane) {
+  float csum = 0.0f;
+  for (int base = 0; base < nsec; base += 64) {
+    const int i = base + lane;
+    const bool ok = i < nsec;
+    const float pdf = ok ? as[i] / total : 0.0f;
+    const float incl = wave_scan_incl_add(pdf, lane);
+    if (ok) cs[i + 1] = csum + incl;
+    csum = csum + __shfl(incl, 63);
+  }
+  if (lane == 0) cs[0] = 0.0f;
+}
+__device__ __forceinline__ void ray_embed_rows(const float o[3], const float d[3], const float* nz, int m, float scale, int multires, float* E, int lane) {
+  const int ntr = kEmb / 3;
+  for (int idx = lane; idx < m * ntr; idx += 64) {
+    const int j = idx / ntr, t = idx - j * ntr;
+    const float z = nz[j];
+    float v[3];
+    const int k = t > 0 ? (t - 1) >> 1 : 0;
+    const float f = (float)(1 << k);
+#pragma unroll
+    for (int c = 0; c < 3; ++c) {
+      const float x = (o[c] + d[c] * z) * scale;
+      float sn, cn;
+      sincosf(x * f, &sn, &cn);
+      v[c] = t == 0 ? x : (t <= 2 * multires ? ((t & 1) ? sn : cn) : 0.0f);
+    }
+    float* e = E + j * kEmb + 3 * t;
+    e[0] = v[0]; e[1] = v[1]; e[2] = v[2];
+  }
+}
+
+constexpr int kRayRows = 7, kRayNewRows = 2;
+struct RayRows { float *zs, *ss, *cs, *rs, *as, *zo, *so, *nz, *ns; };
+__device__ __forceinline__ RayRows ray_rows(float* rows, int ld, float* newrows) {
+  RayRows r;
+  r.zs = rows; r.ss = rows + ld; r.cs = rows + 2 * ld; r.rs = rows + 3 * ld; r.as = rows + 4 * ld; r.zo = rows + 5 * ld; r.so = rows + 6 * ld;
+  r.nz = newrows; r.ns = newrows + 64;
+  return r;
+}
+
+template <class Sync>
+__device__ __forceinline__ void sampler_step_ray(const SamplerStep& p, long ray, bool active, const RayRows& r, const float* tile_sdf, bool store_merged,
+                                                 int lane, Sync sync) {
+  const UpSample& u = p.u;
+  const int n = u.n, nsec = u.n - 1;
+  float o[3], d[3];
+  for (int c = 0; c < 3; ++c) { o[c] = u.o[ray * 3 + c]; d[c] = u.d[ray * 3 + c]; }
+  if (p.do_merge) {
+    const MergeZ& g = p.g;
+    for (int i = lane; i < g.n; i += 64) { r.zo[i] = g.z[ray * g.ldz + i]; r.so[i] = g.sdf_in[ray * g.lds_in + i]; }
+    for (int j = lane; j < g.m; j += 64) { r.nz[j] = g.new_z[ray * g.m + j]; r.ns[j] = tile_sdf ? tile_sdf[j] : g.new_sdf[ray * g.m + j]; }
+    sync();
+    merge_samples(r.zo, r.so, g.n, r.nz, r.ns, g.m, lane, 64, [&](int at, float z, float s) { r.zs[at] = z; r.ss[at] = s; });
+    sync();
+    if (active && store_merged)
+      for (int i = lane; i < n; i += 64) { g.z[ray * g.ldz + i] = r.zs[i]; g.sdf_out[ray * g.lds_out + i] = r.ss[i]; }
+  } else {
+    for (int i = lane; i < n; i += 64) { r.zs[i] = u.z[ray * u.ldz + i]; r.ss[i] = tile_sdf ? tile_sdf[i] : u.sdf[ray * u.lds + i]; }
+    sync();
+  }
+  for (int i = lane; i < n; i += 64) r.rs[i] = ray_radius(o, d, r.zs[i]);
+  sync();
+  ray_section_slopes(r.zs, r.ss, nsec, r.cs, lane);
+  sync();
+  ray_section_alphas(r.zs, r.ss, r.cs, r.rs, nsec, u.inv_s, r.as, lane);
+  sync();
+  const float total = ray_pdf_weights(r.as, nsec, false, lane);
+  sync();
+  ray_cdf(r.as, total, nsec, r.cs, lane);
+  sync();
+  if (lane < u.m) {
+    const float znew = invert_cdf(r.cs, r.zs, n, linspace_at(0.5f / (float)u.m, 1.0f - 0.5f / (float)u.m, u.m, lane));
+    r.nz[lane] = znew;
+    if (active) u.new_z[ray * u.m + lane] = znew;
+  }
+  if (p.do_embed) {
+    sync();
+    if (active) ray_embed_rows(o, d, r.nz, u.m, p.scale, p.multires, p.E + ray * u.m * kEmb, lane);
+  }
+}
+
+constexpr int kFineStageRows = 64, kFineRowLd = 49;
+template <class Sync>
+__device__ __forceinline__ void sampler_final_ray(const MergeZ& g, const FineSetup& f, bool do_fine, long ray, bool active, const RayRows& r, float* stage,
+                                                  int lane, Sync sync) {
+  sync();
+  merge_samples(r.zs, r.ss, g.n, r.nz, r.ns, g.m, lane, 64, [&](int at, float z, float) { r.zo[at] = z; });
+  sync();
+  const int M = g.n + g.m;
+  if (active)
+    for (int i = lane; i < M; i += 64) g.z[ray * g.ldz + i] = r.zo[i];
+  if (!do_fine) return;
+  static_assert(kFineStageRows == 64 && kEmb == 48 && kAux == 48, "one staged row per lane, 48-float rows");
+  for (int base = 0; base < M; base += kFineStageRows) {
+    const int j = base + lane;
+    float z0 = 0.0f, dist = 0.0f;
+    if (j < M) fine_section(r.zo, j, M, f.sample_dist, z0, dist);
+    const int cnt = (M - base < kFineStageRows ? M - base : kFineStageRows) * 48;
+    if (j < M) fine_setup_row(f, ray, z0, dist, stage + lane * kFineRowLd, nullptr);
+    sync();
+    if (active)
+      for (int e = lane; e < cnt; e += 64) { const int row = e / 48; f.E[(ray * M + base) * kEmb + e] = stage[row * kFineRowLd + e - row * 48]; }
+    sync();
+    if (j < M) fine_setup_row(f, ray, z0, dist, nullptr, stage + lane * kFineRowLd);
+    sync();
+    if (active)
+      for (int e = lane; e < cnt; e += 64) { const int row = e / 48; f.AUX[(ray * M + base) * kAux + e] = stage[row * kFineRowLd + e - row * 48]; }
+    sync();
+  }
+}
+
+}
```

After: 187,900 rays/s. Within noise of the previous version (-0.0%).
